# arnauqb/GradABM-JUNE

Measured on AMD Instinct MI355X. Metric: simulation steps/sec, higher is better.
Workload: dtype f32

## Files before the change

### gradabm-june_amd/csrc/gj_tiled.h

```cpp
#pragma once
#include <hip/hip_runtime.h>
#include <stdint.h>

#include "../../include/gradjune_hip.h"
#include "gj_device.h"

namespace gj {

constexpr int kTileThreads = 1024;
constexpr int kTileWaves = kTileThreads / kWave;
constexpr int kMaxSliceAgents = 19840;
constexpr int kUnroll = 8;
#ifndef GJ_UNROLL_NARROW
#define GJ_UNROLL_NARROW 16
#endif
constexpr int kUnrollNarrow = GJ_UNROLL_NARROW;
#ifndef GJ_VENUE_UNROLL
#define GJ_VENUE_UNROLL 2
#endif
constexpr int kVenueUnroll = GJ_VENUE_UNROLL;
#ifndef GJ_VENUE_UNROLL_C
#define GJ_VENUE_UNROLL_C GJ_VENUE_UNROLL
#endif
constexpr int kVenueUnrollC = GJ_VENUE_UNROLL_C;
#ifndef GJ_CUM_BATCH
#define GJ_CUM_BATCH 8
#endif
constexpr int kCumBatch = GJ_CUM_BATCH;
#ifndef GJ_DMA_WIDE
#define GJ_DMA_WIDE 0
#endif

typedef unsigned long long fx_t;
template <int BITS>
__device__ __forceinline__ constexpr float fx_max() { return (float)(1ull << (50 - BITS)); }
template <int BITS>
__device__ __forceinline__ fx_t to_fx(float x) {
  constexpr double scale = (double)(1ull << BITS);
  constexpr double magic = 6755399441055744.0;
  const double d = __builtin_fma((double)x, scale, magic);
  return (fx_t)(__double_as_longlong(d) - 0x4338000000000000LL);
}
template <int BITS>
__device__ __forceinline__ float from_fx(fx_t v) {
  return (float)((double)(long long)v * (1.0 / (double)(1ull << BITS)));
}
constexpr float kSaturated = 1.0e30f;
__device__ __forceinline__ void fx_flag(uint32_t* flags, int words, int i, float x) {
  const uint32_t bit = 1u << (i & 31);
  if (!(x < 0.0f)) atomicOr(&flags[i >> 5], bit);
  if (!(x > 0.0f)) atomicOr(&flags[words + (i >> 5)], bit);
}
template <int BITS>
__device__ __forceinline__ void fx_add(fx_t* sums, uint32_t* flags, int words, int i, float x) {
  const bool ok = fabsf(x) <= fx_max<BITS>();
  atomicAdd(&sums[i], to_fx<BITS>(ok ? x : 0.0f));
  if (__builtin_expect(!ok, 0)) fx_flag(flags, words, i, x);
}
__device__ __forceinline__ float fx_special(uint32_t pos, uint32_t neg, float v) {
  return (pos & neg) ? __builtin_nanf("") : (pos ? kSaturated : (neg ? -kSaturated : v));
}
template <int BITS>
__device__ __forceinline__ float fx_read(const fx_t* sums, const uint32_t* flags, int words, int i) {
  const uint32_t pos = (flags[i >> 5] >> (i & 31)) & 1u, neg = (flags[words + (i >> 5)] >> (i & 31)) & 1u;
  return fx_special(pos, neg, from_fx<BITS>(sums[i]));
}
constexpr int kFxVenue = 36, kFxAgent = 32;

template <typename T>
__device__ __forceinline__ T at32(const T* base, int idx) {
  return *reinterpret_cast<const T*>(reinterpret_cast<const char*>(base) + (uint64_t)((uint32_t)idx * (uint32_t)sizeof(T)));
}
template <typename T>
__device__ __forceinline__ void put32(T* base, int idx, T v) {
  *reinterpret_cast<T*>(reinterpret_cast<char*>(base) + (uint64_t)((uint32_t)idx * (uint32_t)sizeof(T))) = v;
}

typedef float gj_v4f __attribute__((ext_vector_type(4)));
typedef unsigned int gj_v4u __attribute__((ext_vector_type(4)));
typedef unsigned int gj_v2u __attribute__((ext_vector_type(2)));
template <typename T>
__device__ __forceinline__ T at32nt(const T* base, int idx) {
  return __builtin_nontemporal_load(reinterpret_cast<const T*>(reinterpret_cast<const char*>(base) + (uint64_t)((uint32_t)idx * (uint32_t)sizeof(T))));
}
template <typename T>
__device__ __forceinline__ void put32nt(T* base, int idx, T v) {
  __builtin_nontemporal_store(v, reinterpret_cast<T*>(reinterpret_cast<char*>(base) + (uint64_t)((uint32_t)idx * (uint32_t)sizeof(T))));
}
__device__ __forceinline__ uint4 load_nt(const uint4* p) {
  const gj_v4u v = __builtin_nontemporal_load(reinterpret_cast<const gj_v4u*>(p));
  return make_uint4(v.x, v.y, v.z, v.w);
}
__device__ __forceinline__ float4 load_nt(const float4* p) {
  const gj_v4f v = __builtin_nontemporal_load(reinterpret_cast<const gj_v4f*>(p));
  return make_float4(v.x, v.y, v.z, v.w);
}
__device__ __forceinline__ void store_nt(float4* p, float4 x) {
  gj_v4f v = {x.x, x.y, x.z, x.w};
  __builtin_nontemporal_store(v, reinterpret_cast<gj_v4f*>(p));
}
struct TSetA {
  const uint16_t* a_la;
  const int32_t* tile_sptr;
  const int32_t* tile_jpos;
  const int32_t* chunk_ptr;
  const int4* chunk_desc;
  float* val;
  int32_t J;
  int32_t active;
  int32_t raw;
  int32_t wide;
  int32_t direct;
  int32_t presum;
  const int32_t* multi_slots;
};

struct TileAArgs {
  TSetA sets[GJ_MAX_SETS];
  int32_t n_sets;
  int32_t slice_agents;
  int64_t n_agents;
  const float* trans;
  const float* qtrans;
};

__device__ __forceinline__ void load_slice(float* lds, const float* __restrict__ src, int64_t base, int n_local,
                                           int tid) {
  const int n4 = n_local >> 2;
  const float4* s4 = reinterpret_cast<const float4*>(src + base);
  float4* d4 = reinterpret_cast<float4*>(lds);
  constexpr int kQ = (kMaxSliceAgents + 4 * kTileThreads - 1) / (4 * kTileThreads);
  if (n4 > 0) {
    float4 v[kQ];
#pragma unroll
    for (int u = 0; u < kQ; ++u) v[u] = s4[min(tid + u * kTileThreads, n4 - 1)];
#pragma unroll
    for (int u = 0; u < kQ; ++u)
      if (tid + u * kTileThreads < n4) d4[tid + u * kTileThreads] = v[u];
  }
  for (int i = (n4 << 2) + tid; i < n_local; i += kTileThreads) lds[i] = src[base + i];
}

__device__ __forceinline__ int chunk_slot_fast(const int4 d, int lane) {
  const int split = d.z & 0xFFFF;
  return (lane < split) ? d.x + lane : d.y + (lane - split);
}
__device__ __noinline__ int chunk_slot_slow(const TSetA& T, const int4 d, int row, int i, int lane) {
  const int split = d.z & 0xFFFF;
  if (lane < split) return d.x + lane;
  int j = d.w;
  while (i >= T.tile_sptr[row + j + 1]) ++j;
  return T.tile_jpos[row + j] + (i - T.tile_sptr[row + j]);
}

__device__ __forceinline__ int chunk_slot_wide(const int4 d0, const int4 d1, int lane) {
  int b = d0.x;
  b = (lane >= (d1.z & 0xFF)) ? d0.y : b;
  b = (lane >= ((d1.z >> 8) & 0xFF)) ? d0.z : b;
  b = (lane >= ((d1.z >> 16) & 0xFF)) ? d0.w : b;
  b = (lane >= ((d1.z >> 24) & 0xFF)) ? d1.x : b;
  b = (lane >= (d1.w & 0xFF)) ? d1.y : b;
  return b + lane;
}
__device__ __noinline__ int chunk_slot_walk(const TSetA& T, int row, int i, int j) {
  while (i >= T.tile_sptr[row + j + 1]) ++j;
  return T.tile_jpos[row + j] + (i - T.tile_sptr[row + j]);
}

template <bool WIDE, int U>
__device__ __forceinline__ int batch_desc_load(const TSetA& T, int c_base, int n_chunks, int c0, int lane) {
  constexpr int W = WIDE ? 8 : 4;
  static_assert(U * W <= kWave, "a batch's descriptors must fit one wave-wide load");
  const int32_t* desc = reinterpret_cast<const int32_t*>(T.chunk_desc);
  const int u_l = min(lane / W, U - 1), k_l = lane % W;
  return at32(desc, (c_base + min(c0 + u_l, n_chunks - 1)) * W + k_l);
}

template <bool WIDE, int U>
__device__ __forceinline__ void batch_slots(const TSetA& T, const int word, int row, int seg0, int seg1, int c0,
                                            int lane, int (&slot)[U]) {
  constexpr int W = WIDE ? 8 : 4;
  const int k_l = lane % W;
  const bool flag = WIDE ? (k_l == 7 && (word & 0x100)) : (k_l == 2 && (word >> 16));
  const bool any_multi = __builtin_amdgcn_ballot_w64(flag) != 0ull;
#define GJ_DW(u, k) __builtin_amdgcn_readlane(word, (u) * W + (k))
  if (!any_multi) {
#pragma unroll
    for (int u = 0; u < U; ++u) {
      if (!WIDE) {
        slot[u] = chunk_slot_fast(make_int4(GJ_DW(u, 0), GJ_DW(u, 1), GJ_DW(u, 2), 0), lane);
      } else {
        slot[u] = chunk_slot_wide(make_int4(GJ_DW(u, 0), GJ_DW(u, 1), GJ_DW(u, 2), GJ_DW(u, 3)),
                                  make_int4(GJ_DW(u, 4), GJ_DW(u, 5), GJ_DW(u, 6), GJ_DW(u, 7)), lane);
      }
    }
  } else if (T.multi_slots) {
    int ms[U];
    bool mu[U];
#pragma unroll
    for (int u = 0; u < U; ++u) {
      const int w = WIDE ? GJ_DW(u, 7) : GJ_DW(u, 2);
      mu[u] = WIDE ? ((w & 0x100) != 0) : ((w >> 16) != 0);
      const int j0 = WIDE ? (int)((unsigned)w >> 9) : GJ_DW(u, 3);
      ms[u] = at32(T.multi_slots, (mu[u] ? j0 : 0) * kWave + lane);
    }
#pragma unroll
    for (int u = 0; u < U; ++u) {
      int f;
      if (!WIDE) {
        f = chunk_slot_fast(make_int4(GJ_DW(u, 0), GJ_DW(u, 1), GJ_DW(u, 2), 0), lane);
      } else {
        f = chunk_slot_wide(make_int4(GJ_DW(u, 0), GJ_DW(u, 1), GJ_DW(u, 2), GJ_DW(u, 3)),
                            make_int4(GJ_DW(u, 4), GJ_DW(u, 5), GJ_DW(u, 6), GJ_DW(u, 7)), lane);
      }
      slot[u] = mu[u] ? ms[u] : f;
    }
  } else {
#pragma unroll
    for (int u = 0; u < U; ++u) {
      const int i = min(seg0 + (c0 + u) * kWave + lane, seg1 - 1);
      if (!WIDE) {
        const int4 d = make_int4(GJ_DW(u, 0), GJ_DW(u, 1), GJ_DW(u, 2), GJ_DW(u, 3));
        slot[u] = (d.z >> 16) ? chunk_slot_slow(T, d, row, i, lane) : chunk_slot_fast(d, lane);
      } else {
        const int4 d0 = make_int4(GJ_DW(u, 0), GJ_DW(u, 1), GJ_DW(u, 2), GJ_DW(u, 3));
        const int4 d1 = make_int4(GJ_DW(u, 4), GJ_DW(u, 5), GJ_DW(u, 6), GJ_DW(u, 7));
        slot[u] = (d1.w & 0x100) ? chunk_slot_walk(T, row, i, (int)((unsigned)d1.w >> 9))
                                 : chunk_slot_wide(d0, d1, lane);
      }
    }
  }
#undef GJ_DW
}

#ifndef GJ_SCATTER_PIPELINE
#define GJ_SCATTER_PIPELINE 1
#endif
template <bool WIDE, int kU, bool NT = false>
__device__ __forceinline__ void scatter_batches(const TSetA& T, const float* lds_x, int s, int wave, int lane) {
  const int row = s * T.J;
  const int seg0 = T.tile_sptr[row], seg1 = T.tile_sptr[row + T.J];
  const int c_base = T.chunk_ptr[s];
  const int n_chunks = T.chunk_ptr[s + 1] - c_base;
  constexpr int kStride = kTileWaves * kU;
  auto stage1 = [&](int c, int& word, int (&la)[kU]) {
    const int cc = min(c, n_chunks - 1);
    word = batch_desc_load<WIDE, kU>(T, c_base, n_chunks, cc, lane);
#pragma unroll
    for (int u = 0; u < kU; ++u) la[u] = at32(T.a_la, min(seg0 + (cc + u) * kWave + lane, seg1 - 1));
  };
  auto stage2 = [&](int c, int word, const int (&la)[kU]) {
    int slot[kU];
    batch_slots<WIDE, kU>(T, word, row, seg0, seg1, c, lane, slot);
#ifdef GJ_DIAG_EXTRA_VALU
#pragma unroll
    for (int u = 0; u < kU; ++u)
#pragma unroll
      for (int r = 0; r < GJ_DIAG_EXTRA_VALU; ++r) asm volatile("v_add_u32 %0, %0, 0" : "+v"(slot[u]));
#endif
#pragma unroll
    for (int u = 0; u < kU; ++u) {
      const int i = seg0 + (c + u) * kWave + lane;
      if ((c + u < n_chunks) && (i < seg1)) {
        if (NT) put32nt(T.val, slot[u], lds_x[la[u]]); else put32(T.val, slot[u], lds_x[la[u]]);
      }
    }
  };
  int c0 = wave * kU;
  if (c0 >= n_chunks) return;
  int laA[kU], wordA;
#if GJ_SCATTER_PIPELINE
  int laB[kU], wordB;
  stage1(c0, wordA, laA);
  while (true) {
    const int c1 = c0 + kStride;
    stage1(c1, wordB, laB);
    stage2(c0, wordA, laA);
// ... 38 lines not shown
template <bool WIDE>
__device__ __forceinline__ void gather_set(const TSetA& T, fx_t* lds_acc, uint32_t* lds_flags, int flag_words, int s,
                                           int wave, int lane) {
  const int row = s * T.J;
  const int seg0 = T.tile_sptr[row], seg1 = T.tile_sptr[row + T.J];
  const int c_base = T.chunk_ptr[s];
  const int n_chunks = T.chunk_ptr[s + 1] - c_base;
  constexpr int kU = WIDE ? kUnroll : GJ_UNROLL_D_NARROW;
  constexpr int kStride = kTileWaves * kU;
  auto stage1 = [&](int c, int& word, int (&la)[kU]) {
    const int cc = min(c, n_chunks - 1);
    word = batch_desc_load<WIDE, kU>(T, c_base, n_chunks, cc, lane);
#pragma unroll
    for (int u = 0; u < kU; ++u) la[u] = at32(T.a_la, min(seg0 + (cc + u) * kWave + lane, seg1 - 1));
  };
  auto values = [&](int c, int word, float (&v)[kU]) {
    int slot[kU];
    batch_slots<WIDE, kU>(T, word, row, seg0, seg1, c, lane, slot);
#pragma unroll
    for (int u = 0; u < kU; ++u) {
      const int i = seg0 + (c + u) * kWave + lane;
      const bool ok = (c + u < n_chunks) && (i < seg1);
      v[u] = at32nt(T.val, ok ? slot[u] : 0);
    }
  };
  auto add = [&](int c, const int (&la)[kU], const float (&v)[kU]) {
    constexpr uint32_t kLimit = 0x48800000u;
    static_assert(kFxAgent == 32, "kLimit is the pattern of 2^(50 - kFxAgent)");
    float x[kU];
    uint32_t m = 0u;
#pragma unroll
    for (int u = 0; u < kU; ++u) {
      const int i = seg0 + (c + u) * kWave + lane;
      const bool edge = (c + u < n_chunks) && (i < seg1);
      x[u] = edge ? v[u] : 0.0f;
      m = max(m, __float_as_uint(x[u]) & 0x7FFFFFFFu);
    }
#ifdef GJ_DIAG_EXTRA_VALU
#pragma unroll
    for (int u = 0; u < kU; ++u)
#pragma unroll
      for (int r = 0; r < GJ_DIAG_EXTRA_VALU; ++r) asm volatile("v_add_f32 %0, %0, 0" : "+v"(x[u]));
#endif
    if (__builtin_expect(m <= kLimit, 1)) {
#pragma unroll
      for (int u = 0; u < kU; ++u) atomicAdd(&lds_acc[la[u]], to_fx<kFxAgent>(x[u]));
    } else {
#pragma unroll
      for (int u = 0; u < kU; ++u) {
        if ((__float_as_uint(x[u]) & 0x7FFFFFFFu) <= kLimit) {
          atomicAdd(&lds_acc[la[u]], to_fx<kFxAgent>(x[u]));
        } else {
          fx_flag(lds_flags, flag_words, la[u], x[u]);
        }
      }
    }
  };
  int c0 = wave * kU;
  if (c0 >= n_chunks) return;
  int laA[kU], wordA;
  float v[kU];
#if GJ_GATHER_PIPELINE
  int laB[kU], wordB;
  stage1(c0, wordA, laA);
  while (true) {
    const int c1 = c0 + kStride;
    values(c0, wordA, v);
    stage1(c1, wordB, laB);
    add(c0, laA, v);
    if (c1 >= n_chunks) break;
    const int c2 = c1 + kStride;
    values(c1, wordB, v);
    stage1(c2, wordA, laA);
    add(c1, laB, v);
    if (c2 >= n_chunks) break;
    c0 = c2;
  }
#else
  for (; c0 < n_chunks; c0 += kStride) {
    stage1(c0, wordA, laA);
    values(c0, wordA, v);
    add(c0, laA, v);
  }
#endif
}

template <int kU>
__device__ __forceinline__ void scatter_explicit(const TSetA& T, const float* lds_x, int s, int wave, int lane) {
  const int row = s * T.J;
  const int seg0 = T.tile_sptr[row], seg1 = T.tile_sptr[row + T.J];
  const int n_chunks = T.chunk_ptr[s + 1] - T.chunk_ptr[s];
  const int32_t* slots = reinterpret_cast<const int32_t*>(T.chunk_desc);
  for (int c0 = wave * kU; c0 < n_chunks; c0 += kTileWaves * kU) {
    int la[kU], sl[kU];
#pragma unroll
    for (int u = 0; u < kU; ++u) {
      const int i = min(seg0 + (c0 + u) * kWave + lane, seg1 - 1);
      la[u] = at32(T.a_la, i);
      sl[u] = at32(slots, i);
    }
#pragma unroll
    for (int u = 0; u < kU; ++u) {
      const int i = seg0 + (c0 + u) * kWave + lane;
      if ((c0 + u < n_chunks) && (i < seg1)) put32(T.val, sl[u], lds_x[la[u]]);
    }
  }
}

template <int kU>
__device__ __forceinline__ void gather_explicit(const TSetA& T, fx_t* lds_acc, uint32_t* lds_flags, int flag_words, int s,
                                                int wave, int lane) {
  const int row = s * T.J;
  const int seg0 = T.tile_sptr[row], seg1 = T.tile_sptr[row + T.J];
  const int n_chunks = T.chunk_ptr[s + 1] - T.chunk_ptr[s];
  const int32_t* slots = reinterpret_cast<const int32_t*>(T.chunk_desc);
  constexpr uint32_t kLimit = 0x48800000u;
  for (int c0 = wave * kU; c0 < n_chunks; c0 += kTileWaves * kU) {
    int la[kU], sl[kU];
#pragma unroll
    for (int u = 0; u < kU; ++u) {
      const int i = min(seg0 + (c0 + u) * kWave + lane, seg1 - 1);
      la[u] = at32(T.a_la, i);
      sl[u] = at32(slots, i);
    }
    float x[kU];
#pragma unroll
    for (int u = 0; u < kU; ++u) x[u] = at32(T.val, sl[u]);
    uint32_t m = 0u;
#pragma unroll
    for (int u = 0; u < kU; ++u) {
      const int i = seg0 + (c0 + u) * kWave + lane;
      x[u] = ((c0 + u < n_chunks) && (i < seg1)) ? x[u] : 0.0f;
      m = max(m, __float_as_uint(x[u]) & 0x7FFFFFFFu);
    }
    if (__builtin_expect(m <= kLimit, 1)) {
#pragma unroll
      for (int u = 0; u < kU; ++u) atomicAdd(&lds_acc[la[u]], to_fx<kFxAgent>(x[u]));
    } else {
#pragma unroll
      for (int u = 0; u < kU; ++u) {
        if ((__float_as_uint(x[u]) & 0x7FFFFFFFu) <= kLimit) {
          atomicAdd(&lds_acc[la[u]], to_fx<kFxAgent>(x[u]));
        } else {
          fx_flag(lds_flags, flag_words, la[u], x[u]);
        }
      }
    }
  }
}

#ifndef GJ_SCATTER_WAVES_PER_SIMD
#define GJ_SCATTER_WAVES_PER_SIMD 4
#endif
__global__ __launch_bounds__(kTileThreads, GJ_SCATTER_WAVES_PER_SIMD) void k_tile_scatter(const TileAArgs A) {
  extern __shared__ __align__(16) float lds_x[];
  const int tid = threadIdx.x;
  const int wave = __builtin_amdgcn_readfirstlane(tid / kWave), lane = tid % kWave;
  const int s = blockIdx.x;
  const int64_t base = (int64_t)s * A.slice_agents;
  const int n_local = (int)min((int64_t)A.slice_agents, A.n_agents - base);
  const bool two_sources = A.qtrans != A.trans;
  for (int pass = 0; pass < 2; ++pass) {
    if (pass == 1 && !two_sources) break;
    bool any = false;
    for (int t = 0; t < A.n_sets; ++t)
      if (A.sets[t].active && !A.sets[t].presum && (!two_sources || A.sets[t].raw == pass)) any = true;
    if (!any) continue;
    if (pass == 1) __syncthreads();
    load_slice(lds_x, pass == 0 ? A.qtrans : A.trans, base, n_local, tid);
    __syncthreads();
    for (int t = 0; t < A.n_sets; ++t) {
      const TSetA& T = A.sets[t];
      if (!T.active || T.presum || (two_sources && T.raw != pass)) continue;
      if (T.wide == 2) {
        scatter_explicit<kUnroll>(T, lds_x, s, wave, lane);
      } else if (T.wide) {
        scatter_set<true>(T, lds_x, s, wave, lane);
      } else {
        scatter_set<false>(T, lds_x, s, wave, lane);
      }
    }
  }
}

struct TSetB {
  const int32_t* blk_v0;
  const int32_t* blk_e0;
  const uint16_t* e_lv;
  const uint8_t* e_cls;
  float* val;
  const float* v_pc;
  float* cum;
  int32_t stride;
  int32_t nk;
  float beta[GJ_MAX_NETS_PER_SET];
  int32_t table[GJ_MAX_NETS_PER_SET];
  int32_t age75[GJ_MAX_NETS_PER_SET];
  int32_t leisure;
  int32_t direct;
  uint32_t term_limit;
  int32_t _pad_b;
  const uint16_t* pv_blk;
  const int32_t* blk_r0;
  const float* x;
  int64_t n_x;
};

struct TileBArgs {
  TSetB sets[GJ_MAX_SETS];
  const int32_t* work;
  const float* tables;
  int32_t day_type;
  int32_t mode;
  int32_t transpose;
  int32_t _pad;
};

__device__ __noinline__ void venue_group_slow(fx_t* sums, uint32_t* vflags, int words, uint32_t limit, int base_k, int l0,
                                              int l1, int l2, int l3, int l4, int l5, int l6, int l7, float x0, float x1,
                                              float x2, float x3, float x4, float x5, float x6, float x7) {
  const int lv[8] = {l0, l1, l2, l3, l4, l5, l6, l7};
  const float x[8] = {x0, x1, x2, x3, x4, x5, x6, x7};
#pragma unroll
  for (int q = 0; q < 8; ++q) {
    if (lv[q] == 0xFFFF) continue;
    if ((__float_as_uint(x[q]) & 0x7FFFFFFFu) <= limit) {
      atomicAdd(&sums[base_k + lv[q]], to_fx<kFxVenue>(x[q]));
    } else {
      fx_flag(vflags, words, base_k + lv[q], x[q]);
    }
  }
}

struct Slots8 {
  uint32_t w[4];
  __device__ __forceinline__ int lv(int q) const { return (w[q >> 1] >> ((q & 1) * 16)) & 0xFFFF; }
};

#ifdef GJ_DIAG_STAMPS
constexpr int kDiagVenueSlots = 8192;
__device__ unsigned long long gj_diag_venue[3 * kDiagVenueSlots];
struct VenueStamp {
  unsigned long long t0;
  __device__ VenueStamp() : t0(__builtin_amdgcn_s_memrealtime()) {}
  __device__ ~VenueStamp() {
    if (threadIdx.x == 0 && blockIdx.x < kDiagVenueSlots) {
      gj_diag_venue[3 * blockIdx.x] = t0;
      gj_diag_venue[3 * blockIdx.x + 1] = __builtin_amdgcn_s_memrealtime();
      gj_diag_venue[3 * blockIdx.x + 2] = __builtin_amdgcn_s_getreg((31 << 11) | 20) & 0xF;
    }
  }
};
#endif

#ifndef GJ_VENUE_WAVES_PER_SIMD
#define GJ_VENUE_WAVES_PER_SIMD 4
#endif
__global__ __launch_bounds__(kTileThreads, GJ_VENUE_WAVES_PER_SIMD) void k_tile_venues(const TileBArgs B) {
  extern __shared__ __align__(16) float lds_s[];
#ifdef GJ_DIAG_STAMPS
  VenueStamp gj_stamp;
#endif
  const int tid = threadIdx.x;
  const int set = B.work[2 * blockIdx.x], j = B.work[2 * blockIdx.x + 1];
  const TSetB& T = B.sets[set];
  const int nk = T.nk;
  if (nk == 0) return;
  const int v0 = T.blk_v0[j], nv = T.blk_v0[j + 1] - v0;
  const int g0 = T.blk_e0[j] >> 3, g1 = T.blk_e0[j + 1] >> 3;
  fx_t* sums = reinterpret_cast<fx_t*>(lds_s);
  float* cumf = lds_s;
  float* tabs = lds_s + 2 * ((size_t)nk * nv + 64);
  uint32_t* vflags = reinterpret_cast<uint32_t*>(tabs + (T.leisure ? 2 * nk * 200 : 0));
  const int vwords = (nk * nv + 64 + 31) / 32;
  if (T.leisure) {
    for (int i = tid; i < nk * 200; i += kTileThreads) {
      const int k = i / 200, c = i % 200;
      const float l = B.tables[(int64_t)T.table[k] * GJ_TABLE_SIZE + B.day_type * 200 + c];
      const float lw = T.age75[k] ? l * (((c % 100) > 75) ? 1.0f : 0.0f) : l;
      tabs[i] = B.transpose ? lw : l;
      tabs[nk * 200 + i] = B.transpose ? l : lw;
    }
  }
  const uint4* lv8 = reinterpret_cast<const uint4*>(T.e_lv);
  const uint2* cls8 = reinterpret_cast<const uint2*>(T.e_cls);
  float4* val4 = reinterpret_cast<float4*>(T.val);
  if (B.mode != 2) {
    for (int i = tid; i < nk * nv + 64; i += kTileThreads) sums[i] = 0;
    for (int i = tid; i < 2 * vwords; i += kTileThreads) vflags[i] = 0u;
    __syncthreads();
    const int dummy = nk * nv + (tid & 63);
#if defined(GJ_DIAG_FLOAT_RUNS)
    auto run_sums = [&](const int (&lv)[8], const float (&x)[8], int base_k) {
      float s8 = x[0];
#pragma unroll
      for (int q = 0; q < 8; ++q) {
        const bool last = (q == 7) || (lv[q + (q < 7)] != lv[q]);
        const bool take = last && lv[q] != 0xFFFF;
        fx_add<kFxVenue>(sums, vflags, vwords, take ? base_k + lv[q] : dummy, take ? s8 : 0.0f);
        if (q < 7) s8 = last ? x[q + 1] : s8 + x[q + 1];
      }
    };
#elif defined(GJ_DIAG_SLOT_ADDS)
    auto run_sums = [&](const int (&lv)[8], const float (&x)[8], int base_k) {
#pragma unroll
      for (int q = 0; q < 8; ++q) {
        const bool valid = lv[q] != 0xFFFF;
        const bool ok = fabsf(x[q]) <= fx_max<kFxVenue>();
        atomicAdd(&sums[valid ? base_k + lv[q] : dummy], to_fx<kFxVenue>((ok && valid) ? x[q] : 0.0f));
        if (__builtin_expect(!ok && valid, 0)) fx_flag(vflags, vwords, base_k + lv[q], x[q]);
      }
    };
#else
    auto run_sums = [&](const int (&lv)[8], const float (&x)[8], int base_k) {
      const uint32_t kLimit = T.term_limit;
      static_assert(kFxVenue == 36, "term_limit is derived from 2^(50 - kFxVenue) (fill_set_b)");
      uint32_t m = 0u;
#pragma unroll
      for (int q = 0; q < 8; ++q) m = max(m, __float_as_uint(x[q]) & 0x7FFFFFFFu);
      if (__builtin_expect(m > kLimit, 0)) {
        venue_group_slow(sums, vflags, vwords, kLimit, base_k, lv[0], lv[1], lv[2], lv[3], lv[4], lv[5], lv[6], lv[7], x[0],
                         x[1], x[2], x[3], x[4], x[5], x[6], x[7]);
        return;
      }
      fx_t s8 = 0;
#pragma unroll
      for (int q = 0; q < 8; ++q) {
        const fx_t f = to_fx<kFxVenue>(x[q]);
        const bool first = (q == 0) || (lv[q] != lv[q - (q > 0)]);
        s8 = first ? f : s8 + f;
        const bool last = (q == 7) || (lv[q + (q < 7)] != lv[q]);
        const bool take = last && lv[q] != 0xFFFF;
        atomicAdd(&sums[take ? base_k + lv[q] : dummy], s8);
      }
    };
#endif
#ifndef GJ_WAVE_RUNS
#define GJ_WAVE_RUNS 1
#endif
    auto wave_sum = [&](const float (&xl)[8], int target) -> bool {
      uint32_t m = 0u;
#pragma unroll
      for (int q = 0; q < 8; ++q) m = max(m, __float_as_uint(xl[q]) & 0x7FFFFFFFu);
      if (__builtin_amdgcn_ballot_w64(m > T.term_limit) != 0ull) return false;
      fx_t s = 0;
#pragma unroll
      for (int q = 0; q < 8; ++q) s += to_fx<kFxVenue>(xl[q]);
#pragma unroll
      for (int off = 32; off > 0; off >>= 1) s += __shfl_xor(s, off, kWave);
      if ((tid & (kWave - 1)) == 0) atomicAdd(&sums[target], s);
      return true;
    };
    auto add_group = [&](const uint4 raw, const float4 xa, const float4 xb, const uint2 craw) {
      const Slots8 L{{raw.x, raw.y, raw.z, raw.w}};
      const float x[8] = {xa.x, xa.y, xa.z, xa.w, xb.x, xb.y, xb.z, xb.w};
      int lv[8];
#pragma unroll
      for (int q = 0; q < 8; ++q) lv[q] = L.lv(q);
      bool one_venue = false;
#if GJ_WAVE_RUNS
      {
        const bool mine = (raw.x == raw.y) && (raw.y == raw.z) && (raw.z == raw.w) && ((raw.x >> 16) == (raw.x & 0xFFFFu)) &&
                          (lv[0] != 0xFFFF) && (lv[0] == __builtin_amdgcn_readfirstlane(lv[0]));
        one_venue = __builtin_amdgcn_ballot_w64(mine) == ~0ull;
      }
#endif
      if (!T.leisure) {
        if (!(one_venue && wave_sum(x, lv[0]))) run_sums(lv, x, 0);
      } else {
        const uint32_t cw[2] = {craw.x, craw.y};
        for (int k = 0; k < nk; ++k) {
          const float* tk = tabs + k * 200;
          float xl[8];
#pragma unroll
          for (int q = 0; q < 8; ++q) xl[q] = tk[(cw[q >> 2] >> ((q & 3) * 8)) & 0xFF] * x[q];
          if (!(one_venue && wave_sum(xl, k * nv + lv[0]))) run_sums(lv, xl, k * nv);
        }
      }
    };
    for (int g = g0 + tid; g < g1; g += kVenueUnroll * kTileThreads) {
      uint4 raw[kVenueUnroll];
      float4 xa[kVenueUnroll], xb[kVenueUnroll];
      uint2 craw[kVenueUnroll];
#pragma unroll
      for (int u = 0; u < kVenueUnroll; ++u) {
        const int gu = min(g + u * kTileThreads, g1 - 1);
        raw[u] = lv8[gu];
        xa[u] = load_nt(val4 + 2 * gu);
        xb[u] = load_nt(val4 + 2 * gu + 1);
        craw[u] = T.leisure ? cls8[gu] : make_uint2(0u, 0u);
      }
#pragma unroll
      for (int u = 0; u < kVenueUnroll; ++u)
        if (g + u * kTileThreads < g1) add_group(raw[u], xa[u], xb[u], craw[u]);
    }
    if (T.pv_blk) {
      const int r0 = T.blk_r0[j], r1 = T.blk_r0[j + 1];
      const uint4* pv8 = reinterpret_cast<const uint4*>(T.pv_blk);
      const float4* x4 = reinterpret_cast<const float4*>(T.x);
      const int ga = r0 >> 3, gb = (r1 + 7) >> 3;
      const int g_in = (int)(T.n_x >> 3);
      for (int g = ga + tid; g < gb; g += kVenueUnroll * kTileThreads) {
        uint4 raw[kVenueUnroll];
        float4 xa[kVenueUnroll], xb[kVenueUnroll];
#pragma unroll
        for (int u = 0; u < kVenueUnroll; ++u) {
          const int gu = min(g + u * kTileThreads, gb - 1);
          raw[u] = pv8[gu];
          if (gu < g_in) {
            xa[u] = x4[2 * gu];
            xb[u] = x4[2 * gu + 1];
          } else {
            float t[8];
#pragma unroll
            for (int q = 0; q < 8; ++q) t[q] = ((int64_t)gu * 8 + q < T.n_x) ? T.x[(int64_t)gu * 8 + q] : 0.0f;
            xa[u] = make_float4(t[0], t[1], t[2], t[3]);
            xb[u] = make_float4(t[4], t[5], t[6], t[7]);
          }
        }
#pragma unroll
        for (int u = 0; u < kVenueUnroll; ++u) {
          const int gu = g + u * kTileThreads;
          if (gu >= gb) continue;
          const Slots8 L{{raw[u].x, raw[u].y, raw[u].z, raw[u].w}};
          const float x[8] = {xa[u].x, xa[u].y, xa[u].z, xa[u].w, xb[u].x, xb[u].y, xb[u].z, xb[u].w};
          int lv[8];
#pragma unroll
          for (int q = 0; q < 8; ++q) {
            const int a = gu * 8 + q;
            lv[q] = (a >= r0 && a < r1) ? L.lv(q) : 0xFFFF;
          }
          run_sums(lv, x, 0);
        }
      }
    }
    __syncthreads();
    for (int l0 = tid; l0 < nv; l0 += kCumBatch * kTileThreads) {
      float pc[kCumBatch];
#pragma unroll
      for (int u = 0; u < kCumBatch; ++u) pc[u] = T.v_pc[v0 + min(l0 + u * kTileThreads, nv - 1)];
      for (int k = 0; k < nk; ++k) {
        const float beta = T.beta[k];
#pragma unroll
        for (int u = 0; u < kCumBatch; ++u) {
          const int lv = l0 + u * kTileThreads;
          if (lv < nv) {
            const float c = (beta * pc[u]) * fx_read<kFxVenue>(sums, vflags, vwords, k * nv + lv);
            T.cum[(int64_t)(v0 + lv) * T.stride + k] = c;
            cumf[2 * (k * nv + lv)] = c;
          }
        }
      }
    }
    if (B.mode == 1 || T.direct) return;
  } else {
    if (T.direct) return;
    for (int k = 0; k < nk; ++k) {
      for (int l0 = tid; l0 < nv; l0 += kCumBatch * kTileThreads) {
        float c[kCumBatch];
#pragma unroll
        for (int u = 0; u < kCumBatch; ++u)
          c[u] = T.cum[(int64_t)(v0 + min(l0 + u * kTileThreads, nv - 1)) * T.stride + k];
#pragma unroll
        for (int u = 0; u < kCumBatch; ++u) {
          const int lv = l0 + u * kTileThreads;
          if (lv < nv) cumf[2 * (k * nv + lv)] = c[u];
        }
      }
    }
  }
  __syncthreads();
  for (int g = g0 + tid; g < g1; g += kVenueUnrollC * kTileThreads) {
    uint4 raw[kVenueUnrollC];
    uint2 craw[kVenueUnrollC];
#pragma unroll
    for (int u = 0; u < kVenueUnrollC; ++u) {
      const int gu = min(g + u * kTileThreads, g1 - 1);
      raw[u] = lv8[gu];
      craw[u] = T.leisure ? cls8[gu] : make_uint2(0u, 0u);
    }
#pragma unroll
    for (int u = 0; u < kVenueUnrollC; ++u) {
      const int gu = g + u * kTileThreads;
      if (gu >= g1) continue;
      const Slots8 L{{raw[u].x, raw[u].y, raw[u].z, raw[u].w}};
      float r[8];
      if (!T.leisure) {
#pragma unroll
        for (int q = 0; q < 8; ++q) {
          const int lv = L.lv(q);
          const float c = cumf[2 * (lv != 0xFFFF ? lv : 0)];
          r[q] = (lv != 0xFFFF) ? c : 0.0f;
        }
      } else {
        const uint32_t cw[2] = {craw[u].x, craw[u].y};
#pragma unroll
        for (int q = 0; q < 8; ++q) {
          const int lv = L.lv(q);
          const int c = (cw[q >> 2] >> ((q & 3) * 8)) & 0xFF;
          const int li = lv != 0xFFFF ? lv : 0;
          float a = 0.0f;
          for (int k = 0; k < nk; ++k) a += tabs[nk * 200 + k * 200 + c] * cumf[2 * (k * nv + li)];
          r[q] = (lv != 0xFFFF) ? a : 0.0f;
        }
      }
      store_nt(val4 + 2 * gu, make_float4(r[0], r[1], r[2], r[3]));
      store_nt(val4 + 2 * gu + 1, make_float4(r[4], r[5], r[6], r[7]));
    }
  }
}

constexpr int GJ_MAX_PRESUM = 6;
constexpr int64_t kPresumBad = (int64_t)0x8000000000000000ll;
struct TPSet {
  const uint16_t* ell;
  int64_t plane_stride;
  fx_t* partial;
  int32_t planes, V, stride, nk;
  int32_t group_venues;
  int32_t raw, leisure, _pad;
  int32_t table[GJ_MAX_NETS_PER_SET];
  int32_t age75[GJ_MAX_NETS_PER_SET];
};
struct TilePArgs {
  TPSet sets[GJ_MAX_PRESUM];
  int32_t n_sets;
  int32_t agents_per_wg;
  int64_t n_agents;
  const float* trans;
  const float* qtrans;
  const uint8_t* cls;
  const float* tables;
  int32_t day_type, transpose;
};

constexpr int kPresumQuads = 3;
__device__ __forceinline__ void fx_add_or_poison(fx_t* sums, uint32_t* flags, int i, float x) {
  const bool ok = fabsf(x) <= fx_max<kFxVenue>();
  atomicAdd(&sums[i], to_fx<kFxVenue>(ok ? x : 0.0f));
  if (__builtin_expect(!ok, 0)) atomicOr(&flags[i >> 5], 1u << (i & 31));
}

__global__ __launch_bounds__(kTileThreads) void k_tile_presum(const TilePArgs P) {
  extern __shared__ __align__(16) fx_t lds_p[];
  const int tid = threadIdx.x;
  const int64_t a_begin = (int64_t)blockIdx.x * P.agents_per_wg;
  const int64_t a_end = min(P.n_agents, a_begin + P.agents_per_wg);
  const int n_quads = (int)((max(a_end - a_begin, (int64_t)0) + 3) >> 2);
  for (int t = 0; t < P.n_sets; ++t) {
    const TPSet& T = P.sets[t];
    const int nk = T.nk;
    const float* x = T.raw ? P.trans : P.qtrans;
    for (int v0 = 0; v0 < T.V; v0 += T.group_venues) {
      const int nv = min(T.group_venues, T.V - v0);
      const int n_sums = nv * nk;
      const int dummy = n_sums + (tid & 63);
      float* wtab = reinterpret_cast<float*>(lds_p + n_sums + 64);
      uint32_t* flags = reinterpret_cast<uint32_t*>(wtab + (T.leisure ? nk * 200 : 0));
      __syncthreads();
      for (int i = tid; i < n_sums + 64; i += kTileThreads) lds_p[i] = 0;
      for (int i = tid; i < (n_sums + 64 + 31) / 32; i += kTileThreads) flags[i] = 0u;
      if (T.leisure) {
        for (int i = tid; i < nk * 200; i += kTileThreads) {
          const int k = i / 200, c = i % 200;
          const float l = P.tables[(int64_t)T.table[k] * GJ_TABLE_SIZE + P.day_type * 200 + c];
          const float lw = T.age75[k] ? l * (((c % 100) > 75) ? 1.0f : 0.0f) : l;
          wtab[i] = P.transpose ? lw : l;
        }
      }
      __syncthreads();
      for (int plane = 0; plane < T.planes; ++plane) {
        const uint16_t* ell = T.ell + plane * T.plane_stride + a_begin * 2;
        struct Batch {
          uint4 rows[kPresumQuads];
          float4 xs[kPresumQuads];
          uint32_t cl[kPresumQuads];
        };
        auto load = [&](int b0, Batch& B) {
#pragma unroll
          for (int u = 0; u < kPresumQuads; ++u) {
            const int q = min(b0 + tid + u * kTileThreads, n_quads - 1);
            const int64_t a0 = a_begin + 4 * (int64_t)q;
            B.rows[u] = *reinterpret_cast<const uint4*>(ell + 8 * (int64_t)q);
            if (a0 + 4 <= P.n_agents) {
              B.xs[u] = *reinterpret_cast<const float4*>(x + a0);
            } else {
              B.xs[u] = make_float4(a0 < P.n_agents ? x[a0] : 0.0f, a0 + 1 < P.n_agents ? x[a0 + 1] : 0.0f,
                                    a0 + 2 < P.n_agents ? x[a0 + 2] : 0.0f, 0.0f);
            }
            B.cl[u] = T.leisure ? *reinterpret_cast<const uint32_t*>(P.cls + a0) : 0u;
          }
        };
        auto add = [&](int b0, const Batch& B) {
#pragma unroll
          for (int u = 0; u < kPresumQuads; ++u) {
            const int q = b0 + tid + u * kTileThreads;
            if (q >= n_quads) continue;
            const uint32_t w[4] = {B.rows[u].x, B.rows[u].y, B.rows[u].z, B.rows[u].w};
            const float xv[4] = {B.xs[u].x, B.xs[u].y, B.xs[u].z, B.xs[u].w};
            const int n_ok = (int)min((int64_t)4, a_end - (a_begin + 4 * (int64_t)q));
#pragma unroll
            for (int j = 0; j < 4; ++j) {
#pragma unroll
              for (int c = 0; c < 2; ++c) {
                const int lv = (int)((w[j] >> (16 * c)) & 0xFFFF) - v0;
                const bool in = ((unsigned)lv < (unsigned)nv) && (j < n_ok);
                if (!T.leisure) {
                  fx_add_or_poison(lds_p, flags, in ? lv : dummy, in ? xv[j] : 0.0f);
                } else {
                  const int cj = (B.cl[u] >> (8 * j)) & 0xFF;
                  for (int k = 0; k < nk; ++k)
                    fx_add_or_poison(lds_p, flags, in ? lv * nk + k : dummy, in ? wtab[k * 200 + cj] * xv[j] : 0.0f);
                }
              }
            }
          }
        };
        constexpr int kStep = kPresumQuads * kTileThreads;
        if (n_quads > 0) {
          Batch ba, bb;
          int b0 = 0;
          load(b0, ba);
          while (true) {
            const bool more1 = b0 + kStep < n_quads;
            if (more1) load(b0 + kStep, bb);
            add(b0, ba);
            if (!more1) break;
            b0 += kStep;
            const bool more2 = b0 + kStep < n_quads;
            if (more2) load(b0 + kStep, ba);
            add(b0, bb);
            if (!more2) break;
            b0 += kStep;
          }
        }
      }
      __syncthreads();
      fx_t* out = T.partial + (int64_t)blockIdx.x * T.V * T.stride;
      for (int i = tid; i < n_sums; i += kTileThreads) {
        const int lv = i / nk, k = i % nk;
        const bool bad = (flags[i >> 5] >> (i & 31)) & 1u;
        out[(int64_t)(v0 + lv) * T.stride + k] = bad ? (fx_t)kPresumBad : lds_p[i];
      }
    }
  }
}

struct PReduceSet {
  const fx_t* partial;
  const float* v_pc;
  float* cum;
  int32_t V, stride, nk, first;
  float beta[GJ_MAX_NETS_PER_SET];
};
struct PReduceArgs {
  PReduceSet sets[GJ_MAX_PRESUM];
  int32_t n_sets, n_wgs;
  int32_t total;
  int32_t _pad;
};

__global__ __launch_bounds__(kThreads) void k_presum_reduce(const PReduceArgs R) {
  __shared__ fx_t part[kThreads / kWave][kWave];
  __shared__ uint32_t bad_any[kWave];
  const int lane = threadIdx.x % kWave, wave = threadIdx.x / kWave;
  const int i = blockIdx.x * kWave + lane;
  const bool in = i < R.total;
  int t = 0;
  while (t + 1 < R.n_sets && i >= R.sets[t + 1].first) ++t;
  const PReduceSet& T = R.sets[t];
  const int e = in ? i - T.first : 0;
  const int v = e / T.nk, k = e % T.nk;
  const int64_t idx = (int64_t)v * T.stride + k, table = (int64_t)T.V * T.stride;
  fx_t s = 0;
  bool bad = false;
  if (threadIdx.x < kWave) bad_any[threadIdx.x] = 0u;
  constexpr int kWaves = kThreads / kWave;
  for (int w0 = wave; w0 < R.n_wgs; w0 += kWaves * 8) {
    fx_t p[8];
#pragma unroll
    for (int u = 0; u < 8; ++u) {
      const int w = w0 + u * kWaves;
      p[u] = (in && w < R.n_wgs) ? T.partial[w * table + idx] : (fx_t)0;
    }
#pragma unroll
    for (int u = 0; u < 8; ++u) {
      bad |= p[u] == (fx_t)kPresumBad;
      s += p[u];
    }
  }
  part[wave][lane] = s;
  __syncthreads();
  if (bad) atomicOr(&bad_any[lane], 1u);
  __syncthreads();
  if (wave == 0 && in) {
    fx_t total = 0;
#pragma unroll
    for (int w = 0; w < kWaves; ++w) total += part[w][lane];
    T.cum[idx] = (T.beta[k] * T.v_pc[v]) * (bad_any[lane] ? __builtin_nanf("") : from_fx<kFxVenue>(total));
  }
}

constexpr int GJ_MAX_DIRECT = GJ_MAX_SETS;
constexpr int kClassWeightFloats = GJ_MAX_NETS_PER_SET * 200;
struct TDirect {
  const uint16_t* ell;
  const float* cum;
  int64_t plane_stride;
  int32_t K, planes;
  int32_t V, stride, nk;
  int32_t region;
  int32_t group_venues;
  int32_t _pad;
  int32_t raw, leisure;
  int32_t table[GJ_MAX_NETS_PER_SET];
  int32_t age75[GJ_MAX_NETS_PER_SET];
  const int32_t* win_lo;
  const int32_t* win_n;
};

struct TileDArgs {
  TSetA sets[GJ_MAX_SETS];
  int32_t n_sets;
  int32_t slice_agents;
  int64_t n_agents;
  const float* stage;
  float* susceptibility;
  float* is_infected;
  float* infection_time;
  float* not_infected_probs;
  float* new_infected;
  float* trans_susc;
  const float* exp_noise;
  float now, dt, q_thr;
  int32_t has_q, sample;
  uint64_t seed, step;
  int64_t agent_offset;
  float* acc_scratch;
  float* agent_sums;
  TDirect direct[GJ_MAX_DIRECT];
  int32_t n_direct;
  int32_t table_floats;
  int32_t table1_floats;
  int32_t _pad3;
  int32_t day_type, transpose;
  const uint8_t* cls;
  const float* tables;
  const gj_clock* clock;
  int32_t _pad2;
  int32_t io_vec4;
};

__global__ __launch_bounds__(256) void k_tile_epilogue(const TileDArgs D) {
  const int64_t a = (int64_t)blockIdx.x * blockDim.x + threadIdx.x;
  if (a >= D.n_agents) return;
  const float now = D.clock ? D.clock->now : D.now;
  const uint64_t step = D.clock ? D.clock->step : D.step;
  float susc = D.susceptibility[a];
  float ts = susc * D.acc_scratch[a];
  if (D.trans_susc) D.trans_susc[a] = ts;
  const float p = not_infected_prob(ts, D.dt);
  if (D.not_infected_probs) D.not_infected_probs[a] = p;
  if (!D.sample) return;
  float e0, e1;
  if (D.exp_noise) {
    e0 = D.exp_noise[a];
    e1 = D.exp_noise[D.n_agents + a];
  } else {
    e0 = e1 = 1.0f;
  }
  const float nw = D.exp_noise ? gumbel_new_infected(p, e0, e1)
                               : own_new_infected(p, infection_uniform(D.seed, step, D.agent_offset + a));
  if (D.new_infected) D.new_infected[a] = nw;
  if (nw != 0.0f) {
    float inf = D.is_infected[a], t_inf = D.infection_time[a];
    infect(nw, now, susc, inf, t_inf);
    D.susceptibility[a] = susc;
    D.is_infected[a] = inf;
    D.infection_time[a] = t_inf;
  }
}

constexpr int kQuadsPerLane = (kMaxSliceAgents + 4 * kTileThreads - 1) / (4 * kTileThreads);
static_assert(kQuadsPerLane * 4 * kTileThreads >= kMaxSliceAgents, "a lane's quads must cover the largest slice");

struct DirectBatch {
  uint32_t w[kQuadsPerLane][4];
  uint32_t cls[kQuadsPerLane];
};

__device__ __forceinline__ void direct_load(const TileDArgs& D, const TDirect& T, int64_t base, int n_local, int tid,
                                            int plane, DirectBatch& b) {
  const unsigned last_quad = (unsigned)(n_local - 1) >> 2;
  const uint16_t* ell = T.ell + plane * T.plane_stride + base * 2;
  const uint8_t* cls = D.cls + base;
#pragma unroll
  for (int u = 0; u < kQuadsPerLane; ++u) {
    unsigned q = min((unsigned)(tid + u * kTileThreads), last_quad);
    asm volatile("" : "+v"(q));
    if (!T.win_lo) {
      const uint4 r = load_nt(reinterpret_cast<const uint4*>(ell + 8u * q));
      b.w[u][0] = r.x;
      b.w[u][1] = r.y;
      b.w[u][2] = r.z;
      b.w[u][3] = r.w;
    } else {
      const uint2 r = *reinterpret_cast<const uint2*>(T.ell + base + 4u * q);
      b.w[u][0] = (r.x & 0xFFFFu) | 0xFFFF0000u;
      b.w[u][1] = (r.x >> 16) | 0xFFFF0000u;
      b.w[u][2] = (r.y & 0xFFFFu) | 0xFFFF0000u;
      b.w[u][3] = (r.y >> 16) | 0xFFFF0000u;
    }
    b.cls[u] = T.leisure ? *reinterpret_cast<const uint32_t*>(cls + 4u * q) : 0u;
  }
}

__device__ __forceinline__ void direct_add(const TileDArgs& D, const TDirect& T, float (&acc)[kQuadsPerLane][4],
                                           uint32_t qmask, const float* wtab, const float* tab, int v0, int nv,
                                           int n_local, int tid, const DirectBatch& b) {
  constexpr int K = 2;
  const int nk = T.nk, stride = T.stride;
#pragma unroll
  for (int u = 0; u < kQuadsPerLane; ++u) {
    const int q = tid + u * kTileThreads;
    if (4 * q >= n_local) continue;
    const uint32_t quarantined = T.raw ? 0u : (qmask >> (4 * u)) & 0xFu;
    int idx[4][K];
    bool ok[4][K];
    float x[4][K];
#pragma unroll
    for (int j = 0; j < 4; ++j) {
#pragma unroll
      for (int c = 0; c < K; ++c) {
        const int h = j * K + c;
        const int lv = (int)((b.w[u][h >> 1] >> (16 * (h & 1))) & 0xFFFF) - v0;
        ok[j][c] = ((unsigned)lv < (unsigned)nv) && !((quarantined >> j) & 1u);
        idx[j][c] = ok[j][c] ? lv : 0;
      }
    }
    if (!T.leisure) {
#pragma unroll
      for (int j = 0; j < 4; ++j)
#pragma unroll
        for (int c = 0; c < K; ++c) x[j][c] = tab[idx[j][c] * stride];
    } else {
#pragma unroll
      for (int j = 0; j < 4; ++j)
#pragma unroll
        for (int c = 0; c < K; ++c) x[j][c] = 0.0f;
#pragma unroll
      for (int k = 0; k < GJ_MAX_NETS_PER_SET; ++k) {
        if (k >= nk) break;
        float w[4];
#pragma unroll
        for (int j = 0; j < 4; ++j) w[j] = wtab[k * 200 + ((b.cls[u] >> (8 * j)) & 0xFF)];
#pragma unroll
        for (int j = 0; j < 4; ++j)
#pragma unroll
          for (int c = 0; c < K; ++c) x[j][c] += w[j] * tab[idx[j][c] * stride + k];
      }
    }
#pragma unroll
    for (int j = 0; j < 4; ++j) {
      float sj = 0.0f;
#pragma unroll
      for (int c = 0; c < K; ++c) sj += ok[j][c] ? x[j][c] : 0.0f;
      acc[u][j] += sj;
    }
  }
}

__device__ __forceinline__ void direct_stage(const TileDArgs& D, const TDirect& T, float* wtab, float* tab, int v0,
                                             int nv, int tid) {
  if (T.leisure && v0 == 0) {
    for (int i = tid; i < T.nk * 200; i += kTileThreads) {
      const int k = i / 200, c = i % 200;
      const float l = D.tables[(int64_t)T.table[k] * GJ_TABLE_SIZE + D.day_type * 200 + c];
      const float lw = T.age75[k] ? l * (((c % 100) > 75) ? 1.0f : 0.0f) : l;
      wtab[i] = D.transpose ? l : lw;
    }
  }
#ifndef GJ_DIAG_NO_DIRECT_TABLE
  const float* src = T.cum + (int64_t)v0 * T.stride;
  const int n = nv * T.stride;
  const int lane = tid % kWave, wave = __builtin_amdgcn_readfirstlane(tid / kWave);
#if GJ_DMA_WIDE
  const bool aligned = ((reinterpret_cast<uintptr_t>(src) | reinterpret_cast<uintptr_t>(tab)) & 15u) == 0;
  const int n_wide = aligned ? (n / (4 * kWave)) * (4 * kWave) : 0;
  for (int p = wave; (p + 1) * 4 * kWave <= n_wide; p += kTileWaves)
    __builtin_amdgcn_global_load_lds(src + p * 4 * kWave + 4 * lane, tab + p * 4 * kWave, 16, 0, 0);
  for (int p = wave; n_wide + p * kWave < n; p += kTileWaves)
    __builtin_amdgcn_global_load_lds(src + min(n_wide + p * kWave + lane, n - 1), tab + n_wide + p * kWave, 4, 0, 0);
#else
  for (int p = wave; p * kWave < n; p += kTileWaves)
    __builtin_amdgcn_global_load_lds(src + min(p * kWave + lane, n - 1), tab + p * kWave, 4, 0, 0);
#endif
#endif
}

__device__ __forceinline__ void publish_staged() {
  asm volatile("s_waitcnt vmcnt(0)" ::: "memory");
  __syncthreads();
}

__device__ __forceinline__ bool direct_next(const TileDArgs& D, int& t, int& v0, int& plane) {
  const TDirect& T = D.direct[t];
  if (plane + 1 < T.planes) {
    ++plane;
    return true;
  }
  plane = 0;
  if (!T.win_lo && v0 + T.group_venues < T.V) {
    v0 += T.group_venues;
    return true;
  }
  v0 = 0;
  ++t;
  return t < D.n_direct;
}

__device__ __forceinline__ void direct_sets(const TileDArgs& D, float (&acc)[kQuadsPerLane][4], uint32_t qmask,
                                            float* lds, int64_t base, int n_local, int tid, DirectBatch& cur,
                                            uint64_t diag_t0 = 0) {
  auto wtab_of = [&](int t) { return lds + (t & 1) * kClassWeightFloats; };
  auto tab_of = [&](const TDirect& T) {
    return lds + 2 * kClassWeightFloats + (T.region ? D.table_floats + kWave : 0);
  };
  auto group_nv = [&](const TDirect& T, int v0) { return T.win_lo ? T.win_n[blockIdx.x] : min(T.group_venues, T.V - v0); };
  auto group_lo = [&](const TDirect& T, int v0) { return T.win_lo ? T.win_lo[blockIdx.x] : v0; };
  int t = 0, v0 = 0, plane = 0;
  __syncthreads();
  direct_stage(D, D.direct[0], wtab_of(0), tab_of(D.direct[0]), group_lo(D.direct[0], 0), group_nv(D.direct[0], 0), tid);
  bool more = true;
  while (more) {
    const TDirect& T = D.direct[t];
    const int nv = group_nv(T, v0);
    if (plane == 0) publish_staged();
#ifdef GJ_DIAG_STAMPS
    if (threadIdx.x == 0 && D.trans_susc && t < 4)
      D.trans_susc[(int64_t)blockIdx.x * D.slice_agents + 8 + 2 * t] = (float)(__builtin_amdgcn_s_memtime() - diag_t0);
#endif
    int tn = t, vn = v0, pn = plane;
    more = direct_next(D, tn, vn, pn);
    const bool new_group = more && pn == 0;
    const bool overlap = new_group && D.direct[tn].region != T.region;
    if (overlap)
      direct_stage(D, D.direct[tn], wtab_of(tn), tab_of(D.direct[tn]), group_lo(D.direct[tn], vn), group_nv(D.direct[tn], vn), tid);
    DirectBatch nxt;
    if (more) direct_load(D, D.direct[tn], base, n_local, tid, pn, nxt);
#ifndef GJ_DIAG_NO_DIRECT_ADD
    direct_add(D, T, acc, qmask, wtab_of(t), tab_of(T), v0, nv, n_local, tid, cur);
#else
    if (cur.w[0][0] == 0x12345678u && cur.cls[0] == 77u) acc[0][0] = 1.0f;
#endif
#ifdef GJ_DIAG_STAMPS
    if (threadIdx.x == 0 && D.trans_susc && t < 4)
      D.trans_susc[(int64_t)blockIdx.x * D.slice_agents + 9 + 2 * t] = (float)(__builtin_amdgcn_s_memtime() - diag_t0);
#endif
    if (new_group && !overlap) {
      __syncthreads();
      direct_stage(D, D.direct[tn], wtab_of(tn), tab_of(D.direct[tn]), group_lo(D.direct[tn], vn), group_nv(D.direct[tn], vn), tid);
    }
    if (more) cur = nxt;
    t = tn;
    v0 = vn;
    plane = pn;
  }
}

__device__ __forceinline__ void load_quad(const float* p, int64_t a0, int n_ok, bool vec, float (&v)[4]) {
  if (vec && n_ok >= 4) {
    const float4 x = *reinterpret_cast<const float4*>(p + a0);
    v[0] = x.x;
    v[1] = x.y;
    v[2] = x.z;
    v[3] = x.w;
  } else {
#pragma unroll
    for (int j = 0; j < 4; ++j) v[j] = (j < n_ok) ? p[a0 + j] : 0.0f;
  }
}
template <bool NT = false>
__device__ __forceinline__ void store_quad(float* p, int64_t a0, int n_ok, bool vec, const float (&v)[4]) {
  if (vec && n_ok >= 4) {
    if (NT) {
      store_nt(reinterpret_cast<float4*>(p + a0), make_float4(v[0], v[1], v[2], v[3]));
    } else {
      *reinterpret_cast<float4*>(p + a0) = make_float4(v[0], v[1], v[2], v[3]);
    }
  } else {
#pragma unroll
    for (int j = 0; j < 4; ++j)
      if (j < n_ok) p[a0 + j] = v[j];
  }
}

#ifdef GJ_DIAG_STAMPS
#define GJ_STAMP(k)                                                                                         \
  do {                                                                                                      \
    if (threadIdx.x == 0 && D.trans_susc)                                                                    \
      D.trans_susc[(int64_t)blockIdx.x * D.slice_agents + (k)] = (float)(__builtin_amdgcn_s_memtime() - gj_t0); \
  } while (0)
#else
#define GJ_STAMP(k) do { } while (0)
#endif

__global__ __launch_bounds__(kTileThreads) void k_tile_agents(const TileDArgs D) {
  extern __shared__ __align__(16) fx_t lds_acc[];
#ifdef GJ_DIAG_STAMPS
  const uint64_t gj_t0 = __builtin_amdgcn_s_memtime();
#endif
  const int tid = threadIdx.x;
  const int wave = __builtin_amdgcn_readfirstlane(tid / kWave), lane = tid % kWave;
  const int s = blockIdx.x;
  const int64_t base = (int64_t)s * D.slice_agents;
  const int n_local = (int)min((int64_t)D.slice_agents, D.n_agents - base);
  uint32_t* lds_flags = reinterpret_cast<uint32_t*>(lds_acc + D.slice_agents);
  const int fwords = D.slice_agents / 32;
  for (int i = tid; i < n_local; i += kTileThreads) lds_acc[i] = 0;
  for (int i = tid; i < 2 * fwords; i += kTileThreads) lds_flags[i] = 0u;
  DirectBatch first;
  if (D.n_direct > 0) direct_load(D, D.direct[0], base, n_local, tid, 0, first);
  __syncthreads();
  for (int pass = 0; pass < 2; ++pass) {
    for (int t = 0; t < D.n_sets; ++t) {
      const TSetA& T = D.sets[t];
      if (!T.active || T.direct || T.raw != pass) continue;
      if (T.wide == 2) {
        gather_explicit<kUnroll>(T, lds_acc, lds_flags, fwords, s, wave, lane);
      } else if (T.wide) {
        gather_set<true>(T, lds_acc, lds_flags, fwords, s, wave, lane);
      } else {
        gather_set<false>(T, lds_acc, lds_flags, fwords, s, wave, lane);
      }
    }
    __syncthreads();
    if (pass == 0 && D.has_q) {
      constexpr int kStageBatch = 10;
      for (int i0 = tid; i0 < n_local; i0 += kStageBatch * kTileThreads) {
        float stg[kStageBatch];
#pragma unroll
        for (int u = 0; u < kStageBatch; ++u) stg[u] = D.stage[base + min(i0 + u * kTileThreads, n_local - 1)];
#pragma unroll
        for (int u = 0; u < kStageBatch; ++u) {
          const int i = i0 + u * kTileThreads;
          if (i < n_local && !(stg[u] < D.q_thr)) {
            lds_acc[i] = 0;
            const uint32_t bit = 1u << (i & 31);
            const bool pos = lds_flags[i >> 5] & bit, neg = lds_flags[fwords + (i >> 5)] & bit;
            if (pos != neg) {
              atomicAnd(&lds_flags[i >> 5], ~bit);
              atomicAnd(&lds_flags[fwords + (i >> 5)], ~bit);
            }
          }
        }
      }
      __syncthreads();
    }
  }
  GJ_STAMP(1);
  constexpr int kQ = kQuadsPerLane;
  float acc[kQ][4];
#pragma unroll
  for (int m = 0; m < kQ; ++m) {
    const int i0 = 4 * (tid + m * kTileThreads);
    const int iq = min(i0, D.slice_agents - 4);
    const uint32_t pos = (lds_flags[iq >> 5] >> (iq & 31)) & 0xFu, neg = (lds_flags[fwords + (iq >> 5)] >> (iq & 31)) & 0xFu;
    fx_t raw[4];
#pragma unroll
    for (int j = 0; j < 4; ++j) raw[j] = lds_acc[iq + j];
#pragma unroll
    for (int j = 0; j < 4; ++j) {
      const float v = from_fx<kFxAgent>(raw[j]);
      acc[m][j] = (i0 < n_local) ? (((pos | neg) >> j) & 1u ? fx_special((pos >> j) & 1u, (neg >> j) & 1u, v) : v) : 0.0f;
    }
  }
  if (D.n_direct > 0) {
    uint32_t qmask = 0u;
    if (D.has_q) {
      float stg[kQ][4];
#pragma unroll
      for (int m = 0; m < kQ; ++m) {
        const int i0 = 4 * (tid + m * kTileThreads);
#pragma unroll
        for (int j = 0; j < 4; ++j) stg[m][j] = (i0 + j < n_local) ? D.stage[base + i0 + j] : -INFINITY;
      }
#pragma unroll
      for (int m = 0; m < kQ; ++m)
#pragma unroll
        for (int j = 0; j < 4; ++j) qmask |= (stg[m][j] < D.q_thr) ? 0u : (1u << (4 * m + j));
    }
    GJ_STAMP(2);
#ifndef GJ_DIAG_NO_DIRECT_SETS
#ifdef GJ_DIAG_STAMPS
    direct_sets(D, acc, qmask, reinterpret_cast<float*>(lds_acc), base, n_local, tid, first, gj_t0);
#else
    direct_sets(D, acc, qmask, reinterpret_cast<float*>(lds_acc), base, n_local, tid, first);
#endif
#endif
    GJ_STAMP(3);
  }
  const bool vec = D.io_vec4 != 0;
  if (D.agent_sums) {
#pragma unroll
    for (int m = 0; m < kQ; ++m) {
      const int i0 = 4 * (tid + m * kTileThreads);
      if (i0 < n_local) store_quad<true>(D.agent_sums, base + i0, n_local - i0, vec, acc[m]);
    }
  }
  if (D.acc_scratch) {
#pragma unroll
    for (int m = 0; m < kQ; ++m) {
      const int i0 = 4 * (tid + m * kTileThreads);
      if (i0 < n_local) store_quad(D.acc_scratch, base + i0, n_local - i0, vec, acc[m]);
    }
    return;
  }
  const float now = D.clock ? D.clock->now : D.now;
  const uint64_t step = D.clock ? D.clock->step : D.step;
  const bool own_noise = D.sample && !D.exp_noise;
  const int mis = (int)((D.agent_offset + base) & 3);
  float4* ts4 = reinterpret_cast<float4*>(lds_acc);
  {
    float sq[kQ][4];
#pragma unroll
    for (int m = 0; m < kQ; ++m) {
      int i0 = 4 * (tid + m * kTileThreads);
      asm volatile("" : "+v"(i0));
#pragma unroll
      for (int j = 0; j < 4; ++j) sq[m][j] = 0.0f;
      if (i0 < n_local) load_quad(D.susceptibility, base + i0, n_local - i0, vec, sq[m]);
    }
    __syncthreads();
#pragma unroll
    for (int m = 0; m < kQ; ++m) {
      const int q = tid + m * kTileThreads;
      if (4 * q < n_local)
        ts4[q] = make_float4(sq[m][0] * acc[m][0], sq[m][1] * acc[m][1], sq[m][2] * acc[m][2], sq[m][3] * acc[m][3]);
    }
  }
  GJ_STAMP(4);
  uint32_t infected = 0u;
  int m_run = 0;
  for (int q = tid; 4 * q < n_local; q += kTileThreads, ++m_run) {
    const int i0 = 4 * q;
    const float4 tq = ts4[q];
    const float ts[4] = {tq.x, tq.y, tq.z, tq.w};
    const int64_t a0 = base + i0;
    const int n_ok = n_local - i0;
    float p[4];
#pragma unroll
    for (int j = 0; j < 4; ++j) p[j] = not_infected_prob(ts[j], D.dt);
#ifndef GJ_DIAG_STAMPS
    if (D.trans_susc) store_quad<true>(D.trans_susc, a0, n_ok, vec, ts);
#endif
    if (D.not_infected_probs) store_quad<true>(D.not_infected_probs, a0, n_ok, vec, p);
    if (!D.sample) continue;
    float nw[4], th[4] = {0.0f, 0.0f, 0.0f, 0.0f};
    if (own_noise) {
      const uint64_t g0 = (uint64_t)(D.agent_offset + a0);
      uint32_t r0[4], r1[4] = {0u, 0u, 0u, 0u};
      philox4x32_10(g0 >> 2, step, D.seed, r0);
      if (mis) philox4x32_10((g0 >> 2) + 1, step, D.seed, r1);
#pragma unroll
      for (int j = 0; j < 4; ++j) {
        const int w = mis + j;
        th[j] = u01(w == 0 ? r0[0] : w == 1 ? r0[1] : w == 2 ? r0[2] : w == 3 ? r0[3] : w == 4 ? r1[0] : w == 5 ? r1[1] : r1[2]);
      }
    }
#pragma unroll
    for (int j = 0; j < 4; ++j) {
      if (own_noise) {
        nw[j] = own_new_infected(p[j], th[j]);
      } else {
        float e0 = 1.0f, e1 = 1.0f;
        if (j < n_ok) {
          e0 = D.exp_noise[a0 + j];
          e1 = D.exp_noise[D.n_agents + a0 + j];
        }
        nw[j] = gumbel_new_infected(p[j], e0, e1);
      }
      if (j < n_ok && nw[j] != 0.0f) infected |= 1u << (4 * m_run + j);
    }
    if (D.new_infected) store_quad<true>(D.new_infected, a0, n_ok, vec, nw);
#pragma unroll
    for (int j = 0; j < 4; ++j) {
      if (j < n_ok && nw[j] != 0.0f && nw[j] != 1.0f) {
        infected &= ~(1u << (4 * m_run + j));
        const int64_t a = a0 + j;
        float sc = D.susceptibility[a], inf = D.is_infected[a], t_inf = D.infection_time[a];
        infect(nw[j], now, sc, inf, t_inf);
        D.susceptibility[a] = sc;
        D.is_infected[a] = inf;
        D.infection_time[a] = t_inf;
      }
    }
  }
  GJ_STAMP(6);
#ifndef GJ_TAIL_BATCHED
  if (__builtin_amdgcn_ballot_w64(infected != 0u) != 0ull) {
    uint32_t todo = infected;
    while (todo) {
      const int k = __builtin_ctz(todo);
      todo &= todo - 1u;
      const int64_t a = base + 4 * (tid + (k >> 2) * kTileThreads) + (k & 3);
      float sc = D.susceptibility[a], inf = D.is_infected[a], tinf = D.infection_time[a];
      infect(1.0f, now, sc, inf, tinf);
      D.susceptibility[a] = sc;
      D.is_infected[a] = inf;
      D.infection_time[a] = tinf;
    }
  }
#else
  if (__builtin_amdgcn_ballot_w64(infected != 0u) != 0ull) {
    float sc[kQ][4], inf[kQ][4], tinf[kQ][4];
#pragma unroll
    for (int m = 0; m < kQ; ++m) {
#pragma unroll
      for (int j = 0; j < 4; ++j) {
        const bool hit = (infected >> (4 * m + j)) & 1u;
        const int64_t a = hit ? base + 4 * (tid + m * kTileThreads) + j : base;
        sc[m][j] = D.susceptibility[a];
        inf[m][j] = D.is_infected[a];
        tinf[m][j] = D.infection_time[a];
      }
    }
#pragma unroll
    for (int m = 0; m < kQ; ++m) {
#pragma unroll
      for (int j = 0; j < 4; ++j) {
        const int64_t a = base + 4 * (tid + m * kTileThreads) + j;
        infect(1.0f, now, sc[m][j], inf[m][j], tinf[m][j]);
        if ((infected >> (4 * m + j)) & 1u) {
          D.susceptibility[a] = sc[m][j];
          D.is_infected[a] = inf[m][j];
          D.infection_time[a] = tinf[m][j];
        }
      }
    }
  }
#endif
  GJ_STAMP(5);
}

}
```

### gradabm-june_amd/csrc/gradjune_hip.hip

```cpp
#include <hip/hip_runtime.h>
#include <math.h>
#include <stdint.h>
#include <string.h>

#include "../../include/gradjune_hip.h"
#include "gj_device.h"
#include "gj_tiled.h"

namespace gj {

struct SetP1 {
  const int32_t* v_rowptr;
  const int32_t* v_agent;
  const float* v_pc;
  float* cum;
  int32_t stride;
  int32_t nk;
  float beta[GJ_MAX_NETS_PER_SET];
  int32_t table[GJ_MAX_NETS_PER_SET];
  int32_t raw;
  int32_t leisure;
};

struct P1Args {
  SetP1 sets[GJ_MAX_SETS];
  const gj_block* blocks;
  const float* trans;
  const float* qtrans;
  const uint8_t* cls;
  const float* tables;
  float* partial;
  int32_t day_type;
};

struct SetP2 {
  const int32_t* a_rowptr;
  const int32_t* a_venue;
  const float* cum;
  int32_t stride;
  int32_t nk;
  int32_t mask[GJ_MAX_NETS_PER_SET];
  int32_t table[GJ_MAX_NETS_PER_SET];
};

struct P2Args {
  SetP2 groups[GJ_MAX_SETS];
  int32_t n_groups;
  int32_t any_leisure;
  int64_t n_agents;
  const uint8_t* cls;
  const float* tables;
  const float* stage;
  float* susceptibility;
  float* is_infected;
  float* infection_time;
  float* not_infected_probs;
  float* new_infected;
  float* trans_susc;
  const float* exp_noise;
  float now, dt, q_thr;
  int32_t day_type, has_q, sample;
  uint64_t seed, step;
  int64_t agent_offset;
  const gj_clock* clock;
};

__device__ __forceinline__ float inv_gamma(float x) {
  if (!(x > 0.25f && x < 16.0f)) return expf(-lgammaf(x));
  float up = 1.0f, down = 1.0f;
  while (x > 2.0f) {
    x -= 1.0f;
    up *= x;
  }
  while (x < 1.0f) {
    down *= x;
    x += 1.0f;
  }
  const float z = x - 1.0f;
  float g = 0.035868343f;
  g = g * z - 0.193527818f;
  g = g * z + 0.482199394f;
  g = g * z - 0.756704078f;
  g = g * z + 0.918206857f;
  g = g * z - 0.897056937f;
  g = g * z + 0.988205891f;
  g = g * z - 0.577191652f;
  g = g * z + 1.0f;
  return down / (g * up);
}
__device__ __forceinline__ float fast_pow(float x, float y) {
  if (y == 0.0f) return 1.0f;
  if (x < 0.0f) {
    const float yi = truncf(y);
    if (yi != y) return __builtin_nanf("");
    const float r = __builtin_amdgcn_exp2f(y * __builtin_amdgcn_logf(-x));
    const float h = 0.5f * yi;
    return (truncf(h) != h) ? -r : r;
  }
  return __builtin_amdgcn_exp2f(y * __builtin_amdgcn_logf(x));
}
__device__ __forceinline__ float fast_exp(float e) { return __builtin_amdgcn_exp2f(e * 1.44269504088896341f); }

__device__ __forceinline__ float transmission_value(float mx, float shp, float rt, float sh, float t_inf,
                                                    float inf, float now) {
  const float t = now - t_inf;
  const float d = t - sh;
  const float sign = (sgnf(d + 1e-10f) + 1.0f) / 2.0f;
  const float aux = inv_gamma(shp) * fast_pow(d * rt, shp - 1.0f);
  const float aux2 = fast_exp((sh - t) * rt) * rt;
  return mx * sign * aux * aux2 * inf;
}

__global__ __launch_bounds__(kThreads) void k_transmission(
    int64_t n, const float* __restrict__ mx, const float* __restrict__ shp, const float* __restrict__ rt,
    const float* __restrict__ sh, const float* __restrict__ t_inf, const float* __restrict__ inf,
    const float* __restrict__ stage, float* __restrict__ trans, float* __restrict__ qtrans, float now_arg,
    int has_q, float q_thr, const gj_clock* __restrict__ clock) {
  const float now = clock ? clock->now : now_arg;
  const int64_t n4 = n >> 2;
  const int64_t stride = (int64_t)gridDim.x * blockDim.x;
  for (int64_t i = (int64_t)blockIdx.x * blockDim.x + threadIdx.x; i < n4; i += stride) {
    const float4 f = load_nt(reinterpret_cast<const float4*>(inf) + i);
    float4 r = make_float4(0.0f, 0.0f, 0.0f, 0.0f);
    unsigned m = (f.x != 0.0f ? 1u : 0u) | (f.y != 0.0f ? 2u : 0u) | (f.z != 0.0f ? 4u : 0u) | (f.w != 0.0f ? 8u : 0u);
    if (m) {
      const float4 a = load_nt(reinterpret_cast<const float4*>(mx) + i);
      const float4 b = load_nt(reinterpret_cast<const float4*>(shp) + i);
      const float4 c = load_nt(reinterpret_cast<const float4*>(rt) + i);
      const float4 d = load_nt(reinterpret_cast<const float4*>(sh) + i);
      const float4 e = load_nt(reinterpret_cast<const float4*>(t_inf) + i);
      while (m) {
        const int k = __builtin_ctz(m);
        m &= m - 1u;
#define GJ_PICK(v) (k == 0 ? v.x : k == 1 ? v.y : k == 2 ? v.z : v.w)
        const float val = transmission_value(GJ_PICK(a), GJ_PICK(b), GJ_PICK(c), GJ_PICK(d), GJ_PICK(e), GJ_PICK(f), now);
#undef GJ_PICK
        r.x = k == 0 ? val : r.x;
        r.y = k == 1 ? val : r.y;
        r.z = k == 2 ? val : r.z;
        r.w = k == 3 ? val : r.w;
      }
    }
    reinterpret_cast<float4*>(trans)[i] = r;
    if (has_q) {
      const float4 s = reinterpret_cast<const float4*>(stage)[i];
      float4 q;
      q.x = (s.x < q_thr ? 1.0f : 0.0f) * r.x;
      q.y = (s.y < q_thr ? 1.0f : 0.0f) * r.y;
      q.z = (s.z < q_thr ? 1.0f : 0.0f) * r.z;
      q.w = (s.w < q_thr ? 1.0f : 0.0f) * r.w;
      reinterpret_cast<float4*>(qtrans)[i] = q;
    }
  }
  if (blockIdx.x == 0) {
    const int64_t i = (n4 << 2) + threadIdx.x;
// ... 977 lines not shown
    S.v_rowptr = E.v_rowptr;
    S.v_agent = E.v_agent;
    S.v_pc = E.v_pcontact;
    S.cum = E.cum;
    S.stride = E.cum_stride;
    S.nk = G.nk[g];
    S.raw = p->nets[G.first[g]].mask_kind == GJ_MASK_RAW;
    S.leisure = 0;
    for (int k = 0; k < G.nk[g]; ++k) {
      const gj_network& N = p->nets[G.first[g] + k];
      S.beta[k] = N.beta;
      S.table[k] = N.mask_kind >= GJ_MASK_QL ? N.table : -1;
      if (N.mask_kind >= GJ_MASK_QL) S.leisure = 1;
    }
    if (S.leisure) {
      for (int k = 0; k < G.nk[g]; ++k)
        if (S.table[k] < 0) return GJ_E_PLAN;
    }
  }
  A.blocks = plan->blocks;
  A.trans = st->transmission;
  A.qtrans = p->has_quarantine ? st->q_transmission : st->transmission;
  A.cls = plan->agent_class;
  A.tables = plan->tables;
  A.partial = plan->partial;
  A.day_type = p->day_type;
  hipLaunchKernelGGL(k_venue_reduce, dim3((unsigned)plan->n_blocks), dim3(kThreads), 0, stream, A);
  int rc = launch_status();
  if (rc != GJ_OK) return rc;
  if (plan->n_long_rows > 0) {
    CombineArgs C;
    for (int s = 0; s < GJ_MAX_SETS; ++s) {
      C.sets[s].cum = A.sets[s].cum;
      C.sets[s].stride = A.sets[s].stride;
      C.sets[s].nk = A.sets[s].nk;
    }
    C.rows = plan->long_rows;
    C.partial = plan->partial;
    C.n_rows = plan->n_long_rows;
    const int64_t threads = (int64_t)plan->n_long_rows * GJ_MAX_NETS_PER_SET;
    hipLaunchKernelGGL(k_combine_long, dim3((unsigned)((threads + kThreads - 1) / kThreads)), dim3(kThreads), 0,
                       stream, C);
    rc = launch_status();
  }
  return rc;
}

static int do_agent_gather(const gj_plan* plan, const gj_agent_state* st, const gj_step_params* p, const Groups& G,
                           const gj_step_io* io, int sample, hipStream_t stream) {
  const int64_t n = plan->n_agents;
  if (n == 0) return GJ_OK;
  if (io && io->agent_sums) return GJ_E_PLAN;
  P2Args P;
  P.n_groups = G.n;
  P.any_leisure = 0;
  for (int g = 0; g < G.n; ++g) {
    const gj_edge_set& E = plan->sets[G.set[g]];
    SetP2& S = P.groups[g];
    S.a_rowptr = E.a_rowptr;
    S.a_venue = E.a_venue;
    S.cum = E.cum;
    S.stride = E.cum_stride;
    S.nk = G.nk[g];
    for (int k = 0; k < GJ_MAX_NETS_PER_SET; ++k) {
      S.mask[k] = 0;
      S.table[k] = 0;
    }
    for (int k = 0; k < G.nk[g]; ++k) {
      const gj_network& N = p->nets[G.first[g] + k];
      S.mask[k] = N.mask_kind;
      S.table[k] = N.mask_kind >= GJ_MASK_QL ? N.table : 0;
      if (N.mask_kind >= GJ_MASK_QL) P.any_leisure = 1;
    }
  }
  P.n_agents = n;
  P.cls = plan->agent_class;
  P.tables = plan->tables;
  P.stage = st->current_stage;
  P.susceptibility = st->susceptibility;
  P.is_infected = st->is_infected;
  P.infection_time = st->infection_time;
  P.not_infected_probs = io ? io->not_infected_probs : nullptr;
  P.new_infected = io ? io->new_infected : nullptr;
  P.trans_susc = io ? io->trans_susc : nullptr;
  P.exp_noise = io ? io->exp_noise : nullptr;
  P.now = p->now;
  P.dt = p->delta_time;
  P.q_thr = p->q_threshold;
  P.day_type = p->day_type;
  P.has_q = p->has_quarantine;
  P.sample = sample;
  P.seed = p->seed;
  P.step = p->step;
  P.agent_offset = p->agent_offset;
  P.clock = p->clock;
  const int64_t blocks = (n + kThreads - 1) / kThreads;
  hipLaunchKernelGGL(k_agent_gather, dim3((unsigned)blocks), dim3(kThreads), 0, stream, P);
  return launch_status();
}

static int check_tiled(const gj_plan* plan) {
  const gj_tiled* T = plan->tiled;
  if (T->n_slices < 1 || T->slice_agents < 64 || T->slice_agents % 64 || T->slice_agents > kMaxSliceAgents) return GJ_E_PLAN;
  if ((int64_t)T->n_slices * T->slice_agents < plan->n_ext_agents) return GJ_E_PLAN;
  if (T->n_work < 0 || (T->n_work > 0 && !T->work)) return GJ_E_PLAN;
  for (int s = 0; s < plan->n_sets; ++s) {
    const gj_tiled_set& S = T->sets[s];
    if (S.n_blocks < 0) return GJ_E_PLAN;
    if (S.n_blocks == 0) continue;
    if (!S.blk_v0 || !S.blk_e0 || !S.tile_sptr || !S.tile_jpos || !S.chunk_ptr) return GJ_E_NULL;
    const bool run = S.run_pv_blk || S.run_pv_win || S.run_blk_r0 || S.run_win_lo || S.run_win_n;
    if (run) {
      if (!S.run_pv_blk || !S.run_pv_win || !S.run_blk_r0 || !S.run_win_lo || !S.run_win_n) return GJ_E_NULL;
      if (S.run_max_window < 0 || S.run_max_window > 32768 || S.run_tiled_edges < 0 ||
          S.run_tiled_edges > plan->sets[s].n_edges || S.ell_k)
        return GJ_E_PLAN;
    }
    if (S.presum && (!S.ell_k || T->presum_wgs < 1 || T->presum_wgs > 4096)) return GJ_E_PLAN;
    const int64_t held = run ? (int64_t)S.run_tiled_edges : plan->sets[s].n_edges;
    if (held > 0 && (!S.e_lv || !S.a_la || !S.val || !S.chunk_desc)) return GJ_E_NULL;
    if (S.max_block_venues < 1 || S.max_block_venues > 65536) return GJ_E_PLAN;
    if (plan->sets[s].n_edges >= ((int64_t)1 << 30) - 8 * (int64_t)S.n_blocks) return GJ_E_RANGE;
    if (S.ell_k) {
      if (S.ell_k != 2 && S.ell_k != 4 && S.ell_k != 8) return GJ_E_PLAN;
      if (!S.ell) return GJ_E_NULL;
      if (plan->sets[s].n_venues > 65534) return GJ_E_PLAN;
    }
  }
  return GJ_OK;
}

static inline int64_t tiled_edges(const gj_plan* plan, int s) {
  const gj_tiled_set& S = plan->tiled->sets[s];
  return S.run_pv_blk ? (int64_t)S.run_tiled_edges : plan->sets[s].n_edges;
}

static inline bool uses_presum(const gj_plan* plan, int s) {
  const gj_tiled* T = plan->tiled;
  return T->presum_wgs > 0 && T->sets[s].presum != nullptr && T->sets[s].ell_k != 0 && T->sets[s].n_blocks > 0 &&
         plan->sets[s].n_edges > 0;
}

template <typename K>
static int allow_lds(K kernel, size_t bytes) {
  if (bytes > 160 * 1024) return GJ_E_PLAN;
  if (bytes > 64 * 1024) {
    const hipError_t e = hipFuncSetAttribute(reinterpret_cast<const void*>(kernel),
                                             hipFuncAttributeMaxDynamicSharedMemorySize, (int)bytes);
    if (e != hipSuccess) return (int)e;
  }
  return GJ_OK;
}

static void fill_set_a(const gj_plan* plan, const gj_step_params* p, const Groups& G, TSetA* sets) {
  const gj_tiled* T = plan->tiled;
  for (int s = 0; s < GJ_MAX_SETS; ++s) sets[s] = TSetA{};
  for (int g = 0; g < G.n; ++g) {
    const int s = G.set[g];
    const gj_tiled_set& S = T->sets[s];
    sets[s].a_la = S.a_la;
    sets[s].tile_sptr = S.tile_sptr;
    sets[s].tile_jpos = S.tile_jpos;
    sets[s].chunk_ptr = S.chunk_ptr;
    sets[s].chunk_desc = reinterpret_cast<const int4*>(S.chunk_desc);
    sets[s].val = S.val;
    sets[s].J = S.n_blocks;
    sets[s].active = (S.n_blocks > 0 && tiled_edges(plan, s) > 0) ? G.nk[g] : 0;
    sets[s].presum = uses_presum(plan, s);
    sets[s].raw = p->nets[G.first[g]].mask_kind == GJ_MASK_RAW;
    sets[s].wide = S.desc_wide;
    sets[s].direct = S.ell_k != 0;
    sets[s].multi_slots = S.multi_slots;
  }
}

static size_t slice_lds(const gj_tiled* T, size_t elem) { return (size_t)T->slice_agents * elem; }
static size_t agents_lds(const gj_tiled* T) { return (size_t)T->slice_agents * sizeof(fx_t) + 2 * ((size_t)T->slice_agents / 8); }

static int presum_fill(const gj_plan* plan, const gj_step_params* p, const Groups& G, int g, TPSet* X) {
  const gj_tiled* T = plan->tiled;
  const int s = G.set[g];
  const gj_tiled_set& S = T->sets[s];
  const gj_edge_set& E = plan->sets[s];
  const int64_t owned_slices = (plan->n_agents + T->slice_agents - 1) / T->slice_agents;
  X->ell = S.ell;
  X->plane_stride = owned_slices * (int64_t)T->slice_agents * 2;
  X->partial = reinterpret_cast<fx_t*>(S.presum);
  X->planes = S.ell_k / 2;
  X->V = (int32_t)E.n_venues;
  X->stride = E.cum_stride;
  X->nk = G.nk[g];
  X->raw = p->nets[G.first[g]].mask_kind == GJ_MASK_RAW;
  X->leisure = 0;
  X->_pad = 0;
  for (int k = 0; k < GJ_MAX_NETS_PER_SET; ++k) X->table[k] = X->age75[k] = 0;
  for (int k = 0; k < G.nk[g]; ++k) {
    const gj_network& N = p->nets[G.first[g] + k];
    X->table[k] = N.mask_kind >= GJ_MASK_QL ? N.table : -1;
    X->age75[k] = N.mask_kind == GJ_MASK_QL_AGE75;
    if (N.mask_kind >= GJ_MASK_QL) X->leisure = 1;
  }
  if (X->leisure) {
    if (!plan->agent_class || (uintptr_t)plan->agent_class % 4 != 0) return GJ_E_PLAN;
    for (int k = 0; k < G.nk[g]; ++k)
      if (X->table[k] < 0) return GJ_E_PLAN;
  } else if (G.nk[g] != 1) {
    return GJ_E_PLAN;
  }
  return GJ_OK;
}

static int tiled_presum(const gj_plan* plan, const gj_agent_state* st, const gj_step_params* p, const Groups& G,
                        hipStream_t stream) {
  const gj_tiled* T = plan->tiled;
  TilePArgs P;
  P.n_sets = 0;
  for (int g = 0; g < G.n; ++g) {
    if (!uses_presum(plan, G.set[g])) continue;
    if (P.n_sets == GJ_MAX_PRESUM) return GJ_E_PLAN;
    const int rc = presum_fill(plan, p, G, g, &P.sets[P.n_sets++]);
    if (rc) return rc;
  }
  if (P.n_sets == 0 || plan->n_agents == 0) return GJ_OK;
  const int64_t budget = 160 * 1024;
  size_t lds = 0;
  for (int t = 0; t < P.n_sets; ++t) {
    TPSet& X = P.sets[t];
    const int64_t fixed = 64 * 8 + (X.leisure ? (int64_t)X.nk * 200 * 4 : 0) + 64;
    int64_t per_venue = (int64_t)X.nk * 8;
    int64_t gv = (budget - fixed) * 8 / (per_venue * 8 + X.nk);
    if (T->direct_table_floats > 0 && gv > T->direct_table_floats / X.nk) gv = T->direct_table_floats / X.nk;
    if (gv > X.V) gv = X.V;
    if (gv < 1) gv = 1;
    X.group_venues = (int32_t)gv;
    const size_t need = (size_t)(gv * X.nk + 64) * 8 + (X.leisure ? (size_t)X.nk * 200 * 4 : 0) + ((size_t)(gv * X.nk + 64 + 31) / 32) * 4;
    if (need > lds) lds = need;
  }
  int64_t apw = (plan->n_agents + T->presum_wgs - 1) / T->presum_wgs;
  apw = (apw + 63) / 64 * 64;
  P.agents_per_wg = (int32_t)apw;
  P.n_agents = plan->n_agents;
  P.trans = st->transmission;
  P.qtrans = p->has_quarantine ? st->q_transmission : st->transmission;
  if ((uintptr_t)P.trans % 16 != 0 || (uintptr_t)P.qtrans % 16 != 0) return GJ_E_PLAN;
  P.cls = plan->agent_class;
  P.tables = plan->tables;
  P.day_type = p->day_type;
  P.transpose = p->transpose;
  int rc = allow_lds(k_tile_presum, lds);
  if (rc) return rc;
  hipLaunchKernelGGL(k_tile_presum, dim3((unsigned)T->presum_wgs), dim3(kTileThreads), lds, stream, P);
  return launch_status();
}

static int tiled_presum_reduce(const gj_plan* plan, const gj_step_params* p, const Groups& G, hipStream_t stream) {
  const gj_tiled* T = plan->tiled;
  PReduceArgs R;
  R.n_sets = 0;
  R.n_wgs = T->presum_wgs;
  R._pad = 0;
  int64_t total = 0;
  for (int g = 0; g < G.n; ++g) {
    const int s = G.set[g];
    if (!uses_presum(plan, s)) continue;
    if (R.n_sets == GJ_MAX_PRESUM) return GJ_E_PLAN;
    PReduceSet& X = R.sets[R.n_sets++];
    const gj_edge_set& E = plan->sets[s];
    X.partial = reinterpret_cast<const fx_t*>(T->sets[s].presum);
    X.v_pc = E.v_pcontact;
    X.cum = E.cum;
    X.V = (int32_t)E.n_venues;
    X.stride = E.cum_stride;
    X.nk = G.nk[g];
    X.first = (int32_t)total;
    for (int k = 0; k < GJ_MAX_NETS_PER_SET; ++k) X.beta[k] = k < G.nk[g] ? p->nets[G.first[g] + k].beta : 0.0f;
    total += (int64_t)X.V * X.nk;
  }
  if (R.n_sets == 0 || total == 0) return GJ_OK;
  if (total > INT32_MAX) return GJ_E_RANGE;
  R.total = (int32_t)total;
  hipLaunchKernelGGL(k_presum_reduce, dim3((unsigned)((total + kWave - 1) / kWave)), dim3(kThreads), 0, stream, R);
  return launch_status();
}

static int tiled_scatter(const gj_plan* plan, const gj_agent_state* st, const gj_step_params* p, const Groups& G,
                         hipStream_t stream) {
  const gj_tiled* T = plan->tiled;
  if (plan->n_ext_agents == 0 || G.n == 0) return GJ_OK;
  TileAArgs A;
  fill_set_a(plan, p, G, A.sets);
  A.n_sets = plan->n_sets;
  A.slice_agents = T->slice_agents;
  A.n_agents = plan->n_ext_agents;
  A.trans = st->transmission;
  A.qtrans = p->has_quarantine ? st->q_transmission : st->transmission;
  const size_t lds = slice_lds(T, sizeof(float));
  int rc = allow_lds(k_tile_scatter, lds);
  if (rc) return rc;
  hipLaunchKernelGGL(k_tile_scatter, dim3((unsigned)T->n_slices), dim3(kTileThreads), lds, stream, A);
  rc = launch_status();
  if (rc) return rc;
  return tiled_presum(plan, st, p, G, stream);
}

static uint32_t venue_term_limit(int32_t max_venue_edges) {
  int e = 14;
  int64_t p2 = 4096;
  while (p2 < (int64_t)max_venue_edges && e > -20) {
    p2 <<= 1;
    --e;
  }
  const float lim = ldexpf(1.0f, e);
  uint32_t bits;
  memcpy(&bits, &lim, sizeof(bits));
  return bits;
}

static int tiled_venues(const gj_plan* plan, const gj_agent_state* st, const gj_step_params* p, const Groups& G, int mode,
                        hipStream_t stream) {
  const gj_tiled* T = plan->tiled;
  if (G.n == 0) return GJ_OK;
  if (T->n_work == 0) return mode == 2 ? GJ_OK : tiled_presum_reduce(plan, p, G, stream);
  TileBArgs B;
  for (int s = 0; s < GJ_MAX_SETS; ++s) B.sets[s] = TSetB{};
  size_t lds = 16;
  for (int g = 0; g < G.n; ++g) {
    const int s = G.set[g];
    const gj_tiled_set& S = T->sets[s];
    const gj_edge_set& E = plan->sets[s];
    TSetB& X = B.sets[s];
    X.blk_v0 = S.blk_v0;
    X.blk_e0 = S.blk_e0;
    X.e_lv = S.e_lv;
    X.e_cls = S.e_cls;
    X.val = S.val;
    X.v_pc = E.v_pcontact;
    X.cum = E.cum;
    X.stride = E.cum_stride;
    X.nk = S.n_blocks > 0 ? G.nk[g] : 0;
    if (uses_presum(plan, s)) X.nk = 0;
    X.direct = S.ell_k != 0;
    X.leisure = 0;
    for (int k = 0; k < G.nk[g]; ++k) {
      const gj_network& N = p->nets[G.first[g] + k];
      X.beta[k] = N.beta;
      X.table[k] = N.mask_kind >= GJ_MASK_QL ? N.table : -1;
      X.age75[k] = N.mask_kind == GJ_MASK_QL_AGE75;
      if (N.mask_kind >= GJ_MASK_QL) X.leisure = 1;
    }
    if (X.leisure) {
      if (!S.e_cls && E.n_edges > 0) return GJ_E_PLAN;
      for (int k = 0; k < G.nk[g]; ++k)
        if (X.table[k] < 0) return GJ_E_PLAN;
    } else if (G.nk[g] != 1) {
      return GJ_E_PLAN;
    }
    X.pv_blk = nullptr;
    X.blk_r0 = nullptr;
    X.x = nullptr;
    X.n_x = 0;
    if (S.run_pv_blk && mode != 2) {
      if (X.leisure) return GJ_E_PLAN;
      const bool raw = p->nets[G.first[g]].mask_kind == GJ_MASK_RAW;
      X.x = (p->has_quarantine && !raw) ? st->q_transmission : st->transmission;
      if (!X.x) return GJ_E_NULL;
      if ((uintptr_t)X.x % 16 != 0 || (uintptr_t)S.run_pv_blk % 16 != 0) return GJ_E_PLAN;
      X.pv_blk = S.run_pv_blk;
      X.blk_r0 = S.run_blk_r0;
      X.n_x = plan->n_ext_agents;
    }
    const size_t n_sums = (size_t)X.nk * S.max_block_venues + 64;
    const size_t need = n_sums * sizeof(fx_t) + (X.leisure ? 2 * 200 * (size_t)X.nk : 0) * sizeof(float) +
                        2 * ((n_sums + 31) / 32 * 4);
    X.term_limit = venue_term_limit(S.max_venue_edges);
    if (X.nk && need > lds) lds = need;
  }
  B.work = T->work;
  B.tables = plan->tables;
  B.day_type = p->day_type;
  B.mode = mode;
  B.transpose = p->transpose;
  int rc = allow_lds(k_tile_venues, lds);
  if (rc) return rc;
  hipLaunchKernelGGL(k_tile_venues, dim3((unsigned)T->n_work), dim3(kTileThreads), lds, stream, B);
  rc = launch_status();
  if (rc || mode == 2) return rc;
  return tiled_presum_reduce(plan, p, G, stream);
}

static int tiled_agents(const gj_plan* plan, const gj_agent_state* st, const gj_step_params* p, const Groups& G,
                        const gj_step_io* io, int sample, hipStream_t stream) {
  const gj_tiled* T = plan->tiled;
  if (plan->n_agents == 0) return GJ_OK;
  TileDArgs D;
  fill_set_a(plan, p, G, D.sets);
  D.n_sets = plan->n_sets;
  D.slice_agents = T->slice_agents;
  D.n_agents = plan->n_agents;
  D.stage = st->current_stage;
  D.susceptibility = st->susceptibility;
  D.is_infected = st->is_infected;
  D.infection_time = st->infection_time;
  D.not_infected_probs = io ? io->not_infected_probs : nullptr;
  D.new_infected = io ? io->new_infected : nullptr;
  D.trans_susc = io ? io->trans_susc : nullptr;
  D.agent_sums = io ? io->agent_sums : nullptr;
  D.exp_noise = io ? io->exp_noise : nullptr;
  D.now = p->now;
  D.dt = p->delta_time;
  D.q_thr = p->q_threshold;
  D.has_q = p->has_quarantine;
  D.sample = sample;
  D.seed = p->seed;
  D.step = p->step;
  D.agent_offset = p->agent_offset;
  D.clock = p->clock;
  D.acc_scratch = T->agent_scratch;
  size_t lds = agents_lds(T);
  D.n_direct = 0;
  D.day_type = p->day_type;
  D.transpose = p->transpose;
  D.cls = plan->agent_class;
  D.tables = plan->tables;
  const int64_t owned_slices = (plan->n_agents + T->slice_agents - 1) / T->slice_agents;
  for (int g = 0; g < G.n; ++g) {
    const int s = G.set[g];
    const gj_tiled_set& S = T->sets[s];
    const gj_edge_set& E = plan->sets[s];
    const bool run = S.run_pv_win != nullptr;
    if ((!S.ell_k && !run) || S.n_blocks == 0 || E.n_edges == 0) continue;
    if (D.n_direct == GJ_MAX_DIRECT) return GJ_E_PLAN;
    TDirect& X = D.direct[D.n_direct++];
    X.ell = run ? S.run_pv_win : S.ell;
    X.cum = E.cum;
    X.K = 2;
    X.planes = run ? 1 : S.ell_k / 2;
    X.plane_stride = owned_slices * (int64_t)T->slice_agents * 2;
    X.V = run ? S.run_max_window : (int32_t)E.n_venues;
    X.win_lo = run ? S.run_win_lo : nullptr;
    X.win_n = run ? S.run_win_n : nullptr;
    if (run && (uintptr_t)S.run_pv_win % 8 != 0) return GJ_E_PLAN;
    X.stride = E.cum_stride;
    X.nk = G.nk[g];
    X.raw = p->nets[G.first[g]].mask_kind == GJ_MASK_RAW;
    X.leisure = 0;
    for (int k = 0; k < GJ_MAX_NETS_PER_SET; ++k) X.table[k] = X.age75[k] = 0;
    for (int k = 0; k < G.nk[g]; ++k) {
      const gj_network& N = p->nets[G.first[g] + k];
      X.table[k] = N.mask_kind >= GJ_MASK_QL ? N.table : -1;
      X.age75[k] = N.mask_kind == GJ_MASK_QL_AGE75;
      if (N.mask_kind >= GJ_MASK_QL) X.leisure = 1;
    }
    if (X.leisure) {
      if (!plan->agent_class || (uintptr_t)plan->agent_class % 4 != 0) return GJ_E_PLAN;
      for (int k = 0; k < G.nk[g]; ++k)
        if (X.table[k] < 0) return GJ_E_PLAN;
    } else if (G.nk[g] != 1) {
      return GJ_E_PLAN;
    }
  }
  D.table_floats = D.table1_floats = 0;
  D._pad3 = 0;
  if (D.n_direct) {
    const int64_t budget = 160 * 1024 / 4 - 2 * kClassWeightFloats - 2 * kWave;
    int64_t largest = 0;
    for (int t = 0; t < D.n_direct; ++t) {
      const int64_t sz = (int64_t)D.direct[t].V * D.direct[t].stride;
      largest = largest > sz ? largest : sz;
    }
    int64_t cap0 = largest < budget ? largest : budget;
    if (T->direct_table_floats > 0 && T->direct_table_floats < cap0) cap0 = T->direct_table_floats;
    if (cap0 < GJ_MAX_NETS_PER_SET) cap0 = GJ_MAX_NETS_PER_SET;
    int64_t cap1 = budget - cap0;
    if (T->direct_table_floats > 0 && T->direct_table_floats < cap1) cap1 = T->direct_table_floats;
    int prev_region = -1;
    for (int t = 0; t < D.n_direct; ++t) {
      TDirect& X = D.direct[t];
      const int64_t sz = (int64_t)X.V * X.stride;
      X.region = (prev_region == 0 && sz <= cap1) ? 1 : 0;
      const int64_t cap = X.region ? cap1 : cap0;
      X.group_venues = sz <= cap ? X.V : (int32_t)(cap / X.stride);
      if (X.group_venues < 1 || (X.win_lo && sz > cap)) return GJ_E_PLAN;
      X._pad = 0;
      prev_region = X.region;
    }
    D.table_floats = (int32_t)cap0;
    D.table1_floats = (int32_t)cap1;
    const size_t direct_lds = 4 * ((size_t)2 * kClassWeightFloats + (size_t)cap0 + kWave + (size_t)cap1 + kWave);
    if (direct_lds > lds) lds = direct_lds;
  }
  {
    uintptr_t bits = (uintptr_t)D.susceptibility | (uintptr_t)D.not_infected_probs | (uintptr_t)D.new_infected |
                     (uintptr_t)D.trans_susc | (uintptr_t)D.acc_scratch | (uintptr_t)D.agent_sums;
    D.io_vec4 = (bits % 16 == 0) ? 1 : 0;
  }
  int rc = allow_lds(k_tile_agents, lds);
  if (rc) return rc;
  hipLaunchKernelGGL(k_tile_agents, dim3((unsigned)owned_slices), dim3(kTileThreads), lds, stream, D);
  rc = launch_status();
  if (rc || !D.acc_scratch) return rc;
  hipLaunchKernelGGL(k_tile_epilogue, dim3((unsigned)((plan->n_agents + 255) / 256)), dim3(256), 0, stream, D);
  return launch_status();
}

}


extern "C" {

#ifdef GJ_DIAG_STAMPS
int gj_diag_venue_stamps(unsigned long long* host_out) {
  return (int)hipMemcpyFromSymbol(host_out, HIP_SYMBOL(gj::gj_diag_venue), sizeof(unsigned long long) * 3 * gj::kDiagVenueSlots);
}
#endif

int gj_version(void) { return GJ_ABI_VERSION; }

const char* gj_error_string(int code) {
  switch (code) {
    case GJ_OK: return "ok";
    case GJ_E_NULL: return "required pointer is NULL";
    case GJ_E_RANGE: return "count or index out of range";
    case GJ_E_PLAN: return "inconsistent plan or network list";
    case GJ_E_NODEVICE: return "no HIP device, or not a gfx950 (MI355X) device";
    default: break;
  }
  if (code > 0) return hipGetErrorString((hipError_t)code);
  return "unknown error";
}

int gj_check_device(void) {
  int dev = 0;
  if (hipGetDevice(&dev) != hipSuccess) return GJ_E_NODEVICE;
  hipDeviceProp_t prop;
  if (hipGetDeviceProperties(&prop, dev) != hipSuccess) return GJ_E_NODEVICE;
  const char* want = "gfx950";
  for (int i = 0; want[i]; ++i)
    if (prop.gcnArchName[i] != want[i]) return GJ_E_NODEVICE;
  return GJ_OK;
}

int gj_transmission_update(const gj_plan* plan, const gj_agent_state* state, const gj_step_params* params,
                           void* stream) {
  int rc = gj::check_plan(plan);
  if (rc) return rc;
  if (!params) return GJ_E_NULL;
  rc = gj::check_state(plan, state, params);
  if (rc) return rc;
  return gj::do_transmission(plan, state, params, (hipStream_t)stream);
}

int gj_quarantine_transmission(const gj_plan* plan, const gj_agent_state* state, const gj_step_params* params,
                               void* stream) {
  int rc = gj::check_plan(plan);
  if (rc) return rc;
  if (!params) return GJ_E_NULL;
  rc = gj::check_state(plan, state, params, false);
  if (rc) return rc;
  if (!params->has_quarantine || plan->n_agents == 0) return GJ_OK;
  const int64_t n = plan->n_agents;
  hipLaunchKernelGGL(gj::k_quarantine_transmission, dim3((unsigned)((n + gj::kThreads - 1) / gj::kThreads)),
                     dim3(gj::kThreads), 0, (hipStream_t)stream, n, state->current_stage, state->transmission,
                     state->q_transmission, params->q_threshold);
  return gj::launch_status();
}

int gj_venue_reduce(const gj_plan* plan, const gj_agent_state* state, const gj_step_params* params, void* stream) {
  int rc = gj::check_plan(plan);
  if (rc) return rc;
  gj::Groups G;
  rc = gj::group_networks(plan, params, &G);
  if (rc) return rc;
  rc = gj::check_state(plan, state, params, false);
  if (rc) return rc;
  if (plan->tiled) {
    rc = gj::tiled_scatter(plan, state, params, G, (hipStream_t)stream);
    if (rc) return rc;
    return gj::tiled_venues(plan, state, params, G, 1, (hipStream_t)stream);
  }
  return gj::do_venue_reduce(plan, state, params, G, (hipStream_t)stream);
}

int gj_agent_gather(const gj_plan* plan, const gj_agent_state* state, const gj_step_params* params,
                    const gj_step_io* io, int sample, void* stream) {
  int rc = gj::check_plan(plan);
  if (rc) return rc;
  gj::Groups G;
  rc = gj::group_networks(plan, params, &G);
  if (rc) return rc;
  rc = gj::check_state(plan, state, params, sample != 0);
  if (rc) return rc;
  if (plan->tiled) {
    rc = gj::tiled_venues(plan, state, params, G, 2, (hipStream_t)stream);
    if (rc) return rc;
    return gj::tiled_agents(plan, state, params, G, io, sample, (hipStream_t)stream);
  }
  return gj::do_agent_gather(plan, state, params, G, io, sample, (hipStream_t)stream);
}

int gj_sample_infect(int64_t n_agents, const float* not_infected_probs, const float* exp_noise, uint64_t seed,
                     uint64_t step, int64_t agent_offset, float now, float* new_infected, float* susceptibility,
                     float* is_infected, float* infection_time, void* stream) {
  if (n_agents < 0) return GJ_E_RANGE;
  if (n_agents == 0) return GJ_OK;
  if (!not_infected_probs) return GJ_E_NULL;
  const int n_state = (susceptibility != nullptr) + (is_infected != nullptr) + (infection_time != nullptr);
  if (n_state != 0 && n_state != 3) return GJ_E_NULL;
  if (n_state == 0 && !new_infected) return GJ_E_NULL;
  const int64_t blocks = (n_agents + gj::kThreads - 1) / gj::kThreads;
  hipLaunchKernelGGL(gj::k_sample_infect, dim3((unsigned)blocks), dim3(gj::kThreads), 0, (hipStream_t)stream, n_agents,
                     not_infected_probs, exp_noise, seed, step, agent_offset, now, new_infected, susceptibility,
                     is_infected, infection_time);
  return gj::launch_status();
}

int gj_adjoint_sample(int64_t n, const float* susceptibility0, const float* infection_time0, const float* acc,
                      const float* exp_noise, uint64_t seed, uint64_t step, int64_t agent_offset, float now,
                      float delta_time, const float* g_susc, const float* g_inf, const float* g_time,
                      const float* g_new, float* x_out, float* grad_susc_out, float* grad_time_out, void* stream) {
  if (n < 0) return GJ_E_RANGE;
  if (n == 0) return GJ_OK;
  if (!susceptibility0 || !infection_time0 || !acc || !x_out || !grad_susc_out || !grad_time_out) return GJ_E_NULL;
  hipLaunchKernelGGL(gj::k_adjoint_sample, dim3((unsigned)((n + gj::kThreads - 1) / gj::kThreads)), dim3(gj::kThreads),
                     0, (hipStream_t)stream, n, susceptibility0, infection_time0, acc, exp_noise, seed, step,
                     agent_offset, now, delta_time, g_susc, g_inf, g_time, g_new, x_out, grad_susc_out, grad_time_out);
  return gj::launch_status();
}

int gj_adjoint_transmission(int64_t n, const gj_agent_state* st, float now, const float* trans_bar,
                            const float* g_inf, float* grad_inf_out, float* grad_time_inout, void* stream) {
  if (n < 0) return GJ_E_RANGE;
  if (n == 0) return GJ_OK;
  if (!st || !trans_bar || !grad_inf_out || !grad_time_inout) return GJ_E_NULL;
  if (!st->max_infectiousness || !st->shape || !st->rate || !st->shift || !st->infection_time || !st->is_infected)
    return GJ_E_NULL;
  hipLaunchKernelGGL(gj::k_adjoint_transmission, dim3((unsigned)((n + gj::kThreads - 1) / gj::kThreads)),
                     dim3(gj::kThreads), 0, (hipStream_t)stream, n, st->max_infectiousness, st->shape, st->rate,
                     st->shift, st->infection_time, st->is_infected, now, trans_bar, g_inf, grad_inf_out,
                     grad_time_inout);
  return gj::launch_status();
}

int gj_adjoint_transmission_params(int64_t n, const gj_agent_state* st, float now, const float* trans_bar,
                                   const float* g_inf, float* grad_inf_out, float* grad_time_inout,
                                   float* grad_max_infectiousness_out, float* grad_shape_out, float* grad_rate_out,
                                   float* grad_shift_out, void* stream) {
  if (n < 0) return GJ_E_RANGE;
  if (n == 0) return GJ_OK;
  if (!st || !trans_bar || !grad_inf_out || !grad_time_inout) return GJ_E_NULL;
  if (!st->max_infectiousness || !st->shape || !st->rate || !st->shift || !st->infection_time || !st->is_infected)
    return GJ_E_NULL;
  hipLaunchKernelGGL(gj::k_adjoint_transmission_params, dim3((unsigned)((n + gj::kThreads - 1) / gj::kThreads)),
                     dim3(gj::kThreads), 0, (hipStream_t)stream, n, st->max_infectiousness, st->shape, st->rate,
                     st->shift, st->infection_time, st->is_infected, now, trans_bar, g_inf, grad_inf_out,
                     grad_time_inout, grad_max_infectiousness_out, grad_shape_out, grad_rate_out, grad_shift_out);
  return gj::launch_status();
}

int gj_adjoint_beta_partial(int64_t n_venues, int32_t stride, int32_t nk, const float* cum_fwd, const float* cum_bwd,
                            const float* v_pcontact, const double* weights, const float* beta, const int32_t* cols,
                            double* partial, void* stream) {
  if (n_venues < 0 || stride < 1 || stride > GJ_MAX_NETS_PER_SET || nk < 0 || nk > stride) return GJ_E_RANGE;
  if (!partial || (nk > 0 && (!beta || !cols))) return GJ_E_NULL;
  if (n_venues == 0 || nk == 0) return GJ_OK;
  if (!cum_fwd || !cum_bwd || !v_pcontact) return GJ_E_NULL;
  gj::AdjBetaArgs A;
  A.n_venues = n_venues;
  A.stride = stride;
  A.nk = nk;
  A.cum_fwd = cum_fwd;
  A.cum_bwd = cum_bwd;
  A.v_pc = v_pcontact;
  A.weights = weights;
  for (int k = 0; k < GJ_MAX_NETS_PER_SET; ++k) {
    A.beta[k] = k < nk ? beta[k] : 0.0f;
    A.cols[k] = k < nk ? cols[k] : 0;
    if (k < nk && (cols[k] < 0 || cols[k] >= GJ_MAX_NETS)) return GJ_E_RANGE;
// ... 73 lines not shown

int gj_step_stats(int64_t n, const uint8_t* agent_class, const float* is_infected, const float* current_stage,
                  int32_t n_bins, const int32_t* bin_edges, int32_t dead_stage, double* out, void* stream) {
  if (n < 0 || n_bins < 0 || n_bins > GJ_MAX_AGE_BINS) return GJ_E_RANGE;
  if (!out || (n_bins > 0 && !bin_edges)) return GJ_E_NULL;
  if (n == 0) return GJ_OK;
  if (!agent_class || !is_infected || !current_stage) return GJ_E_NULL;
  gj::StatsArgs S;
  S.n = n;
  S.cls = agent_class;
  S.inf = is_infected;
  S.stage = current_stage;
  S.n_bins = n_bins;
  for (int b = 0; b <= GJ_MAX_AGE_BINS; ++b) S.edges[b] = (b <= n_bins) ? bin_edges[b] : 0;
  S.dead = dead_stage;
  S.out = out;
  S.vec4 = (((uintptr_t)is_infected | (uintptr_t)current_stage) % 16 == 0 && (uintptr_t)agent_class % 4 == 0) ? 1 : 0;
  int64_t blocks = ((S.vec4 ? (n >> 2) + 3 : n) + gj::kThreads - 1) / gj::kThreads;
  if (blocks > 2048) blocks = 2048;
  if (blocks < 1) blocks = 1;
  hipLaunchKernelGGL(gj::k_step_stats, dim3((unsigned)blocks), dim3(gj::kThreads), 0, (hipStream_t)stream, S);
  return gj::launch_status();
}

int gj_symptoms_step_stats(int64_t n, const uint8_t* agent_class, const float* new_infected, float* current_stage,
                           float* next_stage, float* time_to_next_stage, const gj_symptoms_params* params,
                           const float* progresses, const float* dwell, const float* is_infected, int32_t n_bins,
                           const int32_t* bin_edges, int32_t dead_stage, double* out, void* stream) {
  if (n < 0 || n_bins < 0 || n_bins > GJ_MAX_AGE_BINS) return GJ_E_RANGE;
  if (!out || (n_bins > 0 && !bin_edges)) return GJ_E_NULL;
  if (n == 0) return GJ_OK;
  if (!agent_class || !new_infected || !current_stage || !next_stage || !time_to_next_stage || !params || !is_infected)
    return GJ_E_NULL;
  if (params->n_stages < 3 || params->n_stages > GJ_MAX_STAGES) return GJ_E_RANGE;
  if ((progresses == nullptr) != (dwell == nullptr)) return GJ_E_NULL;
  if (!progresses && !params->progress) return GJ_E_NULL;
  gj::SymptomsArgs S;
  S.P = *params;
  S.n = n;
  S.cls = agent_class;
  S.new_inf = new_infected;
  S.cur = current_stage;
  S.nxt = next_stage;
  S.ttn = time_to_next_stage;
  S.progresses = progresses;
  S.dwell = dwell;
  gj::StatsArgs R;
  R.n = n;
  R.cls = agent_class;
  R.inf = is_infected;
  R.stage = current_stage;
  R.n_bins = n_bins;
  for (int b = 0; b <= GJ_MAX_AGE_BINS; ++b) R.edges[b] = (b <= n_bins) ? bin_edges[b] : 0;
  R.dead = dead_stage;
  R.out = out;
  const uintptr_t bits = (uintptr_t)new_infected | (uintptr_t)current_stage | (uintptr_t)next_stage |
                         (uintptr_t)time_to_next_stage | (uintptr_t)is_infected;
  R.vec4 = (bits % 16 == 0 && (uintptr_t)agent_class % 4 == 0) ? 1 : 0;
  int64_t blocks = ((R.vec4 ? (n >> 2) + 3 : n) + gj::kThreads - 1) / gj::kThreads;
  if (blocks > 4096) blocks = 4096;
  if (blocks < 1) blocks = 1;
  hipLaunchKernelGGL(gj::k_symptoms_stats, dim3((unsigned)blocks), dim3(gj::kThreads), 0, (hipStream_t)stream, S, R);
  return gj::launch_status();
}

int gj_group_stats(int64_t n, const int32_t* group, int32_t n_groups, const float* is_infected,
                   const float* current_stage, int32_t dead_stage, double* out, void* workspace, void* stream) {
  if (n < 0 || n_groups < 1 || n_groups > GJ_MAX_GROUPS) return GJ_E_RANGE;
  if (!out || !workspace) return GJ_E_NULL;
  if (n == 0) return GJ_OK;
  if (!group || !is_infected || !current_stage) return GJ_E_NULL;
  gj::GroupArgs S;
  S.n = n;
  S.group = group;
  S.inf = is_infected;
  S.stage = current_stage;
  S.n_groups = n_groups;
  S.dead = dead_stage;
  S.vec4 = (((uintptr_t)group | (uintptr_t)is_infected | (uintptr_t)current_stage) % 16 == 0) ? 1 : 0;
  S.ws = (gj::fx_t*)workspace;
  const int64_t units = S.vec4 ? (n >> 2) + 1 : n;
  if (n_groups <= gj::kGroupLdsMax) {
    int64_t blocks = (units + gj::kGroupLdsThreads - 1) / gj::kGroupLdsThreads;
    if (blocks > gj::kGroupLdsBlocks) blocks = gj::kGroupLdsBlocks;
    hipLaunchKernelGGL(gj::k_group_stats<true>, dim3((unsigned)blocks), dim3(gj::kGroupLdsThreads),
                       (size_t)n_groups * 2 * sizeof(gj::fx_t), (hipStream_t)stream, S);
  } else {
    int64_t blocks = (units + gj::kThreads - 1) / gj::kThreads;
    if (blocks > 2048) blocks = 2048;
    hipLaunchKernelGGL(gj::k_group_stats<false>, dim3((unsigned)blocks), dim3(gj::kThreads), 0, (hipStream_t)stream, S);
  }
  int rc = gj::launch_status();
  if (rc) return rc;
  hipLaunchKernelGGL(gj::k_group_finish, dim3((unsigned)((2 * (int64_t)n_groups + gj::kThreads - 1) / gj::kThreads)),
                     dim3(gj::kThreads), 0, (hipStream_t)stream, n_groups, S.ws, out);
  return gj::launch_status();
}

int gj_adjoint_group_stats(int64_t n, const int32_t* group, int32_t n_groups, const float* current_stage,
                           int32_t dead_stage, const float* g_cases, const float* g_deaths, float* grad_is_infected,
                           float* grad_stage, void* stream) {
  if (n < 0 || n_groups < 1 || n_groups > GJ_MAX_GROUPS) return GJ_E_RANGE;
  if (grad_stage && dead_stage == 0) return GJ_E_RANGE;
  if (n == 0 || (!grad_is_infected && !grad_stage)) return GJ_OK;
  if (!group || (grad_stage && !current_stage)) return GJ_E_NULL;
  gj::GroupAdjArgs S;
  S.n = n;
  S.group = group;
  S.stage = current_stage;
  S.g_cases = g_cases;
  S.g_deaths = g_deaths;
  S.grad_inf = grad_is_infected;
  S.grad_stage = grad_stage;
  S.n_groups = n_groups;
  S.dead = dead_stage;
  const uintptr_t bits = (uintptr_t)group | (uintptr_t)grad_is_infected | (uintptr_t)grad_stage |
                         (grad_stage ? (uintptr_t)current_stage : 0);
  S.vec4 = (bits % 16 == 0) ? 1 : 0;
  int64_t blocks = ((S.vec4 ? (n >> 2) + 3 : n) + gj::kThreads - 1) / gj::kThreads;
  if (blocks > 2048) blocks = 2048;
  if (blocks < 1) blocks = 1;
  if (n_groups <= gj::kGroupAdjLdsMax)
    hipLaunchKernelGGL(gj::k_adjoint_group_stats<true>, dim3((unsigned)blocks), dim3(gj::kThreads),
                       (size_t)n_groups * 2 * sizeof(float), (hipStream_t)stream, S);
  else
    hipLaunchKernelGGL(gj::k_adjoint_group_stats<false>, dim3((unsigned)blocks), dim3(gj::kThreads), 0,
                       (hipStream_t)stream, S);
  return gj::launch_status();
}

int gj_step(const gj_plan* plan, const gj_agent_state* state, const gj_step_params* params, const gj_step_io* io,
            void* stream) {
  int rc = gj::check_plan(plan);
  if (rc) return rc;
  gj::Groups G;
  rc = gj::group_networks(plan, params, &G);
  if (rc) return rc;
  rc = gj::check_state(plan, state, params);
  if (rc) return rc;
  rc = gj::do_transmission(plan, state, params, (hipStream_t)stream);
  if (rc) return rc;
  if (plan->tiled) {
    rc = gj::tiled_scatter(plan, state, params, G, (hipStream_t)stream);
    if (rc) return rc;
    rc = gj::tiled_venues(plan, state, params, G, 0, (hipStream_t)stream);
    if (rc) return rc;
    return gj::tiled_agents(plan, state, params, G, io, 1, (hipStream_t)stream);
  }
  rc = gj::do_venue_reduce(plan, state, params, G, (hipStream_t)stream);
  if (rc) return rc;
  return gj::do_agent_gather(plan, state, params, G, io, 1, (hipStream_t)stream);
}

int gj_step_phase(const gj_plan* plan, const gj_agent_state* state, const gj_step_params* params,
                  const gj_step_io* io, int phase, void* stream) {
  int rc = gj::check_plan(plan);
  if (rc) return rc;
  gj::Groups G;
  rc = gj::group_networks(plan, params, &G);
  if (rc) return rc;
  rc = gj::check_state(plan, state, params, phase == 0 || phase == 3);
  if (rc) return rc;
  hipStream_t st = (hipStream_t)stream;
  switch (phase) {
    case 0: return gj::do_transmission(plan, state, params, st);
    case 1: return plan->tiled ? gj::tiled_scatter(plan, state, params, G, st)
                               : gj::do_venue_reduce(plan, state, params, G, st);
    case 2: return plan->tiled ? gj::tiled_venues(plan, state, params, G, 0, st) : GJ_OK;
    case 3: return plan->tiled ? gj::tiled_agents(plan, state, params, G, io, 1, st)
                               : gj::do_agent_gather(plan, state, params, G, io, 1, st);
    case 4: return plan->tiled ? gj::tiled_agents(plan, state, params, G, io, 0, st)
                               : gj::do_agent_gather(plan, state, params, G, io, 0, st);
    case 5: return plan->tiled ? gj::tiled_venues(plan, state, params, G, 1, st) : GJ_OK;
    case 6: return plan->tiled ? gj::tiled_venues(plan, state, params, G, 2, st) : GJ_OK;
    case 7:
    case 8:
      if (!plan->tiled) return gj::do_venue_reduce(plan, state, params, G, st);
      rc = gj::tiled_scatter(plan, state, params, G, st);
      if (rc) return rc;
      return gj::tiled_venues(plan, state, params, G, phase == 7 ? 1 : 0, st);
    default: return GJ_E_RANGE;
  }
}

namespace gj {
__global__ void k_clock_advance(gj_clock* clock, double delta_now) {
  const uint64_t step = clock->step + 1;
  clock->step = step;
  clock->now = (float)(clock->now0 + (double)(int64_t)(step - clock->step0) * delta_now);
}
}

int gj_clock_advance(gj_clock* clock, double delta_now, void* stream) {
  if (!clock) return GJ_E_NULL;
  hipLaunchKernelGGL(gj::k_clock_advance, dim3(1), dim3(1), 0, (hipStream_t)stream, clock, delta_now);
  return gj::launch_status();
}

int gj_pack_f32(int64_t n, const int32_t* index, const float* src, float* out, void* stream) {
  if (n < 0) return GJ_E_RANGE;
  if (n == 0) return GJ_OK;
  if (!index || !src || !out) return GJ_E_NULL;
  hipLaunchKernelGGL(gj::k_pack, dim3((unsigned)((n + gj::kThreads - 1) / gj::kThreads)), dim3(gj::kThreads), 0,
                     (hipStream_t)stream, n, index, src, out);
  return gj::launch_status();
}

int gj_unpack_f32(int64_t n, const int32_t* index, const float* in, float* dst, void* stream) {
  if (n < 0) return GJ_E_RANGE;
  if (n == 0) return GJ_OK;
  if (!index || !in || !dst) return GJ_E_NULL;
  hipLaunchKernelGGL(gj::k_unpack, dim3((unsigned)((n + gj::kThreads - 1) / gj::kThreads)), dim3(gj::kThreads), 0,
                     (hipStream_t)stream, n, index, in, dst);
  return gj::launch_status();
}

int gj_event_create(void** event) {
  if (!event) return GJ_E_NULL;
  hipEvent_t e;
  const hipError_t rc = hipEventCreate(&e);
  if (rc != hipSuccess) return (int)rc;
  *event = (void*)e;
  return GJ_OK;
}
int gj_event_record(void* event, void* stream) {
  if (!event) return GJ_E_NULL;
  return (int)hipEventRecord((hipEvent_t)event, (hipStream_t)stream);
}
int gj_event_elapsed_ms(void* start, void* stop, float* ms) {
  if (!start || !stop || !ms) return GJ_E_NULL;
  hipError_t rc = hipEventSynchronize((hipEvent_t)stop);
  if (rc != hipSuccess) return (int)rc;
  return (int)hipEventElapsedTime(ms, (hipEvent_t)start, (hipEvent_t)stop);
}
int gj_event_destroy(void* event) {
  if (!event) return GJ_E_NULL;
  return (int)hipEventDestroy((hipEvent_t)event);
}

}
```

### gradabm-june_amd/grad_june_amd/_native.py

```python
from __future__ import annotations

import ctypes as C
import os
from typing import Optional

GJ_ABI_VERSION = 7
GJ_MAX_SETS = 12
GJ_MAX_NETS = 16
GJ_MAX_NETS_PER_SET = 8
GJ_TABLE_SIZE = 400
GJ_ADJ_BETA_BLOCKS = 256
GJ_STREAM_EDGES = 2048
GJ_MAX_GROUPS = 1 << 28
GJ_GROUP_ERR_LABEL, GJ_GROUP_ERR_VALUE = 1, 2

MASK_RAW, MASK_Q, MASK_QL, MASK_QL_AGE75 = 0, 1, 2, 3

_LIB_DIR = os.path.join(os.path.dirname(os.path.abspath(__file__)), "lib")
LIB_PATH = os.environ.get("GJ_LIB_PATH") or os.path.join(_LIB_DIR, "libgradjune_hip.so")

_vp = C.c_void_p


class EdgeSet(C.Structure):
    _fields_ = [
        ("n_venues", C.c_int64),
        ("n_edges", C.c_int64),
        ("v_rowptr", _vp),
        ("v_agent", _vp),
        ("v_pcontact", _vp),
        ("a_rowptr", _vp),
        ("a_venue", _vp),
        ("cum", _vp),
        ("cum_stride", C.c_int32),
        ("_pad", C.c_int32),
    ]


class TiledSet(C.Structure):
    _fields_ = [
        ("n_blocks", C.c_int32),
        ("max_block_venues", C.c_int32),
        ("desc_wide", C.c_int32),
        ("ell_k", C.c_int32),
        ("blk_v0", _vp),
        ("blk_e0", _vp),
        ("e_lv", _vp),
        ("e_cls", _vp),
        ("a_la", _vp),
        ("tile_sptr", _vp),
        ("tile_jpos", _vp),
        ("chunk_ptr", _vp),
        ("chunk_desc", _vp),
        ("val", _vp),
        ("ell", _vp),
        ("run_pv_blk", _vp),
        ("run_pv_win", _vp),
        ("run_blk_r0", _vp),
        ("run_win_lo", _vp),
        ("run_win_n", _vp),
        ("run_max_window", C.c_int32),
        ("run_tiled_edges", C.c_int32),
        ("presum", _vp),
        ("multi_slots", _vp),
        ("max_venue_edges", C.c_int32),
        ("_pad_mve", C.c_int32),
    ]


class Tiled(C.Structure):
    _fields_ = [
        ("n_slices", C.c_int32),
        ("slice_agents", C.c_int32),
        ("direct_table_floats", C.c_int32),
        ("n_work", C.c_int32),
        ("work", _vp),
        ("agent_scratch", _vp),
        ("presum_wgs", C.c_int32),
        ("_pad_presum", C.c_int32),
        ("sets", TiledSet * GJ_MAX_SETS),
    ]


class Plan(C.Structure):
    _fields_ = [
        ("n_agents", C.c_int64),
        ("n_ext_agents", C.c_int64),
        ("n_sets", C.c_int32),
        ("n_blocks", C.c_int32),
        ("n_long_rows", C.c_int32),
        ("n_partial_slots", C.c_int32),
        ("sets", EdgeSet * GJ_MAX_SETS),
        ("blocks", _vp),
        ("long_rows", _vp),
        ("partial", _vp),
        ("agent_class", _vp),
        ("tables", _vp),
        ("n_tables", C.c_int32),
        ("_pad", C.c_int32),
        ("tiled", C.POINTER(Tiled)),
    ]


class Network(C.Structure):
    _fields_ = [
        ("beta", C.c_float),
        ("set", C.c_int32),
        ("mask_kind", C.c_int32),
        ("table", C.c_int32),
    ]


class StepParams(C.Structure):
    _fields_ = [
        ("now", C.c_float),
        ("delta_time", C.c_float),
        ("day_type", C.c_int32),
        ("has_quarantine", C.c_int32),
        ("q_threshold", C.c_float),
        ("n_nets", C.c_int32),
        ("seed", C.c_uint64),
        ("step", C.c_uint64),
        ("agent_offset", C.c_int64),
        ("transpose", C.c_int32),
        ("_pad", C.c_int32),
        ("nets", Network * GJ_MAX_NETS),
        ("clock", _vp),
    ]


class AgentState(C.Structure):
    _fields_ = [
        ("max_infectiousness", _vp),
        ("shape", _vp),
        ("rate", _vp),
        ("shift", _vp),
        ("infection_time", _vp),
        ("is_infected", _vp),
        ("susceptibility", _vp),
        ("transmission", _vp),
        ("q_transmission", _vp),
        ("current_stage", _vp),
    ]


class StepIO(C.Structure):
    _fields_ = [
        ("not_infected_probs", _vp),
        ("new_infected", _vp),
        ("exp_noise", _vp),
        ("trans_susc", _vp),
        ("agent_sums", _vp),
    ]


GJ_MAX_STAGES = 16


class SymptomsParams(C.Structure):
    _fields_ = [
        ("n_stages", C.c_int32),
        ("_pad", C.c_int32),
        ("progress", _vp),
        ("next_kind", C.c_int32 * GJ_MAX_STAGES),
        ("next_loc", C.c_float * GJ_MAX_STAGES),
        ("next_scale", C.c_float * GJ_MAX_STAGES),
        ("rec_kind", C.c_int32 * GJ_MAX_STAGES),
        ("rec_loc", C.c_float * GJ_MAX_STAGES),
        ("rec_scale", C.c_float * GJ_MAX_STAGES),
        ("time", C.c_float),
        ("_pad2", C.c_float),
        ("seed", C.c_uint64),
        ("step", C.c_uint64),
        ("agent_offset", C.c_int64),
    ]


SYMBOLS = {
    "gj_version": (C.c_int, []),
    "gj_error_string": (C.c_char_p, [C.c_int]),
    "gj_check_device": (C.c_int, []),
    "gj_transmission_update": (C.c_int, [C.POINTER(Plan), C.POINTER(AgentState), C.POINTER(StepParams), _vp]),
    "gj_quarantine_transmission": (C.c_int, [C.POINTER(Plan), C.POINTER(AgentState), C.POINTER(StepParams), _vp]),
    "gj_venue_reduce": (C.c_int, [C.POINTER(Plan), C.POINTER(AgentState), C.POINTER(StepParams), _vp]),
    "gj_agent_gather": (
        C.c_int,
        [C.POINTER(Plan), C.POINTER(AgentState), C.POINTER(StepParams), C.POINTER(StepIO), C.c_int, _vp],
    ),
    "gj_sample_infect": (
        C.c_int,
        [C.c_int64, _vp, _vp, C.c_uint64, C.c_uint64, C.c_int64, C.c_float, _vp, _vp, _vp, _vp, _vp],
    ),
    "gj_adjoint_sample": (
        C.c_int,
        [C.c_int64, _vp, _vp, _vp, _vp, C.c_uint64, C.c_uint64, C.c_int64, C.c_float, C.c_float, _vp, _vp, _vp, _vp,
         _vp, _vp, _vp, _vp],
    ),
    "gj_adjoint_transmission": (C.c_int, [C.c_int64, C.POINTER(AgentState), C.c_float, _vp, _vp, _vp, _vp, _vp]),
    "gj_adjoint_transmission_params": (
        C.c_int, [C.c_int64, C.POINTER(AgentState), C.c_float, _vp, _vp, _vp, _vp, _vp, _vp, _vp, _vp, _vp]),
    "gj_adjoint_beta_partial": (
        C.c_int,
        [C.c_int64, C.c_int32, C.c_int32, _vp, _vp, _vp, _vp, C.POINTER(C.c_float), C.POINTER(C.c_int32), _vp, _vp],
    ),
    "gj_adjoint_beta_finish": (C.c_int, [C.c_int32, _vp, _vp, _vp, _vp]),
    "gj_symptoms_update": (
        C.c_int,
        [C.c_int64, _vp, _vp, _vp, _vp, _vp, C.POINTER(SymptomsParams), _vp, _vp, _vp],
    ),
    "gj_adjoint_symptoms": (
        C.c_int,
        [C.c_int64, _vp, _vp, _vp, _vp, _vp, C.POINTER(SymptomsParams)] + [_vp] * 10,
    ),
    "gj_step_stats": (C.c_int, [C.c_int64, _vp, _vp, _vp, C.c_int32, C.POINTER(C.c_int32), C.c_int32, _vp, _vp]),
    "gj_group_stats": (C.c_int, [C.c_int64, _vp, C.c_int32, _vp, _vp, C.c_int32, _vp, _vp, _vp]),
    "gj_adjoint_group_stats": (C.c_int, [C.c_int64, _vp, C.c_int32, _vp, C.c_int32, _vp, _vp, _vp, _vp, _vp]),
    "gj_step": (C.c_int, [C.POINTER(Plan), C.POINTER(AgentState), C.POINTER(StepParams), C.POINTER(StepIO), _vp]),
    "gj_step_phase": (
        C.c_int,
        [C.POINTER(Plan), C.POINTER(AgentState), C.POINTER(StepParams), C.POINTER(StepIO), C.c_int, _vp],
    ),
    "gj_clock_advance": (C.c_int, [_vp, C.c_double, _vp]),
    "gj_symptoms_step_stats": (
        C.c_int,
        [C.c_int64, _vp, _vp, _vp, _vp, _vp, C.POINTER(SymptomsParams), _vp, _vp, _vp, C.c_int32, C.POINTER(C.c_int32),
         C.c_int32, _vp, _vp],
    ),
    "gj_pack_f32": (C.c_int, [C.c_int64, _vp, _vp, _vp, _vp]),
    "gj_unpack_f32": (C.c_int, [C.c_int64, _vp, _vp, _vp, _vp]),
    "gj_event_create": (C.c_int, [C.POINTER(_vp)]),
    "gj_event_record": (C.c_int, [_vp, _vp]),
    "gj_event_elapsed_ms": (C.c_int, [_vp, _vp, C.POINTER(C.c_float)]),
    "gj_event_destroy": (C.c_int, [_vp]),
}

GJ_COMPILE_COUNTS = 16
GJ_CC_BLOCKS, GJ_CC_SLOTS, GJ_CC_CHUNKS, GJ_CC_MULTI, GJ_CC_OWNED_EDGES, GJ_CC_MAX_DEGREE, GJ_CC_ERROR = 0, 1, 2, 3, 4, 5, 7
GJ_CC_RUN_PRIMARY, GJ_CC_RUN_UNSORTED, GJ_CC_RUN_WINDOW, GJ_CC_WIDE_MULTI = 8, 9, 10, 11


class CompileSet(C.Structure):
    _fields_ = [
        ("agent", _vp), ("venue", _vp), ("agent_class", _vp),
        ("n_edges", C.c_int64), ("n_agents", C.c_int64), ("n_ext_agents", C.c_int64),
        ("n_venues", C.c_int32), ("n_slices", C.c_int32), ("slice_agents", C.c_int32),
        ("sv_max", C.c_int32), ("eb_target", C.c_int32), ("n_blocks", C.c_int32),
    ]


class CompileOut(C.Structure):
    _fields_ = [
        ("blk_e0", _vp), ("e_lv", _vp), ("e_cls", _vp), ("a_la", _vp), ("tile_sptr", _vp), ("tile_jpos", _vp),
        ("chunk_ptr", _vp), ("chunk_desc", _vp), ("slots_cap", C.c_int64), ("chunks_cap", C.c_int64),
    ]


_i64p = C.POINTER(C.c_int64)
SYMBOLS.update({
    "gj_compile_capacity": (C.c_int, [C.POINTER(CompileSet), _i64p, _i64p, _i64p]),
    "gj_compile_workspace_bytes": (C.c_int, [C.POINTER(CompileSet), _i64p]),
    "gj_compile_blocks": (C.c_int, [C.POINTER(CompileSet), _vp, C.c_int32, _vp, _vp, C.c_int64, _vp]),
    "gj_compile_tiles": (C.c_int, [C.POINTER(CompileSet), _vp, C.POINTER(CompileOut), _vp, _vp, C.c_int64, _vp]),
    "gj_compile_wide_descriptors": (C.c_int, [C.POINTER(CompileSet), C.POINTER(CompileOut), C.c_int32, _vp, _vp, _vp]),
    "gj_compile_ell_degrees": (C.c_int, [C.POINTER(CompileSet), _vp, _vp, _vp]),
    "gj_compile_explicit_slots": (C.c_int, [C.POINTER(CompileSet), C.POINTER(CompileOut), _vp, _vp]),
    "gj_compile_multi_slots": (C.c_int, [C.POINTER(CompileSet), C.POINTER(CompileOut), C.c_int32, C.c_int32, _vp,
                                          C.c_int32, _vp, _vp, _vp, C.c_int64, _vp]),
    "gj_compile_runs_pick": (C.c_int, [C.POINTER(CompileSet), _vp, _vp, _vp, _vp, _vp, _vp, _vp]),
    "gj_compile_runs_rest": (C.c_int, [C.POINTER(CompileSet), _vp, _vp, _vp, _vp, C.c_int64, _vp, _vp]),
    "gj_compile_runs_index": (C.c_int, [C.POINTER(CompileSet), _vp, _vp, C.c_int32, C.c_int64, _vp, _vp, _vp, _vp, _vp]),
    "gj_compile_ell": (C.c_int, [C.POINTER(CompileSet), C.c_int32, C.c_int64, _vp, _vp, _vp, C.c_int64, _vp, _vp]),
})

_lib: Optional[C.CDLL] = None


class NativeLibraryMissing(RuntimeError):
    pass


def load() -> C.CDLL:
    global _lib
    if _lib is not None:
        return _lib
    if not os.path.exists(LIB_PATH):
        raise NativeLibraryMissing(
            f"{LIB_PATH} not found: build it with `python __graft_entry__.py` (hipcc --offload-arch=gfx950). "
            "grad_june_amd has no CPU or eager-PyTorch fallback for the infection path."
        )
    lib = C.CDLL(LIB_PATH)
    for name, (restype, argtypes) in SYMBOLS.items():
        fn = getattr(lib, name)
        fn.restype = restype
        fn.argtypes = argtypes
    if lib.gj_version() != GJ_ABI_VERSION:
        raise RuntimeError(f"libgradjune_hip ABI {lib.gj_version()} != binding {GJ_ABI_VERSION}")
    _lib = lib
    return lib


def check(code: int, what: str) -> None:
    if code != 0:
        msg = load().gj_error_string(code)
        raise RuntimeError(f"{what} failed: [{code}] {msg.decode() if msg else '?'}")


def ptr(t) -> Optional[int]:
    if t is None:
        return None
    return t.data_ptr()


def current_stream() -> Optional[int]:
    import torch

    try:
        return torch._C._cuda_getCurrentRawStream(torch._C._cuda_getDevice())
    except AttributeError:
        return torch.cuda.current_stream().cuda_stream
```

### gradabm-june_amd/grad_june_amd/autograd.py

```python
from __future__ import annotations

import ctypes as C
from typing import List

import torch

import os

from . import _native as N
from .engine import AgentBuffers
from .plan import SPLIT_SUFFIX
from .transmission import PROFILE

KEEP_FORWARD_SUMS = os.environ.get("GJ_BACKWARD_RECOMPUTE", "0") in ("", "0")


def _keep_sums(env) -> bool:
    return bool(env.get("keep_sums", KEEP_FORWARD_SUMS))


def _ones(plan, n):
    t = getattr(plan, "_adjoint_ones", None)
    if t is None or t.numel() != n:
        t = torch.ones(n, dtype=torch.float32, device=plan.device)
        plan._adjoint_ones = t
    return t


def _clone_forward_cum(plan, nets):
    cum_fwd = {}
    for _, names in _names_with_twins(plan, nets):
        for name in names:
            es = plan.networks[name].edge_set
            if es not in cum_fwd:
                cum_fwd[es] = plan.cum_of(es).clone()
    return cum_fwd


def _forward_sums(engine, p, bufs, acc, nets, compute_transmission: bool):
    plan = engine.plan
    io = engine.io(trans_susc=acc)
    p.transpose = 0
    if compute_transmission:
        engine.step_phase(bufs, p, io, 0)
    else:
        engine.quarantine_transmission(bufs, p)
    engine.step_phase(bufs, p, io, 8)
    cum_fwd = _clone_forward_cum(plan, nets)
    engine.step_phase(bufs, p, io, 4)
    return cum_fwd


def _transposed_passes(engine, p, bufs, scratch, x, nets, betas, cum_fwd):
    plan = engine.plan
    n = plan.host.n_agents
    lo, hi = torch.aminmax(x)
    scale = _power_of_two_scale(torch.maximum(-lo, hi))
    torch.div(x, scale, out=scratch[:n])
    tbar = torch.empty(n, dtype=torch.float32, device=plan.device)
    io_t = engine.io(trans_susc=tbar)
    p.transpose = 1
    try:
        engine.quarantine_transmission(bufs, p)
        engine.step_phase(bufs, p, io_t, 8)
        grads = [g.to(torch.float32) for g in _beta_gradients(plan, nets, betas, cum_fwd, scale)]
        engine.step_phase(bufs, p, io_t, 4)
    finally:
        p.transpose = 0
    return tbar.mul_(scale), grads


def _names_with_twins(plan, nets):
    return [(net, [nm for nm in (net.name, net.name + SPLIT_SUFFIX) if nm in plan.networks]) for net in nets]


def _beta_gradients(plan, nets, betas, cum_fwd, scale, weights_of=None) -> List[torch.Tensor]:
    lib, dev = N.load(), plan.device
    partial = torch.zeros(N.GJ_ADJ_BETA_BLOCKS * N.GJ_MAX_NETS, dtype=torch.float64, device=dev)
    out = torch.zeros(max(1, len(nets)), dtype=torch.float64, device=dev)
    per_set, per_set_k = {}, {}
    for col, (net, names) in enumerate(_names_with_twins(plan, nets)):
        for name in names:
            es = plan.networks[name].edge_set
            k = per_set_k.get(es, 0)
            per_set_k[es] = k + 1
            per_set.setdefault(es, []).append((k, col, float(betas[net.name])))
    scale32 = scale.to(device=dev, dtype=torch.float32).reshape(1)
    keep = []
    for es, items in per_set.items():
        i = plan.host.set_index[es]
        nk = len(items)
        assert [k for k, _, _ in items] == list(range(nk))
        beta = (C.c_float * nk)(*[b for _, _, b in items])
        cols = (C.c_int32 * nk)(*[c for _, c, _ in items])
        w = weights_of(es) if weights_of is not None else None
        if w is not None:
            w = w.to(device=dev, dtype=torch.float64).contiguous()
        fwd, bwd = cum_fwd[es].contiguous(), plan.cum_of(es)
        keep.append((w, fwd))
        N.check(lib.gj_adjoint_beta_partial(plan.host.sets[i].n_venues, int(plan.c.sets[i].cum_stride), nk, N.ptr(fwd),
                                            N.ptr(bwd), N.ptr(plan.keep[i]["v_pc"]), N.ptr(w), beta, cols, N.ptr(partial),
                                            N.current_stream()), "gj_adjoint_beta_partial")
    N.check(lib.gj_adjoint_beta_finish(len(nets), N.ptr(partial), N.ptr(scale32), N.ptr(out), N.current_stream()),
            "gj_adjoint_beta_finish")
    return [out[i] for i in range(len(nets))]


def _power_of_two_scale(peak: torch.Tensor) -> torch.Tensor:
    scale = torch.where((peak > 0) & torch.isfinite(peak), torch.exp2(torch.ceil(torch.log2(peak.clamp_min(1e-45)))),
                        torch.ones_like(peak))
    return torch.where(torch.isfinite(scale) & (scale > 0), scale, torch.ones_like(scale))


def _param_grads(nets, grads):
    out = []
    for net, g in zip(nets, grads):
        lb = net.log_beta
        out.append(g.to(lb.device).reshape(lb.shape) if isinstance(lb, torch.Tensor) and lb.requires_grad else None)
    return out


def _adjoint_profile(n, st0, now, tbar, g_inf, grad_inf, grad_time, want, dev):
    lib = N.load()
    if not any(want):
        N.check(lib.gj_adjoint_transmission(n, C.byref(st0.c), float(now), N.ptr(tbar), N.ptr(g_inf), N.ptr(grad_inf),
                                            N.ptr(grad_time), N.current_stream()), "gj_adjoint_transmission")
        return [None] * len(PROFILE)
    outs = [torch.empty(n, dtype=torch.float32, device=dev) if w else None for w in want]
    N.check(lib.gj_adjoint_transmission_params(n, C.byref(st0.c), float(now), N.ptr(tbar), N.ptr(g_inf),
                                               N.ptr(grad_inf), N.ptr(grad_time), *[N.ptr(o) for o in outs],
                                               N.current_stream()), "gj_adjoint_transmission_params")
    return outs


def _profile_wanted(ctx, n_nets):
    flags = tuple(ctx.needs_input_grad[4 + n_nets:])
    return flags if flags else (False,) * len(PROFILE)


def _profile_grads(ctx, n_nets, grads):
    if len(ctx.needs_input_grad) <= 4 + n_nets:
        return []
    return [None if g is None else g.to(dev) for g, dev in zip(grads, ctx.profile_devices)]


class HotPathStep(torch.autograd.Function):

    @staticmethod
    def forward(ctx, env, susc, inf, time, *log_betas_and_profile):
        engine, params, fixed, stage, exp_noise, nets = (env[k] for k in ("engine", "params", "fixed", "stage",
                                                                           "exp_noise", "nets"))
        ctx.profile_devices = [t.device for t in log_betas_and_profile[len(nets):]]
        plan = engine.plan
        n = plan.host.n_agents
        out_s, out_i, out_t = (t.detach().to(torch.float32).clone().contiguous() for t in (susc, inf, time))
        n_ext = plan.host.n_ext_agents
        trans = (torch.empty if n_ext == n else torch.zeros)(n_ext, dtype=torch.float32, device=plan.device)
        new_inf = torch.empty(n, dtype=torch.float32, device=plan.device)
        bufs = AgentBuffers(plan, **fixed, infection_time=out_t, is_infected=out_i, susceptibility=out_s,
                            transmission=trans, current_stage=stage)
        keep = _keep_sums(env) and plan.c.tiled is not None and bool(plan.c.tiled)
        acc = torch.empty(n, dtype=torch.float32, device=plan.device) if keep else None
        engine.step(bufs, params, engine.io(new_infected=new_inf, exp_noise=exp_noise, agent_sums=acc))
        ctx.env = env
        ctx.save_for_backward(susc.detach().to(torch.float32).contiguous(), inf.detach().to(torch.float32).contiguous(),
                              time.detach().to(torch.float32).contiguous())
        ctx.transmission = trans
        ctx.kept = (acc, _clone_forward_cum(plan, nets)) if keep else None
        return out_s, out_i, out_t, new_inf

    @staticmethod
    def backward(ctx, g_susc, g_inf, g_time, g_new):
        env = ctx.env
        engine, params, fixed, stage, exp_noise, nets = (env[k] for k in ("engine", "params", "fixed", "stage",
                                                                           "exp_noise", "nets"))
        susc0, inf0, time0 = ctx.saved_tensors
        plan, lib, dev = engine.plan, N.load(), engine.plan.device
        n = plan.host.n_agents
        if plan.c.tiled is None or not bool(plan.c.tiled):
            raise NotImplementedError("the backward pass runs on the tiled layout")

        def f32(g):
            return None if g is None else g.detach().to(torch.float32).contiguous()

        g_susc, g_inf, g_time, g_new = f32(g_susc), f32(g_inf), f32(g_time), f32(g_new)
        ones = _ones(plan, n)
        n_ext = plan.host.n_ext_agents
        scratch = (torch.empty if n_ext == n else torch.zeros)(n_ext, dtype=torch.float32, device=dev)
        bufs = AgentBuffers(plan, **fixed, infection_time=time0, is_infected=inf0, susceptibility=ones,
                            transmission=scratch, current_stage=stage)
        p = params
        if ctx.kept is not None:
            acc, cum_fwd = ctx.kept
        else:
            acc = torch.empty(n, dtype=torch.float32, device=dev)
            cum_fwd = _forward_sums(engine, p, bufs, acc, nets, compute_transmission=True)
        x = torch.empty(n, dtype=torch.float32, device=dev)
        grad_susc = torch.empty(n, dtype=torch.float32, device=dev)
        grad_time = torch.empty(n, dtype=torch.float32, device=dev)
        N.check(lib.gj_adjoint_sample(n, N.ptr(susc0), N.ptr(time0), N.ptr(acc), N.ptr(exp_noise), int(p.seed),
                                      int(p.step), int(p.agent_offset), float(p.now), float(p.delta_time),
                                      N.ptr(g_susc), N.ptr(g_inf), N.ptr(g_time), N.ptr(g_new), N.ptr(x),
                                      N.ptr(grad_susc), N.ptr(grad_time), N.current_stream()), "gj_adjoint_sample")
        tbar, grads = _transposed_passes(engine, p, bufs, scratch, x, nets, env["betas"], cum_fwd)
        grad_inf = torch.empty(n, dtype=torch.float32, device=dev)
        st0 = AgentBuffers(plan, **fixed, infection_time=time0, is_infected=inf0, susceptibility=ones,
                           transmission=scratch)
        pg = _adjoint_profile(n, st0, p.now, tbar, g_inf, grad_inf, grad_time, _profile_wanted(ctx, len(nets)), dev)
        return (None, grad_susc, grad_inf, grad_time, *_param_grads(nets, grads), *_profile_grads(ctx, len(nets), pg))


class DistributedHotPathStep(torch.autograd.Function):

    @staticmethod
    def forward(ctx, env, susc, inf, time, *log_betas_and_profile):
        hp, params_of, fixed, stage, exp_noise = (env[k] for k in ("hp", "params_of", "fixed", "stage", "exp_noise"))
        ctx.profile_devices = [t.device for t in log_betas_and_profile[len(env["nets"]):]]
        plan = hp.engine.plan
        n = plan.host.n_agents
        out_s, out_i, out_t = (t.detach().to(torch.float32).clone().contiguous() for t in (susc, inf, time))
        new_inf = torch.empty(n, dtype=torch.float32, device=plan.device)
        bufs = AgentBuffers(plan, **fixed, infection_time=out_t, is_infected=out_i, susceptibility=out_s,
                            transmission=hp.state["transmission"], q_transmission=hp.state["q_transmission"],
                            current_stage=stage)
        keep = _keep_sums(env)
        acc = torch.empty(n, dtype=torch.float32, device=plan.device) if keep else None
        hp.run_step(bufs, hp.engine.io(new_infected=new_inf, exp_noise=exp_noise, agent_sums=acc), params_of)
        ctx.env = env
        ctx.save_for_backward(susc.detach().to(torch.float32).contiguous(), inf.detach().to(torch.float32).contiguous(),
                              time.detach().to(torch.float32).contiguous())
        ctx.kept = (acc, _clone_forward_cum(plan, env["nets"])) if keep else None
        return out_s, out_i, out_t, new_inf

    @staticmethod
    def backward(ctx, g_susc, g_inf, g_time, g_new):
        env = ctx.env
        hp, params_of, fixed, stage, exp_noise, nets = (env[k] for k in ("hp", "params_of", "fixed", "stage",
                                                                          "exp_noise", "nets"))
        susc0, inf0, time0 = ctx.saved_tensors
        engine = hp.engine
        plan, lib, dev = engine.plan, N.load(), engine.plan.device
        n, n_ext = plan.host.n_agents, plan.host.n_ext_agents
        p = params_of(None)

        def f32(g):
            return None if g is None else g.detach().to(torch.float32).contiguous()

        g_susc, g_inf, g_time, g_new = f32(g_susc), f32(g_inf), f32(g_time), f32(g_new)
        ones = _ones(plan, n)
        scratch = torch.zeros(n_ext, dtype=torch.float32, device=dev)
        scratch_q = torch.zeros(n_ext, dtype=torch.float32, device=dev) if p.has_quarantine else None
        bufs = AgentBuffers(plan, **fixed, infection_time=time0, is_infected=inf0, susceptibility=ones,
                            transmission=scratch, q_transmission=scratch_q, current_stage=stage)
        if ctx.kept is not None:
            acc, cum_fwd = ctx.kept
        else:
            acc = torch.empty(n, dtype=torch.float32, device=dev)
            cum_fwd = {}

            def keep_forward_sums():
                cum_fwd.update(_clone_forward_cum(plan, nets))

            p.transpose = 0
            engine.step_phase(bufs, p, engine.io(trans_susc=acc), 0)
            hp.sparse_passes(bufs, engine.io(trans_susc=acc), p, between=keep_forward_sums)
        x = torch.empty(n, dtype=torch.float32, device=dev)
        grad_susc = torch.empty(n, dtype=torch.float32, device=dev)
        grad_time = torch.empty(n, dtype=torch.float32, device=dev)
        N.check(lib.gj_adjoint_sample(n, N.ptr(susc0), N.ptr(time0), N.ptr(acc), N.ptr(exp_noise), int(p.seed),
                                      int(p.step), int(p.agent_offset), float(p.now), float(p.delta_time),
                                      N.ptr(g_susc), N.ptr(g_inf), N.ptr(g_time), N.ptr(g_new), N.ptr(x),
                                      N.ptr(grad_susc), N.ptr(grad_time), N.current_stream()), "gj_adjoint_sample")
        scale = _power_of_two_scale(hp.all_reduce_max(x.abs().max().reshape(1)).reshape(()))
        scratch.zero_()
        scratch[:n].copy_(x / scale)
        tbar = torch.empty(n, dtype=torch.float32, device=dev)
        grads: List[torch.Tensor] = []

        def beta_gradients():
            grads.extend(_beta_gradients(plan, nets, env["betas"], cum_fwd, scale, weights_of=hp.venue_weights))

        p.transpose = 1
        try:
            engine.quarantine_transmission(bufs, p)
            hp.sparse_passes(bufs, engine.io(trans_susc=tbar), p, between=beta_gradients)
        finally:
            p.transpose = 0
        tbar = tbar * scale
        total = hp.all_reduce_sum(torch.stack(grads)) if grads else None
        grads32 = [total[i].to(torch.float32) for i in range(len(grads))]
        grad_inf = torch.empty(n, dtype=torch.float32, device=dev)
        st0 = AgentBuffers(plan, **fixed, infection_time=time0, is_infected=inf0, susceptibility=ones,
                           transmission=scratch)
        pg = _adjoint_profile(n, st0, p.now, tbar, g_inf, grad_inf, grad_time, _profile_wanted(ctx, len(nets)), dev)
        return (None, grad_susc, grad_inf, grad_time, *_param_grads(nets, grads32), *_profile_grads(ctx, len(nets), pg))


class TransmissionProfile(torch.autograd.Function):

    @staticmethod
    def forward(ctx, env, mx, shape, rate, shift, time, inf):
        engine, p = env["engine"], env["params"]
        plan = engine.plan
        n, dev = plan.host.n_agents, plan.device
        f = lambda t: t.detach().to(device=dev, dtype=torch.float32).contiguous()
        vals = [f(t) for t in (mx, shape, rate, shift, time, inf)]
        out = torch.empty(n, dtype=torch.float32, device=dev)
        bufs = AgentBuffers(plan, **dict(zip(PROFILE, vals[:4])), infection_time=vals[4], is_infected=vals[5],
                            susceptibility=_ones(plan, n), transmission=out)
        engine.transmission_update(bufs, p)
        ctx.engine, ctx.now = engine, float(p.now)
        ctx.devices = [t.device for t in (mx, shape, rate, shift, time, inf)]
        ctx.save_for_backward(*vals)
        return out

    @staticmethod
# ... 155 lines not shown
```

### gradabm-june_amd/grad_june_amd/engine.py

```python
from __future__ import annotations

import ctypes as C
import math
from typing import Dict, Optional, Sequence

import torch

from . import _native as N
from .plan import DevicePlan


class AgentBuffers:

    _F32 = ("max_infectiousness", "shape", "rate", "shift", "infection_time", "is_infected",
            "susceptibility", "transmission")

    def __init__(self, plan: DevicePlan, *, max_infectiousness=None, shape=None, rate=None, shift=None,
                 infection_time=None, is_infected=None, susceptibility, transmission, q_transmission=None,
                 current_stage=None):
        n, n_ext = plan.host.n_agents, plan.host.n_ext_agents
        self.tensors = dict(max_infectiousness=max_infectiousness, shape=shape, rate=rate, shift=shift,
                            infection_time=infection_time, is_infected=is_infected,
                            susceptibility=susceptibility, transmission=transmission,
                            q_transmission=q_transmission, current_stage=current_stage)
        for k, t in self.tensors.items():
            if t is None:
                continue
            want = n_ext if k in ("transmission", "q_transmission") else n
            if t.dtype != torch.float32 or not t.is_contiguous() or t.device != plan.device or t.numel() != want:
                raise ValueError(f"{k}: need contiguous float32[{want}] on {plan.device}, got "
                                 f"{t.dtype}[{tuple(t.shape)}] on {t.device}")
        c = N.AgentState()
        for k, t in self.tensors.items():
            setattr(c, k, N.ptr(t))
        self.c = c


class StepClock:

    def __init__(self, device):
        self.lib = N.load()
        self.buf = torch.zeros(4, dtype=torch.int64, device=device)

    @property
    def ptr(self) -> int:
        return self.buf.data_ptr()

    def set(self, now: float, step: int) -> None:
        import numpy as np

        host = np.zeros(4, dtype=np.int64)
        host.view(np.float32)[0] = now
        host[1] = step
        host.view(np.float64)[2] = now
        host[3] = step
        self.buf.copy_(torch.from_numpy(host))

    def read(self):
        host = self.buf.cpu().numpy()
        return float(host.view("float32")[0]), int(host[1])

    def advance(self, delta_now: float) -> None:
        N.check(self.lib.gj_clock_advance(self.ptr, float(delta_now), N.current_stream()), "gj_clock_advance")


class InfectionEngine:
    def __init__(self, plan: DevicePlan):
        self.lib = N.load()
        self.plan = plan
        self._q_trans: Optional[torch.Tensor] = None

    def q_transmission_buffer(self) -> torch.Tensor:
        if self._q_trans is None:
            self._q_trans = torch.zeros(self.plan.host.n_ext_agents, dtype=torch.float32, device=self.plan.device)
        return self._q_trans

    def params(self, *, now: float, delta_time: float, day_type: int, active: Sequence[str],
               betas: Dict[str, float], has_quarantine: bool = False, q_threshold: float = math.inf,
               seed: int = 0, step: int = 0, agent_offset: int = 0) -> N.StepParams:
        if len(active) > N.GJ_MAX_NETS:
            raise ValueError(f"at most {N.GJ_MAX_NETS} active networks")
        p = N.StepParams()
        p.now, p.delta_time, p.day_type = float(now), float(delta_time), int(day_type)
        p.has_quarantine = 1 if has_quarantine else 0
        p.q_threshold = float(q_threshold)
        p.seed, p.step, p.agent_offset = int(seed), int(step), int(agent_offset)
        p.n_nets = len(active)
        for i, name in enumerate(active):
            spec = self.plan.networks[name]
            p.nets[i].beta = float(betas[name])
            p.nets[i].set = self.plan.host.set_index[spec.edge_set]
            p.nets[i].mask_kind = spec.mask_kind
            p.nets[i].table = self.plan.table_index.get(name, -1)
        return p

    @staticmethod
    def io(not_infected_probs=None, new_infected=None, exp_noise=None, trans_susc=None, agent_sums=None) -> N.StepIO:
        io = N.StepIO()
        io.not_infected_probs = N.ptr(not_infected_probs)
        io.new_infected = N.ptr(new_infected)
        io.exp_noise = N.ptr(exp_noise)
        io.trans_susc = N.ptr(trans_susc)
        io.agent_sums = N.ptr(agent_sums)
        io._keep = (not_infected_probs, new_infected, exp_noise, trans_susc, agent_sums)
        return io

    def _prep(self, bufs: AgentBuffers, p: N.StepParams):
        if p.has_quarantine and bufs.tensors["q_transmission"] is None:
            bufs.tensors["q_transmission"] = self.q_transmission_buffer()
            bufs.c.q_transmission = bufs.tensors["q_transmission"].data_ptr()

    def transmission_update(self, bufs: AgentBuffers, p: N.StepParams):
        self._prep(bufs, p)
        N.check(self.lib.gj_transmission_update(C.byref(self.plan.c), C.byref(bufs.c), C.byref(p),
                                                N.current_stream()), "gj_transmission_update")

    def quarantine_transmission(self, bufs: AgentBuffers, p: N.StepParams):
        self._prep(bufs, p)
        N.check(self.lib.gj_quarantine_transmission(C.byref(self.plan.c), C.byref(bufs.c), C.byref(p),
                                                    N.current_stream()), "gj_quarantine_transmission")

    def venue_reduce(self, bufs: AgentBuffers, p: N.StepParams):
        self._prep(bufs, p)
        N.check(self.lib.gj_venue_reduce(C.byref(self.plan.c), C.byref(bufs.c), C.byref(p),
                                         N.current_stream()), "gj_venue_reduce")

    def agent_gather(self, bufs: AgentBuffers, p: N.StepParams, io: N.StepIO, sample: bool):
        self._prep(bufs, p)
        N.check(self.lib.gj_agent_gather(C.byref(self.plan.c), C.byref(bufs.c), C.byref(p), C.byref(io),
                                         1 if sample else 0, N.current_stream()), "gj_agent_gather")

    def step(self, bufs: AgentBuffers, p: N.StepParams, io: N.StepIO):
        self._prep(bufs, p)
        N.check(self.lib.gj_step(C.byref(self.plan.c), C.byref(bufs.c), C.byref(p), C.byref(io),
                                 N.current_stream()), "gj_step")

    def step_phase(self, bufs: AgentBuffers, p: N.StepParams, io: N.StepIO, phase: int):
        self._prep(bufs, p)
        N.check(self.lib.gj_step_phase(C.byref(self.plan.c), C.byref(bufs.c), C.byref(p), C.byref(io), int(phase),
                                       N.current_stream()), "gj_step_phase")

    def sample_infect(self, not_infected_probs, *, now: float, susceptibility, is_infected, infection_time,
                      exp_noise=None, new_infected=None, seed: int = 0, step: int = 0, agent_offset: int = 0):
        n = not_infected_probs.numel()
        N.check(self.lib.gj_sample_infect(n, N.ptr(not_infected_probs), N.ptr(exp_noise), int(seed), int(step),
                                          int(agent_offset), float(now), N.ptr(new_infected),
                                          N.ptr(susceptibility), N.ptr(is_infected), N.ptr(infection_time),
                                          N.current_stream()), "gj_sample_infect")


class HipTimer:

    def __init__(self):
        self.lib = N.load()
        self.a, self.b = C.c_void_p(), C.c_void_p()
        N.check(self.lib.gj_event_create(C.byref(self.a)), "gj_event_create")
        N.check(self.lib.gj_event_create(C.byref(self.b)), "gj_event_create")

    def start(self):
        N.check(self.lib.gj_event_record(self.a, N.current_stream()), "gj_event_record")

    def stop(self):
        N.check(self.lib.gj_event_record(self.b, N.current_stream()), "gj_event_record")

    def elapsed_ms(self) -> float:
        ms = C.c_float()
        N.check(self.lib.gj_event_elapsed_ms(self.a, self.b, C.byref(ms)), "gj_event_elapsed_ms")
        return float(ms.value)

    def __del__(self):
        try:
            self.lib.gj_event_destroy(self.a)
            self.lib.gj_event_destroy(self.b)
        except Exception:
            pass
```

### include/gradjune_hip.h

```cpp
#ifndef GRADJUNE_HIP_H
#define GRADJUNE_HIP_H

#include <stdint.h>

#ifdef __cplusplus
extern "C" {
#endif

#define GJ_ABI_VERSION 7

#define GJ_MAX_SETS 12
#define GJ_MAX_NETS 16
#define GJ_MAX_NETS_PER_SET 8
#define GJ_TABLE_SIZE 400

#define GJ_OK 0
#define GJ_E_NULL (-1)
#define GJ_E_RANGE (-2)
#define GJ_E_PLAN (-3)
#define GJ_E_NODEVICE (-4)

typedef enum gj_mask_kind {
  GJ_MASK_RAW = 0,
  GJ_MASK_Q = 1,
  GJ_MASK_QL = 2,
  GJ_MASK_QL_AGE75 = 3
} gj_mask_kind;

typedef struct gj_edge_set {
  int64_t n_venues;
  int64_t n_edges;
  const int32_t* v_rowptr;
  const int32_t* v_agent;
  const float* v_pcontact;
  const int32_t* a_rowptr;
  const int32_t* a_venue;
  float* cum;
  int32_t cum_stride;
  int32_t _pad;
} gj_edge_set;

typedef struct gj_block {
  int32_t set;
  int32_t kind;
  int32_t v0, v1;
  int32_t e0, e1;
  int32_t slot;
  int32_t lanes;
} gj_block;

typedef struct gj_long_row {
  int32_t set;
  int32_t v;
  int32_t slot0, slot1;
} gj_long_row;

#define GJ_STREAM_EDGES 2048

typedef struct gj_tiled_set {
  int32_t n_blocks;
  int32_t max_block_venues;
  int32_t desc_wide;
  int32_t ell_k;
  const int32_t* blk_v0;
  const int32_t* blk_e0;
  const uint16_t* e_lv;
  const uint8_t* e_cls;
  const uint16_t* a_la;
  const int32_t* tile_sptr;
  const int32_t* tile_jpos;
  const int32_t* chunk_ptr;
  const int32_t* chunk_desc;
  float* val;
  const uint16_t* ell;
  const uint16_t* run_pv_blk;
  const uint16_t* run_pv_win;
  const int32_t* run_blk_r0;
  const int32_t* run_win_lo;
  const int32_t* run_win_n;
  int32_t run_max_window;
  int32_t run_tiled_edges;
  int64_t* presum;
  const int32_t* multi_slots;
  int32_t max_venue_edges;
  int32_t _pad_mve;
} gj_tiled_set;

typedef struct gj_tiled {
  int32_t n_slices;
  int32_t slice_agents;
  int32_t direct_table_floats;
  int32_t n_work;
  const int32_t* work;
  float* agent_scratch;
  int32_t presum_wgs;
  int32_t _pad_presum;
  gj_tiled_set sets[GJ_MAX_SETS];
} gj_tiled;

typedef struct gj_plan {
  int64_t n_agents;
  int64_t n_ext_agents;
  int32_t n_sets;
  int32_t n_blocks;
  int32_t n_long_rows;
  int32_t n_partial_slots;
  gj_edge_set sets[GJ_MAX_SETS];
  const gj_block* blocks;
  const gj_long_row* long_rows;
  float* partial;
  const uint8_t* agent_class;
  const float* tables;
  int32_t n_tables;
  int32_t _pad;
  const gj_tiled* tiled;
} gj_plan;

typedef struct gj_network {
  float beta;
  int32_t set;
  int32_t mask_kind;
  int32_t table;
} gj_network;

typedef struct gj_clock {
  float now;
  float _pad;
  uint64_t step;
  double now0;
  uint64_t step0;
} gj_clock;

typedef struct gj_step_params {
  float now;
  float delta_time;
  int32_t day_type;
  int32_t has_quarantine;
  float q_threshold;
  int32_t n_nets;
  uint64_t seed;
  uint64_t step;
  int64_t agent_offset;
  int32_t transpose;
  int32_t _pad;
  gj_network nets[GJ_MAX_NETS];
  const gj_clock* clock;
} gj_step_params;

typedef struct gj_agent_state {
  const float* max_infectiousness;
  const float* shape;
  const float* rate;
  const float* shift;
  float* infection_time;
  float* is_infected;
  float* susceptibility;
  float* transmission;
  float* q_transmission;
  const float* current_stage;
} gj_agent_state;

int gj_version(void);
const char* gj_error_string(int code);

int gj_check_device(void);

typedef struct gj_step_io {
  float* not_infected_probs;
  float* new_infected;
  const float* exp_noise;
  float* trans_susc;
  float* agent_sums;
} gj_step_io;

int gj_transmission_update(const gj_plan* plan, const gj_agent_state* state,
                           const gj_step_params* params, void* stream);

int gj_quarantine_transmission(const gj_plan* plan, const gj_agent_state* state,
                               const gj_step_params* params, void* stream);

int gj_venue_reduce(const gj_plan* plan, const gj_agent_state* state,
                    const gj_step_params* params, void* stream);

int gj_agent_gather(const gj_plan* plan, const gj_agent_state* state,
                    const gj_step_params* params, const gj_step_io* io, int sample,
                    void* stream);

int gj_sample_infect(int64_t n_agents, const float* not_infected_probs, const float* exp_noise,
                     uint64_t seed, uint64_t step, int64_t agent_offset, float now,
                     float* new_infected, float* susceptibility, float* is_infected,
                     float* infection_time, void* stream);

#define GJ_MAX_STAGES 16
typedef struct gj_symptoms_params {
  int32_t n_stages;
  int32_t _pad;
  const float* progress;
  int32_t next_kind[GJ_MAX_STAGES];
  float next_loc[GJ_MAX_STAGES];
  float next_scale[GJ_MAX_STAGES];
  int32_t rec_kind[GJ_MAX_STAGES];
  float rec_loc[GJ_MAX_STAGES];
  float rec_scale[GJ_MAX_STAGES];
  float time;
  float _pad2;
  uint64_t seed, step;
  int64_t agent_offset;
} gj_symptoms_params;

int gj_symptoms_update(int64_t n, const uint8_t* agent_class, const float* new_infected,
                       float* current_stage, float* next_stage, float* time_to_next_stage,
                       const gj_symptoms_params* params, const float* progresses, const float* dwell,
                       void* stream);

#define GJ_MAX_AGE_BINS 8
int gj_step_stats(int64_t n, const uint8_t* agent_class, const float* is_infected,
                  const float* current_stage, int32_t n_bins, const int32_t* bin_edges ,
                  int32_t dead_stage, double* out, void* stream);

int gj_symptoms_step_stats(int64_t n, const uint8_t* agent_class, const float* new_infected,
                           float* current_stage, float* next_stage, float* time_to_next_stage,
                           const gj_symptoms_params* params, const float* progresses, const float* dwell,
                           const float* is_infected, int32_t n_bins, const int32_t* bin_edges ,
                           int32_t dead_stage, double* out, void* stream);

#define GJ_MAX_GROUPS (1 << 28)
#define GJ_GROUP_WORKSPACE_BYTES(n_groups) (16 * (int64_t)(n_groups) + 8)
#define GJ_GROUP_ERR_LABEL 1u
#define GJ_GROUP_ERR_VALUE 2u
int gj_group_stats(int64_t n, const int32_t* group, int32_t n_groups, const float* is_infected,
                   const float* current_stage, int32_t dead_stage, double* out, void* workspace, void* stream);

int gj_adjoint_group_stats(int64_t n, const int32_t* group, int32_t n_groups, const float* current_stage,
                           int32_t dead_stage, const float* g_cases, const float* g_deaths, float* grad_is_infected,
                           float* grad_stage, void* stream);

int gj_adjoint_sample(int64_t n, const float* susceptibility0, const float* infection_time0, const float* acc,
                      const float* exp_noise, uint64_t seed, uint64_t step, int64_t agent_offset, float now,
                      float delta_time, const float* g_susc, const float* g_inf, const float* g_time,
                      const float* g_new, float* x_out, float* grad_susc_out, float* grad_time_out,
                      void* stream);
int gj_adjoint_transmission(int64_t n, const gj_agent_state* state0, float now, const float* trans_bar,
                            const float* g_inf, float* grad_inf_out, float* grad_time_inout, void* stream);
int gj_adjoint_transmission_params(int64_t n, const gj_agent_state* state0, float now, const float* trans_bar,
                                   const float* g_inf, float* grad_inf_out, float* grad_time_inout,
                                   float* grad_max_infectiousness_out, float* grad_shape_out, float* grad_rate_out,
                                   float* grad_shift_out, void* stream);

#define GJ_ADJ_BETA_BLOCKS 256
int gj_adjoint_beta_partial(int64_t n_venues, int32_t stride, int32_t nk, const float* cum_fwd, const float* cum_bwd,
                            const float* v_pcontact, const double* weights, const float* beta ,
                            const int32_t* cols , double* partial, void* stream);
int gj_adjoint_beta_finish(int32_t n_cols, const double* partial, const float* scale, double* out, void* stream);

int gj_adjoint_symptoms(int64_t n, const uint8_t* agent_class, const float* new_infected,
                        const float* current_stage0, const float* next_stage0, const float* time_to_next_stage0,
                        const gj_symptoms_params* params, const float* progresses, const float* dwell,
                        const float* g_current, const float* g_next, const float* g_time, float* g_current_in,
                        float* g_next_in, float* g_time_in, float* g_new_infected, void* stream);

int gj_step(const gj_plan* plan, const gj_agent_state* state, const gj_step_params* params,
            const gj_step_io* io, void* stream);

int gj_step_phase(const gj_plan* plan, const gj_agent_state* state, const gj_step_params* params,
                  const gj_step_io* io, int phase, void* stream);

int gj_clock_advance(gj_clock* clock, double delta_now, void* stream);

int gj_pack_f32(int64_t n, const int32_t* index, const float* src, float* out, void* stream);
int gj_unpack_f32(int64_t n, const int32_t* index, const float* in, float* dst, void* stream);

#define GJ_COMPILE_COUNTS 16
#define GJ_CC_BLOCKS 0
#define GJ_CC_SLOTS 1
#define GJ_CC_CHUNKS 2
#define GJ_CC_MULTI 3
#define GJ_CC_OWNED_EDGES 4
#define GJ_CC_MAX_DEGREE 5
#define GJ_CC_ERROR 7
#define GJ_CC_RUN_PRIMARY 8
#define GJ_CC_RUN_UNSORTED 9
#define GJ_CC_RUN_WINDOW 10
#define GJ_CC_WIDE_MULTI 11

typedef struct gj_compile_set {
  const int64_t* agent;
  const int64_t* venue;
  const uint8_t* agent_class;
  int64_t n_edges;
  int64_t n_agents;
  int64_t n_ext_agents;
  int32_t n_venues;
  int32_t n_slices, slice_agents;
  int32_t sv_max, eb_target;
  int32_t n_blocks;
} gj_compile_set;

typedef struct gj_compile_out {
  int32_t* blk_e0;
  uint16_t* e_lv;
  uint8_t* e_cls;
  uint16_t* a_la;
  int32_t* tile_sptr;
  int32_t* tile_jpos;
  int32_t* chunk_ptr;
  int32_t* chunk_desc;
  int64_t slots_cap, chunks_cap;
} gj_compile_out;

int gj_compile_capacity(const gj_compile_set* set, int64_t* blk_cap, int64_t* slots_cap, int64_t* chunks_cap);
int gj_compile_workspace_bytes(const gj_compile_set* set, int64_t* bytes);
int gj_compile_blocks(const gj_compile_set* set, int32_t* blk_v0 , int32_t blk_cap,
                      int32_t* counts, void* workspace, int64_t workspace_bytes, void* stream);
int gj_compile_tiles(const gj_compile_set* set, const int32_t* blk_v0, const gj_compile_out* out, int32_t* counts,
                     void* workspace, int64_t workspace_bytes, void* stream);
int gj_compile_wide_descriptors(const gj_compile_set* set, const gj_compile_out* out, int32_t n_chunks,
                                int32_t* desc8 , int32_t* counts, void* stream);
int gj_compile_ell_degrees(const gj_compile_set* set, int32_t* degree, int32_t* counts, void* stream);
int gj_compile_ell(const gj_compile_set* set, int32_t ell_k, int64_t rows, const int32_t* degree, uint16_t* ell,
                   void* workspace, int64_t workspace_bytes, int32_t* counts, void* stream);

int gj_compile_explicit_slots(const gj_compile_set* set, const gj_compile_out* out, int32_t* slots, void* stream);
int gj_compile_multi_slots(const gj_compile_set* set, const gj_compile_out* out, int32_t n_chunks, int32_t wide,
                           int32_t* desc, int32_t n_multi, int32_t* multi_slots, int32_t* counts, void* workspace,
                           int64_t workspace_bytes, void* stream);

int gj_compile_runs_pick(const gj_compile_set* set, int32_t* vmin, int32_t* pick, uint8_t* keep, int32_t* win_lo,
// ... 17 lines not shown
```

Before: 2051.

## Fuse scatter, venue and agent phases into one persistent cooperative kernel

Adds a persistent kernel k_tile_step that runs the scatter, venue-reduce and agent-gather phases in a single cooperative launch. Phases are separated by software grid barriers over global atomics, and venue work items are handed out dynamically through an atomic head counter. The aim is to remove per-kernel launch overhead and the tails between phases. In exchange it adds barrier spin cost with a timeout path, a max-LDS footprint across phases that can lower occupancy, and heuristics that fall back to separate launches when there are too few work items.

New measurement: 1993. 0.972x the previous value.

```diff
diff --git a/gradabm-june_amd/csrc/gj_tiled.h b/gradabm-june_amd/csrc/gj_tiled.h
--- a/gradabm-june_amd/csrc/gj_tiled.h
+++ b/gradabm-june_amd/csrc/gj_tiled.h
@@ -115,14 +115,16 @@
   const int32_t* multi_slots;
 };
 
-struct TileAArgs {
-  TSetA sets[GJ_MAX_SETS];
+template <int NS>
+struct TileAArgsT {
+  TSetA sets[NS];
   int32_t n_sets;
   int32_t slice_agents;
   int64_t n_agents;
   const float* trans;
   const float* qtrans;
 };
+typedef TileAArgsT<GJ_MAX_SETS> TileAArgs;
 
 __device__ __forceinline__ void load_slice(float* lds, const float* __restrict__ src, int64_t base, int n_local,
                                            int tid) {
@@ -467,11 +469,9 @@
 #ifndef GJ_SCATTER_WAVES_PER_SIMD
 #define GJ_SCATTER_WAVES_PER_SIMD 4
 #endif
-__global__ __launch_bounds__(kTileThreads, GJ_SCATTER_WAVES_PER_SIMD) void k_tile_scatter(const TileAArgs A) {
-  extern __shared__ __align__(16) float lds_x[];
-  const int tid = threadIdx.x;
+template <class Args>
+__device__ __forceinline__ void tile_scatter_body(const Args& A, const int s, float* lds_x, const int tid) {
   const int wave = __builtin_amdgcn_readfirstlane(tid / kWave), lane = tid % kWave;
-  const int s = blockIdx.x;
   const int64_t base = (int64_t)s * A.slice_agents;
   const int n_local = (int)min((int64_t)A.slice_agents, A.n_agents - base);
   const bool two_sources = A.qtrans != A.trans;
@@ -496,6 +496,10 @@
       }
     }
   }
+}
+__global__ __launch_bounds__(kTileThreads, GJ_SCATTER_WAVES_PER_SIMD) void k_tile_scatter(const TileAArgs A) {
+  extern __shared__ __align__(16) float lds_x[];
+  tile_scatter_body(A, (int)blockIdx.x, lds_x, (int)threadIdx.x);
 }
 
 struct TSetB {
@@ -521,8 +525,9 @@
   int64_t n_x;
 };
 
-struct TileBArgs {
-  TSetB sets[GJ_MAX_SETS];
+template <int NS>
+struct TileBArgsT {
+  TSetB sets[NS];
   const int32_t* work;
   const float* tables;
   int32_t day_type;
@@ -530,6 +535,7 @@
   int32_t transpose;
   int32_t _pad;
 };
+typedef TileBArgsT<GJ_MAX_SETS> TileBArgs;
 
 __device__ __noinline__ void venue_group_slow(fx_t* sums, uint32_t* vflags, int words, uint32_t limit, int base_k, int l0,
                                               int l1, int l2, int l3, int l4, int l5, int l6, int l7, float x0, float x1,
@@ -571,13 +577,9 @@
 #ifndef GJ_VENUE_WAVES_PER_SIMD
 #define GJ_VENUE_WAVES_PER_SIMD 4
 #endif
-__global__ __launch_bounds__(kTileThreads, GJ_VENUE_WAVES_PER_SIMD) void k_tile_venues(const TileBArgs B) {
-  extern __shared__ __align__(16) float lds_s[];
-#ifdef GJ_DIAG_STAMPS
-  VenueStamp gj_stamp;
-#endif
-  const int tid = threadIdx.x;
-  const int set = B.work[2 * blockIdx.x], j = B.work[2 * blockIdx.x + 1];
+template <class Args>
+__device__ __forceinline__ void tile_venues_body(const Args& B, const int item, float* lds_s, const int tid) {
+  const int set = B.work[2 * item], j = B.work[2 * item + 1];
   const TSetB& T = B.sets[set];
   const int nk = T.nk;
   if (nk == 0) return;
@@ -823,6 +825,13 @@
       store_nt(val4 + 2 * gu + 1, make_float4(r[4], r[5], r[6], r[7]));
     }
   }
+}
+__global__ __launch_bounds__(kTileThreads, GJ_VENUE_WAVES_PER_SIMD) void k_tile_venues(const TileBArgs B) {
+  extern __shared__ __align__(16) float lds_s[];
+#ifdef GJ_DIAG_STAMPS
+  VenueStamp gj_stamp;
+#endif
+  tile_venues_body(B, (int)blockIdx.x, lds_s, (int)threadIdx.x);
 }
 
 constexpr int GJ_MAX_PRESUM = 6;
@@ -1034,8 +1043,9 @@
   const int32_t* win_n;
 };
 
-struct TileDArgs {
-  TSetA sets[GJ_MAX_SETS];
+template <int NS>
+struct TileDArgsT {
+  TSetA sets[NS];
   int32_t n_sets;
   int32_t slice_agents;
   int64_t n_agents;
@@ -1053,7 +1063,7 @@
   int64_t agent_offset;
   float* acc_scratch;
   float* agent_sums;
-  TDirect direct[GJ_MAX_DIRECT];
+  TDirect direct[NS];
   int32_t n_direct;
   int32_t table_floats;
   int32_t table1_floats;
@@ -1065,6 +1075,7 @@
   int32_t _pad2;
   int32_t io_vec4;
 };
+typedef TileDArgsT<GJ_MAX_SETS> TileDArgs;
 
 __global__ __launch_bounds__(256) void k_tile_epilogue(const TileDArgs D) {
   const int64_t a = (int64_t)blockIdx.x * blockDim.x + threadIdx.x;
@@ -1104,7 +1115,8 @@
   uint32_t cls[kQuadsPerLane];
 };
 
-__device__ __forceinline__ void direct_load(const TileDArgs& D, const TDirect& T, int64_t base, int n_local, int tid,
+template <class Args>
+__device__ __forceinline__ void direct_load(const Args& D, const TDirect& T, int64_t base, int n_local, int tid,
                                             int plane, DirectBatch& b) {
   const unsigned last_quad = (unsigned)(n_local - 1) >> 2;
   const uint16_t* ell = T.ell + plane * T.plane_stride + base * 2;
@@ -1130,7 +1142,8 @@
   }
 }
 
-__device__ __forceinline__ void direct_add(const TileDArgs& D, const TDirect& T, float (&acc)[kQuadsPerLane][4],
+template <class Args>
+__device__ __forceinline__ void direct_add(const Args& D, const TDirect& T, float (&acc)[kQuadsPerLane][4],
                                            uint32_t qmask, const float* wtab, const float* tab, int v0, int nv,
                                            int n_local, int tid, const DirectBatch& b) {
   constexpr int K = 2;
@@ -1185,7 +1198,8 @@
   }
 }
 
-__device__ __forceinline__ void direct_stage(const TileDArgs& D, const TDirect& T, float* wtab, float* tab, int v0,
+template <class Args>
+__device__ __forceinline__ void direct_stage(const Args& D, const TDirect& T, float* wtab, float* tab, int v0,
                                              int nv, int tid) {
   if (T.leisure && v0 == 0) {
     for (int i = tid; i < T.nk * 200; i += kTileThreads) {
@@ -1218,7 +1232,8 @@
   __syncthreads();
 }
 
-__device__ __forceinline__ bool direct_next(const TileDArgs& D, int& t, int& v0, int& plane) {
+template <class Args>
+__device__ __forceinline__ bool direct_next(const Args& D, int& t, int& v0, int& plane) {
   const TDirect& T = D.direct[t];
   if (plane + 1 < T.planes) {
     ++plane;
@@ -1234,15 +1249,16 @@
   return t < D.n_direct;
 }
 
-__device__ __forceinline__ void direct_sets(const TileDArgs& D, float (&acc)[kQuadsPerLane][4], uint32_t qmask,
+template <class Args>
+__device__ __forceinline__ void direct_sets(const Args& D, float (&acc)[kQuadsPerLane][4], uint32_t qmask,
                                             float* lds, int64_t base, int n_local, int tid, DirectBatch& cur,
-                                            uint64_t diag_t0 = 0) {
+                                            const int s, uint64_t diag_t0 = 0) {
   auto wtab_of = [&](int t) { return lds + (t & 1) * kClassWeightFloats; };
   auto tab_of = [&](const TDirect& T) {
     return lds + 2 * kClassWeightFloats + (T.region ? D.table_floats + kWave : 0);
   };
-  auto group_nv = [&](const TDirect& T, int v0) { return T.win_lo ? T.win_n[blockIdx.x] : min(T.group_venues, T.V - v0); };
-  auto group_lo = [&](const TDirect& T, int v0) { return T.win_lo ? T.win_lo[blockIdx.x] : v0; };
+  auto group_nv = [&](const TDirect& T, int v0) { return T.win_lo ? T.win_n[s] : min(T.group_venues, T.V - v0); };
+  auto group_lo = [&](const TDirect& T, int v0) { return T.win_lo ? T.win_lo[s] : v0; };
   int t = 0, v0 = 0, plane = 0;
   __syncthreads();
   direct_stage(D, D.direct[0], wtab_of(0), tab_of(D.direct[0]), group_lo(D.direct[0], 0), group_nv(D.direct[0], 0), tid);
@@ -1253,7 +1269,7 @@
     if (plane == 0) publish_staged();
 #ifdef GJ_DIAG_STAMPS
     if (threadIdx.x == 0 && D.trans_susc && t < 4)
-      D.trans_susc[(int64_t)blockIdx.x * D.slice_agents + 8 + 2 * t] = (float)(__builtin_amdgcn_s_memtime() - diag_t0);
+      D.trans_susc[(int64_t)s * D.slice_agents + 8 + 2 * t] = (float)(__builtin_amdgcn_s_memtime() - diag_t0);
 #endif
     int tn = t, vn = v0, pn = plane;
     more = direct_next(D, tn, vn, pn);
@@ -1270,7 +1286,7 @@
 #endif
 #ifdef GJ_DIAG_STAMPS
     if (threadIdx.x == 0 && D.trans_susc && t < 4)
-      D.trans_susc[(int64_t)blockIdx.x * D.slice_agents + 9 + 2 * t] = (float)(__builtin_amdgcn_s_memtime() - diag_t0);
+      D.trans_susc[(int64_t)s * D.slice_agents + 9 + 2 * t] = (float)(__builtin_amdgcn_s_memtime() - diag_t0);
 #endif
     if (new_group && !overlap) {
       __syncthreads();
@@ -1314,20 +1330,18 @@
 #define GJ_STAMP(k)                                                                                         \
   do {                                                                                                      \
     if (threadIdx.x == 0 && D.trans_susc)                                                                    \
-      D.trans_susc[(int64_t)blockIdx.x * D.slice_agents + (k)] = (float)(__builtin_amdgcn_s_memtime() - gj_t0); \
+      D.trans_susc[(int64_t)s * D.slice_agents + (k)] = (float)(__builtin_amdgcn_s_memtime() - gj_t0);         \
   } while (0)
 #else
 #define GJ_STAMP(k) do { } while (0)
 #endif
 
-__global__ __launch_bounds__(kTileThreads) void k_tile_agents(const TileDArgs D) {
-  extern __shared__ __align__(16) fx_t lds_acc[];
+template <class Args>
+__device__ __forceinline__ void tile_agents_body(const Args& D, const int s, fx_t* lds_acc, const int tid) {
 #ifdef GJ_DIAG_STAMPS
   const uint64_t gj_t0 = __builtin_amdgcn_s_memtime();
 #endif
-  const int tid = threadIdx.x;
   const int wave = __builtin_amdgcn_readfirstlane(tid / kWave), lane = tid % kWave;
-  const int s = blockIdx.x;
   const int64_t base = (int64_t)s * D.slice_agents;
   const int n_local = (int)min((int64_t)D.slice_agents, D.n_agents - base);
   uint32_t* lds_flags = reinterpret_cast<uint32_t*>(lds_acc + D.slice_agents);
@@ -1408,9 +1422,9 @@
     GJ_STAMP(2);
 #ifndef GJ_DIAG_NO_DIRECT_SETS
 #ifdef GJ_DIAG_STAMPS
-    direct_sets(D, acc, qmask, reinterpret_cast<float*>(lds_acc), base, n_local, tid, first, gj_t0);
+    direct_sets(D, acc, qmask, reinterpret_cast<float*>(lds_acc), base, n_local, tid, first, s, gj_t0);
 #else
-    direct_sets(D, acc, qmask, reinterpret_cast<float*>(lds_acc), base, n_local, tid, first);
+    direct_sets(D, acc, qmask, reinterpret_cast<float*>(lds_acc), base, n_local, tid, first, s);
 #endif
 #endif
     GJ_STAMP(3);
@@ -1557,5 +1571,101 @@
 #endif
   GJ_STAMP(5);
 }
-
-}
+__global__ __launch_bounds__(kTileThreads) void k_tile_agents(const TileDArgs D) {
+  extern __shared__ __align__(16) fx_t lds_acc[];
+  tile_agents_body(D, (int)blockIdx.x, lds_acc, (int)threadIdx.x);
+}
+
+constexpr int kFusedSets = 6;
+enum { kCtlHead = 0, kCtlBarrier = 1, kCtlExit = 2, kCtlError = GJ_STEP_CTL_ERROR_WORD };
+constexpr unsigned long long kBarrierTicks = 5000000ull;
+
+struct FusedCtl {
+  uint32_t* words;
+  int32_t grid;
+  int32_t first, last;
+  int32_t n_a, n_b, n_d;
+  int32_t head_word;
+  int32_t _pad;
+};
+
+__device__ __forceinline__ bool grid_barrier(const FusedCtl& C, uint32_t target, uint32_t* lds_word, bool lane0) {
+  asm volatile("s_waitcnt vmcnt(0)" ::: "memory");
+  __syncthreads();
+  if (lane0) {
+    __builtin_amdgcn_fence(__ATOMIC_RELEASE, "agent");
+    asm volatile("s_waitcnt vmcnt(0)" ::: "memory");
+    __hip_atomic_fetch_add(&C.words[kCtlBarrier], 1u, __ATOMIC_RELAXED, __HIP_MEMORY_SCOPE_AGENT);
+    const unsigned long long t0 = __builtin_amdgcn_s_memrealtime();
+    uint32_t ok = 1u;
+    while (__hip_atomic_load(&C.words[kCtlBarrier], __ATOMIC_RELAXED, __HIP_MEMORY_SCOPE_AGENT) < target) {
+      __builtin_amdgcn_s_sleep(4);
+      const bool late = __builtin_amdgcn_s_memrealtime() - t0 > kBarrierTicks;
+      if (late) __hip_atomic_fetch_or(&C.words[kCtlError], GJ_STEP_CTL_TIMEOUT, __ATOMIC_RELAXED, __HIP_MEMORY_SCOPE_AGENT);
+      if (late || __hip_atomic_load(&C.words[kCtlError], __ATOMIC_RELAXED, __HIP_MEMORY_SCOPE_AGENT) != 0u) {
+        ok = 0u;
+        break;
+      }
+    }
+    __builtin_amdgcn_fence(__ATOMIC_ACQUIRE, "agent");
+    asm volatile("s_waitcnt vmcnt(0)" ::: "memory");
+    *lds_word = ok;
+  }
+  __syncthreads();
+  const bool ok = *lds_word != 0u;
+  __syncthreads();
+  return ok;
+}
+
+__device__ __forceinline__ int item_tid(int wave) {
+  int tid = wave * kWave + (int)__builtin_amdgcn_mbcnt_hi(~0u, __builtin_amdgcn_mbcnt_lo(~0u, 0u));
+  asm volatile("" : "+v"(tid));
+  return tid;
+}
+
+__global__ __launch_bounds__(kTileThreads) void k_tile_step(const TileAArgsT<kFusedSets> A, const TileBArgsT<kFusedSets> B,
+                                                            const TileDArgsT<kFusedSets> D, const FusedCtl C) {
+  extern __shared__ __align__(16) float lds_f[];
+  const int wg = blockIdx.x;
+  const int wave = __builtin_amdgcn_readfirstlane(threadIdx.x / kWave);
+  uint32_t* head = reinterpret_cast<uint32_t*>(lds_f + C.head_word);
+  uint32_t arrivals = 0u;
+  bool alive = true;
+  if (C.first == 0) {
+    for (int s = wg; s < C.n_a; s += C.grid) {
+      tile_scatter_body(A, s, lds_f, item_tid(wave));
+      __syncthreads();
+    }
+    arrivals += (uint32_t)C.grid;
+    if (C.last >= 1) alive = grid_barrier(C, arrivals, head, item_tid(wave) == 0);
+  }
+  if (alive && C.first <= 1 && C.last >= 1) {
+    while (true) {
+      if (item_tid(wave) == 0)
+        *head = __hip_atomic_fetch_add(&C.words[kCtlHead], 1u, __ATOMIC_RELAXED, __HIP_MEMORY_SCOPE_AGENT);
+      __syncthreads();
+      const int item = (int)*head;
+      if (item >= C.n_b) break;
+      tile_venues_body(B, item, lds_f, item_tid(wave));
+      __syncthreads();
+    }
+    arrivals += (uint32_t)C.grid;
+    if (C.last >= 2) alive = grid_barrier(C, arrivals, head, item_tid(wave) == 0);
+  }
+  if (alive && C.last >= 2) {
+    for (int s = wg; s < C.n_d; s += C.grid) {
+      tile_agents_body(D, s, reinterpret_cast<fx_t*>(lds_f), item_tid(wave));
+      __syncthreads();
+    }
+  }
+  if (item_tid(wave) == 0) {
+    const uint32_t left = __hip_atomic_fetch_add(&C.words[kCtlExit], 1u, __ATOMIC_RELAXED, __HIP_MEMORY_SCOPE_AGENT);
+    if (left == (uint32_t)C.grid - 1u) {
+      __hip_atomic_store(&C.words[kCtlHead], 0u, __ATOMIC_RELAXED, __HIP_MEMORY_SCOPE_AGENT);
+      __hip_atomic_store(&C.words[kCtlBarrier], 0u, __ATOMIC_RELAXED, __HIP_MEMORY_SCOPE_AGENT);
+      __hip_atomic_store(&C.words[kCtlExit], 0u, __ATOMIC_RELAXED, __HIP_MEMORY_SCOPE_AGENT);
+    }
+  }
+}
+
+}
diff --git a/gradabm-june_amd/csrc/gradjune_hip.hip b/gradabm-june_amd/csrc/gradjune_hip.hip
--- a/gradabm-june_amd/csrc/gradjune_hip.hip
+++ b/gradabm-june_amd/csrc/gradjune_hip.hip
@@ -1,6 +1,7 @@
 #include <hip/hip_runtime.h>
 #include <math.h>
 #include <stdint.h>
+#include <stdlib.h>
 #include <string.h>
 
 #include "../../include/gradjune_hip.h"
@@ -1284,9 +1285,9 @@
   return GJ_OK;
 }
 
-static void fill_set_a(const gj_plan* plan, const gj_step_params* p, const Groups& G, TSetA* sets) {
+static void fill_set_a(const gj_plan* plan, const gj_step_params* p, const Groups& G, TSetA* sets, int ns = GJ_MAX_SETS) {
   const gj_tiled* T = plan->tiled;
-  for (int s = 0; s < GJ_MAX_SETS; ++s) sets[s] = TSetA{};
+  for (int s = 0; s < ns; ++s) sets[s] = TSetA{};
   for (int g = 0; g < G.n; ++g) {
     const int s = G.set[g];
     const gj_tiled_set& S = T->sets[s];
@@ -1415,17 +1416,24 @@
   return launch_status();
 }
 
+template <int NS>
+static void fill_a(const gj_plan* plan, const gj_agent_state* st, const gj_step_params* p, const Groups& G,
+                   TileAArgsT<NS>& A) {
+  const gj_tiled* T = plan->tiled;
+  fill_set_a(plan, p, G, A.sets, NS);
+  A.n_sets = plan->n_sets;
+  A.slice_agents = T->slice_agents;
+  A.n_agents = plan->n_ext_agents;
+  A.trans = st->transmission;
+  A.qtrans = p->has_quarantine ? st->q_transmission : st->transmission;
+}
+
 static int tiled_scatter(const gj_plan* plan, const gj_agent_state* st, const gj_step_params* p, const Groups& G,
                          hipStream_t stream) {
   const gj_tiled* T = plan->tiled;
   if (plan->n_ext_agents == 0 || G.n == 0) return GJ_OK;
   TileAArgs A;
-  fill_set_a(plan, p, G, A.sets);
-  A.n_sets = plan->n_sets;
-  A.slice_agents = T->slice_agents;
-  A.n_agents = plan->n_ext_agents;
-  A.trans = st->transmission;
-  A.qtrans = p->has_quarantine ? st->q_transmission : st->transmission;
+  fill_a(plan, st, p, G, A);
   const size_t lds = slice_lds(T, sizeof(float));
   int rc = allow_lds(k_tile_scatter, lds);
   if (rc) return rc;
@@ -1448,14 +1456,12 @@
   return bits;
 }
 
-static int tiled_venues(const gj_plan* plan, const gj_agent_state* st, const gj_step_params* p, const Groups& G, int mode,
-                        hipStream_t stream) {
+template <int NS>
+static int fill_b(const gj_plan* plan, const gj_agent_state* st, const gj_step_params* p, const Groups& G, int mode,
+                  TileBArgsT<NS>& B, size_t& lds) {
   const gj_tiled* T = plan->tiled;
-  if (G.n == 0) return GJ_OK;
-  if (T->n_work == 0) return mode == 2 ? GJ_OK : tiled_presum_reduce(plan, p, G, stream);
-  TileBArgs B;
-  for (int s = 0; s < GJ_MAX_SETS; ++s) B.sets[s] = TSetB{};
-  size_t lds = 16;
+  for (int s = 0; s < NS; ++s) B.sets[s] = TSetB{};
+  lds = 16;
   for (int g = 0; g < G.n; ++g) {
     const int s = G.set[g];
     const gj_tiled_set& S = T->sets[s];
@@ -1512,7 +1518,20 @@
   B.day_type = p->day_type;
   B.mode = mode;
   B.transpose = p->transpose;
-  int rc = allow_lds(k_tile_venues, lds);
+  B._pad = 0;
+  return GJ_OK;
+}
+
+static int tiled_venues(const gj_plan* plan, const gj_agent_state* st, const gj_step_params* p, const Groups& G, int mode,
+                        hipStream_t stream) {
+  const gj_tiled* T = plan->tiled;
+  if (G.n == 0) return GJ_OK;
+  if (T->n_work == 0) return mode == 2 ? GJ_OK : tiled_presum_reduce(plan, p, G, stream);
+  TileBArgs B;
+  size_t lds;
+  int rc = fill_b(plan, st, p, G, mode, B, lds);
+  if (rc) return rc;
+  rc = allow_lds(k_tile_venues, lds);
   if (rc) return rc;
   hipLaunchKernelGGL(k_tile_venues, dim3((unsigned)T->n_work), dim3(kTileThreads), lds, stream, B);
   rc = launch_status();
@@ -1520,12 +1539,11 @@
   return tiled_presum_reduce(plan, p, G, stream);
 }
 
-static int tiled_agents(const gj_plan* plan, const gj_agent_state* st, const gj_step_params* p, const Groups& G,
-                        const gj_step_io* io, int sample, hipStream_t stream) {
+template <int NS>
+static int fill_d(const gj_plan* plan, const gj_agent_state* st, const gj_step_params* p, const Groups& G,
+                  const gj_step_io* io, int sample, TileDArgsT<NS>& D, size_t& lds) {
   const gj_tiled* T = plan->tiled;
-  if (plan->n_agents == 0) return GJ_OK;
-  TileDArgs D;
-  fill_set_a(plan, p, G, D.sets);
+  fill_set_a(plan, p, G, D.sets, NS);
   D.n_sets = plan->n_sets;
   D.slice_agents = T->slice_agents;
   D.n_agents = plan->n_agents;
@@ -1548,7 +1566,7 @@
   D.agent_offset = p->agent_offset;
   D.clock = p->clock;
   D.acc_scratch = T->agent_scratch;
-  size_t lds = agents_lds(T);
+  lds = agents_lds(T);
   D.n_direct = 0;
   D.day_type = p->day_type;
   D.transpose = p->transpose;
@@ -1561,7 +1579,7 @@
     const gj_edge_set& E = plan->sets[s];
     const bool run = S.run_pv_win != nullptr;
     if ((!S.ell_k && !run) || S.n_blocks == 0 || E.n_edges == 0) continue;
-    if (D.n_direct == GJ_MAX_DIRECT) return GJ_E_PLAN;
+    if (D.n_direct == NS) return GJ_E_PLAN;
     TDirect& X = D.direct[D.n_direct++];
     X.ell = run ? S.run_pv_win : S.ell;
     X.cum = E.cum;
@@ -1626,7 +1644,20 @@
                      (uintptr_t)D.trans_susc | (uintptr_t)D.acc_scratch | (uintptr_t)D.agent_sums;
     D.io_vec4 = (bits % 16 == 0) ? 1 : 0;
   }
-  int rc = allow_lds(k_tile_agents, lds);
+  D._pad2 = 0;
+  return GJ_OK;
+}
+
+static int tiled_agents(const gj_plan* plan, const gj_agent_state* st, const gj_step_params* p, const Groups& G,
+                        const gj_step_io* io, int sample, hipStream_t stream) {
+  const gj_tiled* T = plan->tiled;
+  if (plan->n_agents == 0) return GJ_OK;
+  const int64_t owned_slices = (plan->n_agents + T->slice_agents - 1) / T->slice_agents;
+  TileDArgs D;
+  size_t lds;
+  int rc = fill_d(plan, st, p, G, io, sample, D, lds);
+  if (rc) return rc;
+  rc = allow_lds(k_tile_agents, lds);
   if (rc) return rc;
   hipLaunchKernelGGL(k_tile_agents, dim3((unsigned)owned_slices), dim3(kTileThreads), lds, stream, D);
   rc = launch_status();
@@ -1655,6 +1686,7 @@
     case GJ_E_RANGE: return "count or index out of range";
     case GJ_E_PLAN: return "inconsistent plan or network list";
     case GJ_E_NODEVICE: return "no HIP device, or not a gfx950 (MI355X) device";
+    case GJ_E_BARRIER: return "a grid barrier of a fused step timed out";
     default: break;
   }
   if (code > 0) return hipGetErrorString((hipError_t)code);
@@ -2034,6 +2066,155 @@
   return gj::do_agent_gather(plan, state, params, G, io, 1, (hipStream_t)stream);
 }
 
+#ifndef GJ_FUSED_DEFAULT_FORM
+#define GJ_FUSED_DEFAULT_FORM GJ_FUSED_OFF
+#endif
+
+namespace gj {
+
+static int fused_env() {
+  static const int mode = [] {
+    const char* e = getenv("GJ_FUSED_STEP");
+    if (!e || !*e) return GJ_FUSED_AUTO;
+    if (!strcmp(e, "0") || !strcmp(e, "off")) return GJ_FUSED_OFF;
+    if (!strcmp(e, "1") || !strcmp(e, "on")) return GJ_FUSED_ALL;
+    if (!strcmp(e, "abc")) return GJ_FUSED_ABC;
+    if (!strcmp(e, "bcd")) return GJ_FUSED_BCD;
+    return GJ_FUSED_AUTO;
+  }();
+  return mode;
+}
+
+static int fused_grid(size_t lds) {
+  static int seen_dev = -1, seen_grid = 0;
+  static size_t seen_lds = 0;
+  int dev = 0;
+  if (hipGetDevice(&dev) != hipSuccess) return 0;
+  if (dev == seen_dev && lds == seen_lds) return seen_grid;
+  int cus = 0, per_cu = 0;
+  if (hipDeviceGetAttribute(&cus, hipDeviceAttributeMultiprocessorCount, dev) != hipSuccess) return 0;
+  if (allow_lds(k_tile_step, lds) != GJ_OK) return 0;
+  if (hipOccupancyMaxActiveBlocksPerMultiprocessor(&per_cu, k_tile_step, kTileThreads, lds) != hipSuccess) {
+    (void)hipGetLastError();
+    return 0;
+  }
+  seen_dev = dev;
+  seen_lds = lds;
+  seen_grid = per_cu >= 1 ? cus : 0;
+  return seen_grid;
+}
+
+static int fused_form(const gj_plan* plan, const gj_step_params* p, const Groups& G, const uint32_t* ctl, int mode,
+                      hipStream_t stream) {
+  const gj_tiled* T = plan->tiled;
+  if (mode == GJ_FUSED_AUTO) mode = fused_env();
+  if (mode == GJ_FUSED_OFF || !ctl || !T) return GJ_FUSED_OFF;
+  if (mode < GJ_FUSED_AUTO || mode > GJ_FUSED_BCD) return GJ_FUSED_OFF;
+  if (p->transpose || T->agent_scratch || plan->n_sets > kFusedSets) return GJ_FUSED_OFF;
+  if (plan->n_agents == 0 || plan->n_ext_agents == 0 || G.n == 0 || T->n_work == 0) return GJ_FUSED_OFF;
+  for (int s = 0; s < plan->n_sets; ++s)
+    if (uses_presum(plan, s)) return GJ_FUSED_OFF;
+  hipStreamCaptureStatus cap = hipStreamCaptureStatusNone;
+  if (hipStreamIsCapturing(stream, &cap) != hipSuccess || cap != hipStreamCaptureStatusNone) {
+    (void)hipGetLastError();
+    return GJ_FUSED_OFF;
+  }
+  return mode;
+}
+
+}
+
+int gj_step_fused(const gj_plan* plan, const gj_agent_state* state, const gj_step_params* params, const gj_step_io* io,
+                  uint32_t* ctl, int32_t mode, int32_t* form_out, void* stream) {
+  using namespace gj;
+  if (form_out) *form_out = GJ_FUSED_OFF;
+  int rc = check_plan(plan);
+  if (rc) return rc;
+  Groups G;
+  rc = group_networks(plan, params, &G);
+  if (rc) return rc;
+  rc = check_state(plan, state, params);
+  if (rc) return rc;
+  hipStream_t st = (hipStream_t)stream;
+  int form = fused_form(plan, params, G, ctl, mode, st);
+  const gj_tiled* T = plan->tiled;
+  TileAArgsT<kFusedSets> A;
+  TileBArgsT<kFusedSets> B;
+  TileDArgsT<kFusedSets> D;
+  FusedCtl C;
+  size_t lds = 0;
+  const bool chosen = mode == GJ_FUSED_AUTO && fused_env() == GJ_FUSED_AUTO;
+  if (chosen && form != GJ_FUSED_OFF) form = GJ_FUSED_DEFAULT_FORM;
+  if (form != GJ_FUSED_OFF) {
+    size_t lds_b = 0, lds_d = 0;
+    fill_a(plan, state, params, G, A);
+    rc = fill_b(plan, state, params, G, 0, B, lds_b);
+    if (rc) return rc;
+    rc = fill_d(plan, state, params, G, io, 1, D, lds_d);
+    if (rc) return rc;
+    const size_t lds_a = slice_lds(T, sizeof(float));
+    lds_b = (lds_b + 15) / 16 * 16;
+    C.head_word = (int32_t)(lds_b / 4);
+    lds_b += 16;
+    lds = lds_b;
+    if (form != GJ_FUSED_BCD && lds_a > lds) lds = lds_a;
+    if (form != GJ_FUSED_ABC && lds_d > lds) lds = lds_d;
+    C.grid = lds <= 160 * 1024 ? fused_grid(lds) : 0;
+    C.words = ctl;
+    C.first = form == GJ_FUSED_BCD ? 1 : 0;
+    C.last = form == GJ_FUSED_ABC ? 1 : 2;
+    C.n_a = T->n_slices;
+    C.n_b = T->n_work;
+    C.n_d = (int32_t)((plan->n_agents + T->slice_agents - 1) / T->slice_agents);
+    C._pad = 0;
+    if (C.grid < 1) form = GJ_FUSED_OFF;
+    if (chosen && form != GJ_FUSED_OFF &&
+        (C.n_a < C.grid || C.n_d < C.grid || C.n_b < 2 * C.grid)) form = GJ_FUSED_OFF;
+  }
+  rc = do_transmission(plan, state, params, st);
+  if (rc) return rc;
+  if (form == GJ_FUSED_OFF) {
+    if (!T) {
+      rc = do_venue_reduce(plan, state, params, G, st);
+      if (rc) return rc;
+      return do_agent_gather(plan, state, params, G, io, 1, st);
+    }
+    rc = tiled_scatter(plan, state, params, G, st);
+    if (rc) return rc;
+    rc = tiled_venues(plan, state, params, G, 0, st);
+    if (rc) return rc;
+    return tiled_agents(plan, state, params, G, io, 1, st);
+  }
+  if (form == GJ_FUSED_BCD) {
+    rc = tiled_scatter(plan, state, params, G, st);
+    if (rc) return rc;
+  }
+  rc = allow_lds(k_tile_step, lds);
+  if (rc) return rc;
+  void* args[] = {(void*)&A, (void*)&B, (void*)&D, (void*)&C};
+#ifdef GJ_FUSED_PLAIN_LAUNCH
+  hipLaunchKernelGGL(k_tile_step, dim3((unsigned)C.grid), dim3(kTileThreads), lds, st, A, B, D, C);
+  (void)args;
+#else
+  const hipError_t e = hipLaunchCooperativeKernel(reinterpret_cast<const void*>(k_tile_step), dim3((unsigned)C.grid),
+                                                  dim3(kTileThreads), args, (unsigned)lds, st);
+  if (e != hipSuccess) return (int)e;
+#endif
+  rc = launch_status();
+  if (rc) return rc;
+  if (form_out) *form_out = form;
+  if (form == GJ_FUSED_ABC) return tiled_agents(plan, state, params, G, io, 1, st);
+  return GJ_OK;
+}
+
+int gj_step_ctl_status(const uint32_t* ctl_host, int32_t n_words) {
+  if (!ctl_host) return GJ_E_NULL;
+  if (n_words < GJ_STEP_CTL_WORDS) return GJ_E_RANGE;
+  if (ctl_host[gj::kCtlError] != 0u) return GJ_E_BARRIER;
+  if (ctl_host[gj::kCtlHead] | ctl_host[gj::kCtlBarrier] | ctl_host[gj::kCtlExit]) return GJ_E_PLAN;
+  return GJ_OK;
+}
+
 int gj_step_phase(const gj_plan* plan, const gj_agent_state* state, const gj_step_params* params,
                   const gj_step_io* io, int phase, void* stream) {
   int rc = gj::check_plan(plan);
diff --git a/gradabm-june_amd/grad_june_amd/_native.py b/gradabm-june_amd/grad_june_amd/_native.py
--- a/gradabm-june_amd/grad_june_amd/_native.py
+++ b/gradabm-june_amd/grad_june_amd/_native.py
@@ -13,6 +13,10 @@
 GJ_STREAM_EDGES = 2048
 GJ_MAX_GROUPS = 1 << 28
 GJ_GROUP_ERR_LABEL, GJ_GROUP_ERR_VALUE = 1, 2
+GJ_ABI_MINOR = 1
+GJ_E_BARRIER = -5
+GJ_STEP_CTL_WORDS, GJ_STEP_CTL_ERROR_WORD, GJ_STEP_CTL_TIMEOUT = 64, 16, 1
+GJ_FUSED_AUTO, GJ_FUSED_OFF, GJ_FUSED_ALL, GJ_FUSED_ABC, GJ_FUSED_BCD = -1, 0, 1, 2, 3
 
 MASK_RAW, MASK_Q, MASK_QL, MASK_QL_AGE75 = 0, 1, 2, 3
 
@@ -220,6 +224,12 @@
         C.c_int,
         [C.POINTER(Plan), C.POINTER(AgentState), C.POINTER(StepParams), C.POINTER(StepIO), C.c_int, _vp],
     ),
+    "gj_step_fused": (
+        C.c_int,
+        [C.POINTER(Plan), C.POINTER(AgentState), C.POINTER(StepParams), C.POINTER(StepIO), _vp, C.c_int32,
+         C.POINTER(C.c_int32), _vp],
+    ),
+    "gj_step_ctl_status": (C.c_int, [C.POINTER(C.c_uint32), C.c_int32]),
     "gj_clock_advance": (C.c_int, [_vp, C.c_double, _vp]),
     "gj_symptoms_step_stats": (
         C.c_int,
diff --git a/gradabm-june_amd/grad_june_amd/autograd.py b/gradabm-june_amd/grad_june_amd/autograd.py
--- a/gradabm-june_amd/grad_june_amd/autograd.py
+++ b/gradabm-june_amd/grad_june_amd/autograd.py
@@ -161,7 +161,8 @@
                             transmission=trans, current_stage=stage)
         keep = _keep_sums(env) and plan.c.tiled is not None and bool(plan.c.tiled)
         acc = torch.empty(n, dtype=torch.float32, device=plan.device) if keep else None
-        engine.step(bufs, params, engine.io(new_infected=new_inf, exp_noise=exp_noise, agent_sums=acc))
+        engine.step(bufs, params, engine.io(new_infected=new_inf, exp_noise=exp_noise, agent_sums=acc),
+                    fused_mode=N.GJ_FUSED_OFF)
         ctx.env = env
         ctx.save_for_backward(susc.detach().to(torch.float32).contiguous(), inf.detach().to(torch.float32).contiguous(),
                               time.detach().to(torch.float32).contiguous())
diff --git a/gradabm-june_amd/grad_june_amd/engine.py b/gradabm-june_amd/grad_june_amd/engine.py
--- a/gradabm-june_amd/grad_june_amd/engine.py
+++ b/gradabm-june_amd/grad_june_amd/engine.py
@@ -4,6 +4,7 @@
 import math
 from typing import Dict, Optional, Sequence
 
+import numpy as np
 import torch
 
 from . import _native as N
@@ -69,6 +70,10 @@
         self.lib = N.load()
         self.plan = plan
         self._q_trans: Optional[torch.Tensor] = None
+        self.fused_mode = N.GJ_FUSED_AUTO
+        self.last_form = N.GJ_FUSED_OFF
+        self._form = C.c_int32(0)
+        self._ctl: Optional[torch.Tensor] = None
 
     def q_transmission_buffer(self) -> torch.Tensor:
         if self._q_trans is None:
@@ -130,10 +135,24 @@
         N.check(self.lib.gj_agent_gather(C.byref(self.plan.c), C.byref(bufs.c), C.byref(p), C.byref(io),
                                          1 if sample else 0, N.current_stream()), "gj_agent_gather")
 
-    def step(self, bufs: AgentBuffers, p: N.StepParams, io: N.StepIO):
+    def step_ctl(self) -> torch.Tensor:
+        if self._ctl is None:
+            self._ctl = torch.zeros(N.GJ_STEP_CTL_WORDS, dtype=torch.int32, device=self.plan.device)
+        return self._ctl
+
+    def step(self, bufs: AgentBuffers, p: N.StepParams, io: N.StepIO, fused_mode: Optional[int] = None):
         self._prep(bufs, p)
-        N.check(self.lib.gj_step(C.byref(self.plan.c), C.byref(bufs.c), C.byref(p), C.byref(io),
-                                 N.current_stream()), "gj_step")
+        N.check(self.lib.gj_step_fused(C.byref(self.plan.c), C.byref(bufs.c), C.byref(p), C.byref(io),
+                                       self.step_ctl().data_ptr(),
+                                       self.fused_mode if fused_mode is None else fused_mode, C.byref(self._form),
+                                       N.current_stream()), "gj_step_fused")
+        self.last_form = self._form.value
+
+    def check_step_ctl(self) -> np.ndarray:
+        words = self.step_ctl().cpu().numpy().view(np.uint32).copy()
+        N.check(self.lib.gj_step_ctl_status(words.ctypes.data_as(C.POINTER(C.c_uint32)), int(words.size)),
+                "fused step")
+        return words
 
     def step_phase(self, bufs: AgentBuffers, p: N.StepParams, io: N.StepIO, phase: int):
         self._prep(bufs, p)
diff --git a/include/gradjune_hip.h b/include/gradjune_hip.h
--- a/include/gradjune_hip.h
+++ b/include/gradjune_hip.h
@@ -8,6 +8,7 @@
 #endif
 
 #define GJ_ABI_VERSION 7
+#define GJ_ABI_MINOR 1
 
 #define GJ_MAX_SETS 12
 #define GJ_MAX_NETS 16
@@ -19,6 +20,7 @@
 #define GJ_E_RANGE (-2)
 #define GJ_E_PLAN (-3)
 #define GJ_E_NODEVICE (-4)
+#define GJ_E_BARRIER (-5)
 
 typedef enum gj_mask_kind {
   GJ_MASK_RAW = 0,
@@ -173,6 +175,19 @@
   float* agent_sums;
 } gj_step_io;
 
+#define GJ_STEP_CTL_WORDS 64
+#define GJ_STEP_CTL_ERROR_WORD 16
+#define GJ_STEP_CTL_TIMEOUT 1u
+#define GJ_FUSED_AUTO (-1)
+#define GJ_FUSED_OFF 0
+#define GJ_FUSED_ALL 1
+#define GJ_FUSED_ABC 2
+#define GJ_FUSED_BCD 3
+int gj_step_fused(const gj_plan* plan, const gj_agent_state* state, const gj_step_params* params,
+                  const gj_step_io* io, uint32_t* ctl, int32_t mode, int32_t* form, void* stream);
+
+int gj_step_ctl_status(const uint32_t* ctl_host, int32_t n_words);
+
 int gj_transmission_update(const gj_plan* plan, const gj_agent_state* state,
                            const gj_step_params* params, void* stream);
 
```
